# schmidtniko/visual_marker_mapping

Hardware: AMD Instinct MI355X
Metric: lm_iterations_per_sec (higher is better)
Workload: dtype f64; 1 GPU; configs[1]: 500 images x 200 tags, visibility 1.00, 100000 tag observations (400000 corner residual blocks), no loss, perturbed initial guess; eliminated_family=cameras, reduced_system_order=1200, elimination_form=dense Z + MFMA rank-k, kept_family_order=natural

## Files before the change

### visual_marker_mapping_amd/csrc/chol_common.hpp

```cpp
#pragma once
#include "engine.hpp"

namespace vmm {

constexpr int kLd = 65;
constexpr int kLdT = 66;

typedef double double4_t __attribute__((ext_vector_type(4)));

__device__ __forceinline__ double safe_rsqrt(double v, bool& ok)
{
    ok = ok && (v > 0.0) && isfinite(v);
    const double y0 = __builtin_amdgcn_rsq(v);
    const double e = fma(-v * y0, y0, 1.0);
    return fma(y0 * e, fma(e, 0.375, 0.5), y0);
}

__device__ __forceinline__ bool nz_bit(const unsigned long long* nz, const int i, const int k)
{
    return (nz[kDfMaskWords * i + (k >> 6)] >> (k & 63)) & 1ull;
}

constexpr int kPs = 9;
constexpr int kPw = 8;
// ... 19 lines not shown
        const double t = p.l[tri8(j, j)];
        bool okj = true;
        const double inv = safe_rsqrt(t, okj);
        p.ok = p.ok && okj;
        p.inv[j] = inv;
        p.l[tri8(j, j)] = t * inv;
#pragma unroll
        for (int i = j + 1; i < 8; ++i)
            p.l[tri8(i, j)] *= inv;
#pragma unroll
        for (int c = j + 1; c < 8; ++c)
#pragma unroll
            for (int i = c; i < 8; ++i)
                p.l[tri8(i, c)] = fma(-p.l[tri8(i, j)], p.l[tri8(c, j)], p.l[tri8(i, c)]);
    }
}

__device__ __forceinline__ void scale8(double (&x)[8], const Piv8& p)
{
#pragma unroll
    for (int q = 0; q < 8; ++q) {
        x[q] *= p.inv[q];
#pragma unroll
        for (int c = q + 1; c < 8; ++c)
            x[c] = fma(-x[q], p.l[tri8(c, q)], x[c]);
    }
}

constexpr unsigned kSpinLimit = 1u << 22;

__device__ __forceinline__ void raise_sync_timeout(LmCtl* ctl, int bit)
{
    atomicOr(&ctl->sync_timeout, bit);
    atomicExch(&ctl->done, 2);
}

__device__ __forceinline__ void chol_inverse_lds(const double* L, const double* di, double* __restrict__ Linvk)
{
    const int tid = threadIdx.x;
    if (tid >= 64)
        return;
    const int c = tid;
    double x[64];
#pragma unroll
    for (int i = 0; i < 64; ++i) {
        double s0 = 0.0, s1 = 0.0, s2 = 0.0, s3 = 0.0;
#pragma unroll
        for (int m = 0; m + 3 < i; m += 4) {
            s0 += L[i * kLd + m] * x[m];
            s1 += L[i * kLd + m + 1] * x[m + 1];
            s2 += L[i * kLd + m + 2] * x[m + 2];
            s3 += L[i * kLd + m + 3] * x[m + 3];
        }
#pragma unroll
        for (int m = (i / 4) * 4; m < i; ++m)
            s0 += L[i * kLd + m] * x[m];
        const double s = (s0 + s1) + (s2 + s3);
        x[i] = (i == c) ? di[i] : ((i < c) ? 0.0 : -s * di[i]);
        Linvk[i * 64 + c] = x[i];
    }
}

__device__ __forceinline__ void chol_inverse_wg(const double* __restrict__ Ldk, const double* __restrict__ dinvk,
                                                double* __restrict__ Linvk, double* smem)
{
    double* L = smem;
    double* di = smem + 64 * kLd;
// ... 13 lines not shown
```

### visual_marker_mapping_amd/csrc/covariance.hip

```cpp
#include <string.h>

#include <algorithm>
#include <functional>
#include <string>
#include <vector>

#include "host.hpp"

namespace vmm {

struct CovDensePath {
    Engine& e;
    bool v, nz;
    CovDensePath(Engine& e_) : e(e_), v(e_.sparse_schur), nz(e_.chol_nz_on) {}
    int enter()
    {
        if (v) {
            int drc;
            if ((drc = ensure_dense_schur(e))) return drc;
            e.sparse_schur = false;
        }
        e.chol_nz_on = false;
        return VMM_BA_OK;
    }
    ~CovDensePath()
    {
        e.sparse_schur = v;
        e.chol_nz_on = nz;
    }
};

static hipError_t cov_factor_and(Engine& e, int robustify, double huber_a, hipError_t err,
                                 const std::function<hipError_t()>& tail)
{
    vmm_ba_options o;
    vmm_ba_default_options(&o);
    o.robustify = robustify;
    o.huber_a = huber_a;
    for (int attempt = 0; attempt < 2 && err == hipSuccess; ++attempt) {
        init_ctl(e, *e.ctl_host, o, 0);
        err = hipMemcpyAsync(e.ctl, e.ctl_host, sizeof(LmCtl), hipMemcpyHostToDevice, e.stream);
        if (err != hipSuccess)
            break;
        launch_eval_passes(e, robustify, huber_a, false);
        launch_cov_prepare(e);
        launch_elim(e);
        launch_syrk_reduced(e);
        launch_cholesky_solve(e, e.S, e.n_pad, e.ldz, e.yf, e.ctl, attempt > 0);
        launch_chol_inverse(e, e.n_blk - 1);
        err = tail();
        if (err == hipSuccess)
            err = hipMemcpyAsync(e.ctl_host, e.ctl, sizeof(LmCtl), hipMemcpyDeviceToHost, e.stream);
        if (err == hipSuccess)
            err = hipStreamSynchronize(e.stream);
        if (err != hipSuccess || e.ctl_host->done != 2)
            break;
    }
    return err;
}

int tag_pose_handle(const Engine& e, const char* who)
{
    if (e.multi || e.points) {
        set_error(std::string(who) + " needs a single-GPU handle with tag-pose landmarks");
        return VMM_BA_ERR_STATE;
    }
    return VMM_BA_OK;
}

static int select_and_flush(Engine& e)
{
    HIP_TRY(hipSetDevice(e.device));
    return flush_state(e);
}

static int covariance_call(Engine& e, const char* who, int robustify, double huber_a,
                           const std::function<void(Arena&)>& carve, const std::function<hipError_t()>& tail,
                           const char* matrix = "J^T J", const std::function<hipError_t()>& upload = nullptr,
                           const std::string& alloc_step = "")
{
    CovDensePath dense(e);
    int rc;
    if ((rc = dense.enter())) return rc;
    Arena ar;
    if (ar.layout(carve) != hipSuccess)
        return hip_failure(who, alloc_step.c_str(), ar.err);
    const hipError_t err = cov_factor_and(e, robustify, huber_a, upload ? upload() : hipSuccess, tail);
    if (err != hipSuccess)
        return hip_failure(who, "", err);
    if (e.ctl_host->lin_fail) {
        set_error(std::string(who) + ": " + matrix + " is not positive definite (rank-deficient Jacobian)");
        return VMM_BA_ERR_NUMERIC;
    }
    return VMM_BA_OK;
}

}

using namespace vmm;

extern "C" {

int vmm_ba_tag_translation_covariance(vmm_ba_handle h, int robustify, double huber_a, double* cov)
{
    if (!h || !cov) {
        set_error("bad argument");
        return VMM_BA_ERR_ARGUMENT;
    }
    static const char who[] = "tag_translation_covariance";
    Engine& e = *reinterpret_cast<Engine*>(h);
    int rc;
    if ((rc = tag_pose_handle(e, who))) return rc;
    if ((rc = select_and_flush(e))) return rc;
    if (e.n_obs == 0 || e.n_tags == 0) {
        memset(cov, 0, sizeof(double) * 9 * (size_t)e.n_tags);
        return VMM_BA_OK;
    }
    const bool identity_rhs = e.elim_cams;
    const int n_rhs = identity_rhs ? e.n_pad : e.k_dim;
    const int ldb = round_up(n_rhs, 64);
    double *B = nullptr, *cov_dev = nullptr;
    auto carve = [&](Arena& a) {
        B = a.take<double>((size_t)e.n_pad * ldb);
// ... 138 lines not shown
```

### visual_marker_mapping_amd/csrc/diagnostics.hip

```cpp
#include <stdio.h>
#include <string.h>

#include <string>
#include <vector>

#include "host.hpp"

namespace vmm {

template <typename T, hipError_t (*Destroy)(T), int N = 1>
struct Owned {
    T h[N] = {};
    Owned() = default;
    Owned(const Owned&) = delete;
    Owned& operator=(const Owned&) = delete;
    ~Owned() { release(); }
    void release()
    {
        for (T& x : h) {
            if (x)
                (void)Destroy(x);
            x = nullptr;
        }
    }
// ... 61 lines not shown
    if ((rc = restore_raw())) return rc;
    OwnedEvents<2> events;
    hipEvent_t &ev0 = events.h[0], &ev1 = events.h[1];
    HIP_TRY(hipEventCreate(&ev0));
    HIP_TRY(hipEventCreate(&ev1));
    auto timed = [&](auto&& fn, auto&& prep, double* ms_out, int inner = 1) -> int {
        Owned<hipGraph_t, hipGraphDestroy> graph;
        Owned<hipGraphExec_t, hipGraphExecDestroy> exec;
        hipGraph_t& g = graph.h[0];
        hipGraphExec_t& ge = exec.h[0];
        HIP_TRY(hipStreamBeginCapture(e.stream, hipStreamCaptureModeThreadLocal));
        for (int q = 0; q < inner; ++q)
            fn();
        HIP_TRY(hipStreamEndCapture(e.stream, &g));
        HIP_TRY(hipGraphInstantiate(&ge, g, nullptr, nullptr, 0));
        graph.release();
        double total = 0.0;
        for (int r = 0; r < reps + 1; ++r) {
            prep();
            HIP_TRY(hipEventRecord(ev0, e.stream));
            HIP_TRY(hipGraphLaunch(ge, e.stream));
            HIP_TRY(hipEventRecord(ev1, e.stream));
            HIP_TRY(hipEventSynchronize(ev1));
            float ms = 0.f;
            HIP_TRY(hipEventElapsedTime(&ms, ev0, ev1));
            if (r > 0) total += ms;
        }
        exec.release();
        *ms_out = total / reps / inner;
        return VMM_BA_OK;
    };
    auto nop = [] {};
    HIP_TRY(hipMemcpy(e.ctl_host, e.ctl, sizeof(LmCtl), hipMemcpyDeviceToHost));
    e.ctl_host->done = 0;
    e.ctl_host->lin_fail = 0;
    HIP_TRY(hipMemcpy(e.ctl, e.ctl_host, sizeof(LmCtl), hipMemcpyHostToDevice));
    if ((rc = timed([&] { launch_eval_passes(e, o.robustify, o.huber_a, false); }, nop, &out->eval_elim_ms, 8))) return rc;
    out->eval_keep_ms = 0.0;
    if ((rc = timed([&] { launch_cost_kernel(e, e.cam_qt, e.tag_qt, false, o.robustify, o.huber_a); }, nop, &out->cost_ms, 8))) return rc;
    if ((rc = timed([&] { launch_elim(e); }, nop, &out->form_z_ms, 8))) return rc;
    if ((rc = timed([&] { launch_syrk_only(e); }, nop, &out->syrk_ms, 4))) return rc;
    if ((rc = timed([&] { launch_cholesky_solve(e, e.S, e.n_pad, e.ldz, e.yf, e.ctl); },
                    [&] {
                        launch_syrk_reduced(e);
                        launch_pack_lower(e, false);
                        launch_pack_lower(e, true);
                    },
                    &out->cholesky_ms)))
        return rc;
    if ((rc = timed([&] { launch_backsub(e); }, nop, &out->backsub_ms, 8))) return rc;
    if (e.sw.debug) {
        HIP_TRY(hipMemcpy(e.ctl_host, e.ctl, sizeof(LmCtl), hipMemcpyDeviceToHost));
        fprintf(stderr, "[vmm_ba debug] after kernel timing: done=%d lin_fail=%d termination=%d iteration=%d\n",
                e.ctl_host->done, e.ctl_host->lin_fail, e.ctl_host->termination, e.ctl_host->iteration);
    }
    if ((rc = restore_raw())) return rc;
    if ((rc = begin_lm_loop(e, ot, 0))) return rc;
    HIP_TRY(hipEventRecord(ev0, e.stream));
    int passes = 0;
    for (int r = 0; r < reps; ++r) {
        if ((rc = run_iteration(e, ot))) return rc;
        passes += e.last_passes;
    }
    HIP_TRY(hipEventRecord(ev1, e.stream));
    HIP_TRY(hipEventSynchronize(ev1));
    float ms = 0.f;
    HIP_TRY(hipEventElapsedTime(&ms, ev0, ev1));
    out->lm_iteration_ms = ms / passes;
    events.release();
    return restore_raw();
}

int vmm_ba_debug_chol_schedule(int n_blk, int n_df, int n_cu, int32_t* launches, int cap, int* n_launches, int* n_df_used)
{
    if (n_blk < 1 || n_cu < 1 || cap < 0 || (cap > 0 && !launches) || !n_launches || (n_df > 0 && n_df > n_blk - 2)) {
        set_error("bad argument");
        return VMM_BA_ERR_ARGUMENT;
    }
    if (n_df < 0) {
        n_df = dataflow_blocks(n_blk, n_cu, read_switches());
        if (n_df == n_blk)
            n_df = 0;
    }
    const std::vector<CholLaunch> sched = chol_step_schedule(n_blk, n_df);
    for (size_t i = 0; i < sched.size() && (int)i < cap; ++i) {
        const CholLaunch& L = sched[i];
        const int32_t row[8] = { L.k, L.lazy[0], L.lazy[1], L.upd[0], L.upd[1], L.c0, L.t0, L.t1 };
// ... 25 lines not shown
    Engine& e = *reinterpret_cast<Engine*>(h);
    if (e.multi || e.sparse_schur || !e.Z) {
        set_error("debug_overlap needs a single-GPU handle on the dense elimination path");
        return VMM_BA_ERR_STATE;
    }
    HIP_TRY(hipSetDevice(e.device));
    int rc;
    if ((rc = flush_state(e))) return rc;
    vmm_ba_options o;
    vmm_ba_default_options(&o);
    o.max_num_iterations = 1 << 30;
    o.function_tolerance = o.parameter_tolerance = o.gradient_tolerance = 0.0;
    if (e.trace_capacity < 1) {
        if ((rc = dev_alloc(e, &e.trace, 1, false))) return rc;
        e.trace_capacity = 1;
        drop_graphs(e);
    }
    if ((rc = begin_lm_loop(e, o, 0))) return rc;
    if ((rc = enqueue_iteration(e, o))) return rc;
    HIP_TRY(hipStreamSynchronize(e.stream));
    Arena scratch;
    Owned<hipStream_t, hipStreamDestroy> second;
    OwnedEvents<5> events;
    hipStream_t& sb = second.h[0];
    hipEvent_t(&ev)[5] = events.h;
    hipError_t err = scratch.alloc(sizeof(double) * (size_t)e.ldz * e.ldz);
    double* const S2 = reinterpret_cast<double*>(scratch.base);
    if (err == hipSuccess) err = hipStreamCreateWithFlags(&sb, hipStreamNonBlocking);
    for (int i = 0; i < 5 && err == hipSuccess; ++i)
        err = hipEventCreate(&ev[i]);
    auto reset_flags = [&]() -> hipError_t {
        hipError_t r = hipMemcpy(e.ctl_host, e.ctl, sizeof(LmCtl), hipMemcpyDeviceToHost);
        if (r != hipSuccess) return r;
        e.ctl_host->done = 0;
        e.ctl_host->lin_fail = 0;
        e.ctl_host->sync_timeout = 0;
        return hipMemcpy(e.ctl, e.ctl_host, sizeof(LmCtl), hipMemcpyHostToDevice);
    };
    double acc[8] = { 0.0, 0.0, 0.0, 0.0, 0.0, 0.0, 0.0, 0.0 };
    for (int r = 0; r < reps + 1 && err == hipSuccess; ++r) {
        float t[8] = { 0.f, 0.f, 0.f, 0.f, 0.f, 0.f, 0.f, 0.f };
        if ((err = reset_flags()) != hipSuccess) break;
        (void)hipEventRecord(ev[0], e.stream);
        launch_syrk_reduced(e);
        (void)hipEventRecord(ev[1], e.stream);
        launch_cholesky_solve(e, e.S, e.n_pad, e.ldz, e.yf, e.ctl);
        (void)hipEventRecord(ev[2], e.stream);
        if ((err = hipEventSynchronize(ev[2])) != hipSuccess) break;
        (void)hipEventElapsedTime(&t[0], ev[0], ev[1]);
        (void)hipEventElapsedTime(&t[1], ev[1], ev[2]);
        (void)hipEventElapsedTime(&t[2], ev[0], ev[2]);
        if ((err = reset_flags()) != hipSuccess) break;
        launch_syrk_reduced(e);
        if ((err = hipStreamSynchronize(e.stream)) != hipSuccess) break;
        (void)hipEventRecord(ev[0], e.stream);
        (void)hipStreamWaitEvent(sb, ev[0], 0);
        launch_cholesky_solve(e, e.S, e.n_pad, e.ldz, e.yf, e.ctl);
        (void)hipEventRecord(ev[3], e.stream);
        launch_syrk_plan(sb, e.ctl, e.Z, e.ldz, e.syrk);
        launch_reduce_plan(sb, e.ctl, e.syrk, e.ldz, e.n_pad + 1, S2);
        (void)hipEventRecord(ev[1], sb);
        (void)hipStreamWaitEvent(e.stream, ev[1], 0);
        (void)hipEventRecord(ev[2], e.stream);
        if ((err = hipEventSynchronize(ev[2])) != hipSuccess) break;
        (void)hipEventElapsedTime(&t[3], ev[0], ev[2]);
        (void)hipEventElapsedTime(&t[4], ev[0], ev[3]);
        (void)hipEventElapsedTime(&t[5], ev[0], ev[1]);
        if ((err = reset_flags()) != hipSuccess) break;
// ... 34 lines not shown
```

### visual_marker_mapping_amd/csrc/engine.hpp

```cpp
#pragma once
#include <hip/hip_runtime.h>
#include <stdint.h>

#include <string>
#include <vector>

#include "../../include/vmm_ba.h"
#include "geom.hpp"
#include "plan.hpp"

namespace vmm {

constexpr int kLdsRow = 80;

struct ObsOrder {
    int64_t n = 0;
    int64_t n_pad = 0;
    int32_t* own = nullptr;
    int32_t* other = nullptr;
    int32_t* caller = nullptr;
    double* px = nullptr;
    Task* tasks = nullptr;
    int32_t n_tasks = 0;
    int32_t* pose_task = nullptr;
    double* part = nullptr;
    int32_t* start = nullptr;
};

struct LmCtl {
    int32_t max_num_iterations, robustify, jacobi_scaling, max_invalid;
    double huber_a, function_tolerance, gradient_tolerance, parameter_tolerance;
    double max_radius, min_radius, min_relative_decrease, min_lm_diagonal, max_lm_diagonal;
    double radius, decrease_factor;
    int32_t reuse_diagonal, num_invalid;
    double x_cost, cand_cost, model_cost_change, x_norm, initial_cost;
    int32_t iteration;
    int32_t first_eval;
    int32_t done, termination;
    int32_t lin_fail;
    int32_t sync_timeout;
    int32_t num_sync_timeouts;
    int32_t sync_kernels;
    uint32_t spin_limit_df, spin_limit_chain;
    int32_t spin_wg;
    int32_t records;
    int32_t num_successful, num_unsuccessful, num_lm_iterations, num_jac_evals, num_cost_evals;
    int32_t trace_capacity;
    int32_t w_which;
    vmm_ba_iteration cur;
    unsigned long long stamp[6];
    unsigned long long phase_ticks[5];
};

__device__ __forceinline__ int64_t small_sel(const LmCtl* ctl, const int64_t alt_off) { return ctl->w_which ? alt_off : 0; }

__device__ __forceinline__ void phase_stamp(const LmCtl* ctl, int slot)
{
    if (blockIdx.x == 0 && blockIdx.y == 0 && threadIdx.x == 0)
        const_cast<LmCtl*>(ctl)->stamp[slot] = __builtin_amdgcn_s_memrealtime();
}

struct SyrkPlan {
    int n_tiles = 0, n_kt = 0, n_wg = 0, n_segments = 0;
    int32_t *tile_bi = nullptr, *tile_bj = nullptr, *wg_seg0 = nullptr, *tile_seg0 = nullptr;
    int64_t *wg_u0 = nullptr, *wg_u1 = nullptr;
    double* partials = nullptr;
    bool wide = false;
};

struct Engine {
    int device = 0;
    int n_cu = 256;
    hipStream_t stream = nullptr;
    int rank = 0, world = 1;
    Switches sw;
    bool multi = false;
    vmm_ba_allreduce_fn allreduce = nullptr;
    void* allreduce_user = nullptr;
    void* rccl_comm = nullptr;
    bool rccl_graph = true;

    Intrinsics K;
    int n_cams = 0, n_tags = 0, fixed_tag = -1;
    bool points = false;
    int n_tags_user = 0;
    int64_t n_obs_user = 0;
    std::vector<double> user_tag_wh;
    int64_t n_obs = 0;
    bool elim_cams = true;
    int n_e = 0, n_f = 0;

    double* cam_qt = nullptr;
    double* tag_qt = nullptr;
    double* cam_cand = nullptr;
    double* tag_cand = nullptr;
    double* tag_wh = nullptr;

    ObsOrder ordE, ordF;
// ... 149 lines not shown
        return p;
    }
    template <typename Carve>
    hipError_t layout(Carve&& carve)
    {
        carve(*this);
        const size_t total = used;
        used = 0;
        if (alloc(total) == hipSuccess)
            carve(*this);
        return err;
    }
    void copy(void* dst, const void* src, size_t bytes, hipMemcpyKind kind)
    {
        if (err == hipSuccess)
            err = hipMemcpy(dst, src, bytes, kind);
    }
};

int preload_eval_kernels();
int preload_schur_kernels();
int preload_chol_kernels();
int preload_lm_kernels();
int preload_cov_kernels();
int preload_init_kernels();

void launch_eval_passes(Engine& e, int robustify, double huber_a, bool use_ctl);
void launch_cost_kernel(Engine& e, const double* cam, const double* tag, bool guard, int robustify, double huber_a);
void launch_cost(Engine& e, const double* cam, const double* tag, bool guard, int robustify, double huber_a,
                 double* out_scalar);
void launch_stats(Engine& e, double* per_corner_dev);
void launch_project(hipStream_t st, const Intrinsics& K, int64_t n, const double* pc, double* uv);
void launch_sum(Engine& e, bool guard, const double* in, int n, double* out);
void launch_elim(Engine& e);
void launch_schur_rows(Engine& e, bool add_diag);
void launch_syrk_only(Engine& e);
void launch_syrk_reduced(Engine& e);
void launch_pack_lower(Engine& e, bool unpack);
void launch_syrk_plan(hipStream_t st, const LmCtl* ctl, const double* Z, int ldz, const SyrkPlan& p);
void launch_reduce_plan(hipStream_t st, const LmCtl* ctl, const SyrkPlan& p, int ld, int n_rows, double* S);
void launch_cholesky_solve(Engine& e, double* S, int n_pad, int ld, double* y, LmCtl* ctl, bool safe = false);
int dataflow_workgroups(int n_blk);
int dataflow_max_workgroups(int n_cu, const Switches& sw);
int dataflow_blocks(int n_blk, int n_cu, const Switches& sw);
void launch_chol_inverse(Engine& e, int k);
struct CholLaunch {
    int k;
    int lazy[2];
    int upd[2];
    int c0, t0, t1;
};
std::vector<CholLaunch> chol_step_schedule(int n_blk, int n_df);
void chol_schedule_tile(int n_blk, const CholLaunch& L, int t, int* bi, int* bj);
void launch_chol_steps(Engine& e, double* S, int n_pad, int ld, LmCtl* ctl, int n_df);
int preload_chol_step_kernels();
void launch_dataflow(Engine& e, double* S, int n_pad, int ld, LmCtl* ctl, int first_blk, int n_blk);
int preload_chol_dataflow_kernels();
void launch_backsolve_chain(Engine& e, double* S, int n_pad, int ld, double* y, LmCtl* ctl);
void launch_backsolve_steps(Engine& e, double* S, int n_pad, int ld, double* y, LmCtl* ctl);
int preload_backsolve_kernels();
void launch_cov_prepare(Engine& e);
void launch_cov_rhs(Engine& e, double* B, int ldb, bool identity_rhs);
void launch_cov_trsm(Engine& e, double* B, int ldb, int n_chunks, bool identity_rhs);
void launch_cov_gram(Engine& e, const double* X, int ldb, double* cov_dev);
void launch_cov_rhs_slots(Engine& e, const int32_t* slot_src, int n_slots, double* B, int ldb);
void launch_cov_trsm_mfma(Engine& e, double* B, int ldb, const std::vector<int>& chunks_at);
// ... 168 lines not shown
```

### visual_marker_mapping_amd/csrc/kernels_backsolve.hip

```cpp
#include "chol_common.hpp"

namespace vmm {

__global__ __launch_bounds__(256) void k_backsolve_step(const LmCtl* ctl, double* __restrict__ S, int ld,
                                                        int n_pad, int n_blk, int kb, double* __restrict__ y,
                                                        const double* __restrict__ dinv,
                                                        const double* __restrict__ Ld)
{
    if (ctl->done || ctl->lin_fail)
        return;
    __shared__ double red[4][64];
    __shared__ double L[64 * kLd];
    __shared__ double ws[64];
    __shared__ double di[64];
    const int m = blockIdx.x;
    const int tid = threadIdx.x;
    const int c = tid & 63, part = tid >> 6;
    double* w = S + (int64_t)n_pad * ld;
    double wc = 0.0;
    if (kb + 1 < n_blk) {
        const int R0 = (kb + 1) * kNB + part * 16;
        const double* Lb = S + (int64_t)R0 * ld + m * kNB + c;
        double acc = 0.0;
#pragma unroll
        for (int r = 0; r < 16; ++r)
            acc += Lb[(int64_t)r * ld] * y[R0 + r];
        red[part][c] = acc;
    }
    if (m == kb) {
        const int K0 = kb * kNB;
        for (int idx = tid; idx < 64 * 64; idx += 256) {
            const int r = idx >> 6, cc = idx & 63;
            L[r * kLd + cc] = (cc <= r) ? Ld[(int64_t)kb * 4096 + r * 64 + cc] : 0.0;
        }
        if (tid < 64)
            di[tid] = dinv[K0 + tid];
    }
    __syncthreads();
    if (part == 0) {
        wc = w[m * kNB + c];
        if (kb + 1 < n_blk) {
            wc -= (red[0][c] + red[1][c]) + (red[2][c] + red[3][c]);
// ... 27 lines not shown

int backsolve_chain_workgroups(int n_blk) { return n_blk; }

__device__ __forceinline__ void chain_block_done(unsigned* n_done, int n_blk, unsigned* epoch_word, unsigned epoch)
{
    if (atomicAdd(n_done, 1u) == (unsigned)n_blk - 1u) {
        *n_done = 0u;
        *epoch_word = epoch;
    }
}

#ifdef VMM_STAMPS
__device__ unsigned long long g_chain_stamps[128][4];
#define CH_RT(blk, slot)                                                                  \
    do {                                                                                  \
        if (threadIdx.x == 0)                                                             \
            g_chain_stamps[(blk) & 127][slot] = __builtin_amdgcn_s_memrealtime();         \
    } while (0)
extern "C" int vmm_ba_debug_read_chain_stamps(unsigned long long* out)
{
    return (int)hipMemcpyFromSymbol(out, HIP_SYMBOL(g_chain_stamps), sizeof(unsigned long long) * 128 * 4);
}
#else
#define CH_RT(blk, slot)
#endif

template <bool TREE>
__device__ __forceinline__ void backsolve_chain_body(LmCtl* ctl, const double* __restrict__ S, int ld, int n_pad, int n_blk,
                                                     double* y, const double* __restrict__ dinv, unsigned long long* gran,
                                                     unsigned* epoch_word, const double* __restrict__ Ld,
                                                     const double* __restrict__ Linv,
                                                     const unsigned long long* __restrict__ nz, unsigned* n_done)
{
    if (ctl->done || ctl->lin_fail) {
        if constexpr (TREE) {
            if (threadIdx.x == 0)
                chain_block_done(n_done, n_blk, epoch_word, *epoch_word + 1u);
        } else {
            if (blockIdx.x == gridDim.x - 1 && threadIdx.x == 0)
                *epoch_word = *epoch_word + 1u;
        }
        return;
    }
    const unsigned spin_limit = (ctl->spin_limit_chain && (ctl->spin_wg < 0 || ctl->spin_wg == (int)blockIdx.x))
                                    ? ctl->spin_limit_chain : kSpinLimit;
    __shared__ double L[64 * kLd];
    __shared__ double Li[64 * kLd];
    __shared__ double red[4][64];
    __shared__ double ws[64];
    __shared__ double ys[2][64];
    __shared__ double sB[16][256];
    __shared__ int s_timeout;
    const int m = n_blk - 1 - (int)blockIdx.x;
    const int tid = threadIdx.x;
    const int c = tid & 63, part = tid >> 6;
    const unsigned epoch = *epoch_word + 1u;
    const int K0 = m * kNB;
    if (tid == 0)
        s_timeout = 0;
    CH_RT(m, 0);
    auto receive = [&](const int j, double* ysj) {
        if (part == 0) {
            const unsigned long long* g = gran + 2 * (int64_t)(j * kNB + c);
            unsigned long long x0, x1;
            for (unsigned n = 0;;) {
                x0 = __hip_atomic_load(g, __ATOMIC_RELAXED, __HIP_MEMORY_SCOPE_AGENT);
                x1 = __hip_atomic_load(g + 1, __ATOMIC_RELAXED, __HIP_MEMORY_SCOPE_AGENT);
                const bool ok = (unsigned)(x0 >> 32) == epoch && (unsigned)(x1 >> 32) == epoch;
                if (__all(ok) && spin_limit != 1u)
                    break;
                __builtin_amdgcn_s_sleep(1);
                if (++n >= spin_limit) {
                    s_timeout = 1;
                    break;
                }
            }
            ysj[c] = __longlong_as_double((long long)(((x1 & 0xffffffffull) << 32) | (x0 & 0xffffffffull)));
        }
// ... 205 lines not shown
```

### visual_marker_mapping_amd/csrc/kernels_chol_dataflow.hip

```cpp
#include <type_traits>
#include <utility>

#include "chol_common.hpp"

namespace vmm {

constexpr int kDfSlice = 2 * 8 * 64;
constexpr int kPsD = 10;
constexpr unsigned kDfSpinDefault = 1u << 21;
constexpr int kDfXs = 8 * kLdsRow;
constexpr int kDfSmemUsed = 64 * kLdT + 4 * 64 * kPsD + 64 + 2 * 8 * kPsD + 4 * kDfXs;
constexpr int kDfSmem = 84 * 1024 / 8;
static_assert(kDfSmemUsed <= kDfSmem, "dataflow LDS layout");
static_assert(4 * 64 * kPsD + 64 + 4 * kDfXs >= 64 * kLd + 64, "the inverse's staging area must fit into the dead buffers");

struct DfArgs {
    LmCtl* ctl;
    double* S;
    int ld, n_pad, n_blk;
    double* dinv;
    double* Ld;
    double* Linv;
    unsigned long long* G;
    const unsigned* epoch_word;
// ... 819 lines not shown
        const double* XJ = m.Xs + (it & 1) * 2 * kDfXs;
        const double* XR = XJ + kDfXs;
        __syncthreads();
        if (WK == 0 || HAS_T) {
            Ops o[2];
            load_ops_slice<WK, HAS_T>(XJ, XR, fr, fk, o);
            for_tiles([&](auto idx) {
                constexpr int I = decltype(idx)::value;
                if constexpr ((HAS_T || !is_t(WK, I)) && I >= kHelpSplit)
                    mfma_tile<WK, I>(acc, o);
            }, Seq13{});
        }
    }
    double* M = m.RA + WK * (13 - kHelpSplit) * 256;
    for_tiles([&](auto idx) {
        constexpr int I = decltype(idx)::value;
        if constexpr (I >= kHelpSplit) {
#pragma unroll
            for (int r = 0; r < 4; ++r)
                M[((I - kHelpSplit) * 4 + r) * 64 + lane] = acc[I][r];
        }
    }, Seq13{});
    __syncthreads();
}

__device__ __forceinline__ void report_give_up(const DfArgs& a, const unsigned epoch, const int& s_timeout)
{
    if (threadIdx.x == 0
        && (s_timeout || __hip_atomic_load(a.abort_word, __ATOMIC_RELAXED, __HIP_MEMORY_SCOPE_AGENT) == epoch))
        raise_sync_timeout(a.ctl, 1);
}

template <bool HAS_T, bool TREE, int MODE>
__device__ __forceinline__ void role(const DfArgs& a, const int j, const int R, double* smem)
{
    constexpr bool BULK = (MODE & 1) != 0, HELP = (MODE & 2) != 0;
    const int tid = threadIdx.x;
    const int lane = tid & 63;
    const int w = __builtin_amdgcn_readfirstlane(tid >> 6);
    const int K0 = j * kNB;
    const int R0 = R * kNB;
    const int n_blk = a.n_blk, ld = a.ld, n_pad = a.n_pad;
    if (TREE && HAS_T && R < n_blk && !nz_bit(a.nz, R, j))
        return;
    const unsigned epoch = *a.epoch_word + 1u;
    Lds m;
    m.RA = smem;
    m.Pd = m.RA + 64 * kLdT;
    m.Pt = m.Pd + 2 * 64 * kPsD;
    m.invd = m.Pt + 2 * 64 * kPsD;
    m.Pb = m.invd + 64;
    m.Nd = m.Pb + 8 * kPsD;
    m.Xs = m.Nd + 8 * kPsD;
    m.stamp_j = -1;
#ifdef VMM_STAMPS
    if (TREE ? !HAS_T : (HAS_T && R == j + 1))
        m.stamp_j = j;
    {
        const bool stamp_on = m.stamp_j >= 0 && w == 0;
        const int stamp_j = m.stamp_j;
        DF_RT(0);
    }
#endif
    double* Li = m.Pd;
    double* di = Li + 64 * kLd;
    __shared__ int s_timeout;
    if (tid == 0)
        s_timeout = 0;
    SliceMap sm;
    sm.G = a.G;
    sm.n_blk = n_blk;
    sm.slot = TREE ? a.slot : nullptr;
    __syncthreads();
    bool ok = true;
    if (w < 2)
        pivot_path<HAS_T, TREE, MODE>(a, w, lane, j, R, m, sm, epoch, &s_timeout, ok);
    else if (w == 2)
        worker_path<0, HAS_T, TREE, HELP>(a, lane, j, R, m);
// ... 15 lines not shown
        for (int idx = tid; idx < 64 * 64; idx += 256) {
            const int r = idx >> 6, c = idx & 63;
            const double v = (c <= r) ? m.RA[c * kLdT + r] : 0.0;
            if (c <= r)
                a.Ld[(int64_t)j * 4096 + r * 64 + c] = v;
            Li[r * kLd + c] = v;
        }
        if (tid < 64)
            di[tid] = iv;
        __syncthreads();
        if (j < n_blk - 1)
            chol_inverse_lds(Li, di, a.Linv + (int64_t)j * 4096);
        report_give_up(a, epoch, s_timeout);
        return;
    }
    for (int idx = tid; idx < 64 * 32; idx += 256) {
        const int rr = idx >> 5, c = (idx & 31) * 2;
        if (R0 + rr <= n_pad)
            *reinterpret_cast<double2*>(a.S + (int64_t)(R0 + rr) * ld + K0 + c)
                = make_double2(m.RA[rr * kLd + c], m.RA[rr * kLd + c + 1]);
    }
    if (BULK) {
        double* cb = a.Gc + sm.index(j, R) * 4096;
        for (int idx = tid; idx < 64 * 64; idx += 256) {
            const int c = idx >> 6, rr = idx & 63;
            cb[idx] = m.RA[rr * kLd + c];
        }
        __threadfence();
        __syncthreads();
        if (tid == 0)
            __hip_atomic_store(a.done + sm.index(j, R), epoch, __ATOMIC_RELEASE, __HIP_MEMORY_SCOPE_AGENT);
    }
    if (j == n_blk - 1 && tid == 0 && !ok)
        a.ctl->lin_fail = 1;
    report_give_up(a, epoch, s_timeout);
}

}

template <bool TREE, int MODE>
__device__ __forceinline__ void chol_dataflow_body(DfArgs& a)
{
    if (a.ctl->done)
        return;
    a.spin_limit = (a.ctl->spin_limit_df && (a.ctl->spin_wg < 0 || a.ctl->spin_wg == (int)blockIdx.x)) ? a.ctl->spin_limit_df
                                                                                                          : kDfSpinDefault;
    phase_stamp(a.ctl, 3);
    if (a.ctl->lin_fail)
        return;
    __shared__ __attribute__((aligned(16))) double smem[kDfSmem];
    if (TREE) {
        const int j = a.wg[2 * (int)blockIdx.x], R = a.wg[2 * (int)blockIdx.x + 1];
        if (R > j)
            df2::role<true, TREE, MODE>(a, j, R, smem);
        else
            df2::role<false, TREE, MODE>(a, j, j, smem);
        return;
    }
    int b = (int)blockIdx.x, j = 0;
    for (; j < a.n_blk; ++j) {
        const int cnt = a.n_blk - j + 1;
        if (b < cnt)
            break;
        b -= cnt;
    }
    if (j >= a.n_blk)
        return;
    if (b < a.n_blk - j)
        df2::role<true, TREE, MODE>(a, j, j + 1 + b, smem);
    else
        df2::role<false, TREE, MODE>(a, j, j, smem);
}

__global__ __launch_bounds__(256) void k_chol_dataflow(DfArgs a)
{
    chol_dataflow_body<false, 0>(a);
}

__global__ __launch_bounds__(256) void k_chol_dataflow_bulk(DfArgs a)
{
    chol_dataflow_body<false, 1>(a);
}

__global__ __launch_bounds__(256) void k_chol_dataflow_tree(DfArgs a)
{
    chol_dataflow_body<true, 1>(a);
}

__global__ __launch_bounds__(384) void k_chol_dataflow_tree_help(DfArgs a)
{
    chol_dataflow_body<true, 3>(a);
}

void launch_dataflow(Engine& e, double* S, int n_pad, int ld, LmCtl* ctl, int first_blk, int n_blk)
{
    DfArgs a;
    a.ctl = ctl;
    a.S = S + (int64_t)first_blk * kNB * (ld + 1);
    a.ld = ld;
    a.n_pad = n_pad - first_blk * kNB;
    a.n_blk = n_blk - first_blk;
    a.dinv = e.dinv + first_blk * kNB;
    a.Ld = e.Ldiag + (int64_t)first_blk * 4096;
    a.Linv = e.Linv + (int64_t)first_blk * 4096;
// ... 35 lines not shown
```

### visual_marker_mapping_amd/csrc/kernels_chol_step.hip

```cpp
#include "chol_common.hpp"

namespace vmm {

#ifdef VMM_STAMPS
__device__ unsigned long long g_stamps[64];
#define STAMP(slot)                                                                  \
    do {                                                                             \
        if (blockIdx.x == 1 && threadIdx.x == 0 && k == 1) {                         \
            g_stamps[slot] = __builtin_amdgcn_s_memtime();                           \
            g_stamps[16 + slot] = __builtin_amdgcn_s_memrealtime();                  \
        }                                                                            \
    } while (0)
#define USTAMP(slot)                                                                 \
    do {                                                                             \
        if (u == 0 && threadIdx.x == 0 && k == 1 && t == u + n_wg)                   \
            g_stamps[(slot)] = __builtin_amdgcn_s_memtime();                         \
    } while (0)
#else
#define USTAMP(slot)
#define STAMP(slot)
#endif

template <int J0, bool HAS_T>
__device__ __forceinline__ void panel_round(const int w, const int lane,
// ... 146 lines not shown
            if (HAS_T)
                *reinterpret_cast<double2*>(&Ats[mm * kLdsRow + c]) = vt[it];
        }
        __syncthreads();
#pragma unroll 4
        for (int ks = 0; ks < 16; ++ks) {
            const int row = (ks * 4 + fk) * kLdsRow;
            const double ad = -Ads[row + 16 * w + fr];
            const double at = HAS_T ? -Ats[row + 16 * w + fr] : 0.0;
#pragma unroll
            for (int tj = 0; tj < 4; ++tj) {
                const double b = Ads[row + 16 * tj + fr];
                const double adm = (tj <= w) ? ad : 0.0;
                Dacc[tj] = __builtin_amdgcn_mfma_f64_16x16x4f64(adm, b, Dacc[tj], 0, 0, 0);
                if (HAS_T)
                    Tacc[tj] = __builtin_amdgcn_mfma_f64_16x16x4f64(at, b, Tacc[tj], 0, 0, 0);
            }
        }
    }
    STAMP(1);
    bool ok = true;
    panel_round<0, HAS_T>(w, lane, Dacc, Tacc, Pd, Pt, RA, RA, invd, ok);
    panel_round<8, HAS_T>(w, lane, Dacc, Tacc, Pd, Pt, RA, RA, invd, ok);
    panel_round<16, HAS_T>(w, lane, Dacc, Tacc, Pd, Pt, RA, RA, invd, ok);
    panel_round<24, HAS_T>(w, lane, Dacc, Tacc, Pd, Pt, RA, RA, invd, ok);
    panel_round<32, HAS_T>(w, lane, Dacc, Tacc, Pd, Pt, RA, RA, invd, ok);
    panel_round<40, HAS_T>(w, lane, Dacc, Tacc, Pd, Pt, RA, RA, invd, ok);
    panel_round<48, HAS_T>(w, lane, Dacc, Tacc, Pd, Pt, RA, RA, invd, ok);
    panel_round<56, HAS_T>(w, lane, Dacc, Tacc, Pd, Pt, RA, RA, invd, ok);
    __syncthreads();
    STAMP(2);
    if (!HAS_T) {
        if (tid == 0 && !ok)
            ctl->lin_fail = 1;
        if (tid < 64)
            dinv[K0 + tid] = invd[tid];
        for (int idx = tid; idx < 64 * 64; idx += 256) {
            const int r = idx >> 6, c = idx & 63;
            if (c <= r)
                Ld[(int64_t)k * 4096 + r * 64 + c] = RA[c * kLdT + r];
        }
        return;
    }
    STAMP(4);
    const double* R = RA;
    for (int idx = tid; idx < 64 * 32; idx += 256) {
        const int rr = idx >> 5, c = (idx & 31) * 2;
        if (R0 + rr <= n_pad)
            *reinterpret_cast<double2*>(S + (int64_t)(R0 + rr) * ld + K0 + c)
                = make_double2(R[rr * kLd + c], R[rr * kLd + c + 1]);
    }
    {
        const int rr = tid & 63;
        if (R0 + rr <= n_pad)
            for (int c = tid >> 6; c < 64; c += 4)
                P[(int64_t)c * ld + R0 + rr] = R[rr * kLd + c];
    }
    STAMP(5);
}

constexpr int kPanelSmem = 64 * kLdT + 4 * 64 * kPs + 64 + 2 * 64 * kLdsRow;
constexpr int kUpdateSmem = 4 * 64 * kLdsRow;
constexpr int kStepSmem = kPanelSmem > kUpdateSmem ? kPanelSmem : kUpdateSmem;

__device__ __forceinline__ void chol_panel_wg(LmCtl* ctl, double* __restrict__ S, int ld, int n_pad, int k,
                                              double* __restrict__ P, const double* __restrict__ Pprev,
                                              const double* __restrict__ Pprev2, double* __restrict__ dinv,
// ... 394 lines not shown
#pragma unroll
        for (int a = 0; a < 2; ++a)
#pragma unroll
            for (int b = 0; b < 2; ++b)
#pragma unroll
                for (int r = 0; r < 4; ++r)
                    __builtin_nontemporal_store(creg[a][b][r] + acc[a][b][r],
                                                &S[(int64_t)(I0 + wi * 32 + a * 16 + fk + 4 * r) * ld + J0 + wj * 32 + b * 16 + fi]);
#pragma unroll
        for (int it = 0; it < 8; ++it) {
            const int idx = it * 256 + tid;
            const int m = idx >> 5, c = (idx & 31) * 2;
            *reinterpret_cast<double2v*>(&L0[m * kLdsRow + c]) = wa[it];
            *reinterpret_cast<double2v*>(&L0[(64 + m) * kLdsRow + c]) = wb[it];
        }
        __syncthreads();
        bi = nbi;
        bj = nbj;
        t = tn;
        tn = slot[2 + (iter & 1)];
        if (t >= t1)
            break;
    }
}

__global__ __launch_bounds__(256) void k_chol_step(LmCtl* ctl, double* __restrict__ S, int ld, int n_pad, int n_blk,
                                                   int k, int n_panel, double* __restrict__ Pcur,
                                                   const double* __restrict__ Pprev, const double* __restrict__ Pprev2,
                                                   double* __restrict__ dinv, double* __restrict__ Ld,
                                                   double* __restrict__ Linv, const double* __restrict__ PA,
                                                   const double* __restrict__ PB, int c0, int t0, int t1, int n_upd_wg,
                                                   unsigned* tile_ctr)
{
    if (ctl->done)
        return;
    if (k == 0)
        phase_stamp(ctl, 3);
    if (ctl->lin_fail)
        return;
    if (blockIdx.x == 0 && threadIdx.x == 0)
        tile_ctr[(k + 1) & 1] = 0u;
    __shared__ __attribute__((aligned(16))) double smem[kStepSmem];
    if ((int)blockIdx.x < n_panel) {
        chol_panel_wg(ctl, S, ld, n_pad, k, Pcur, Pprev, Pprev2, dinv, Ld, smem);
        if (t1 > t0) {
            __syncthreads();
            if (PB)
                chol_update2_wg(S, ld, n_blk, c0, tile_ctr + (k & 1), t0, t1, PA, PB, smem);
            else
                chol_update_wg(S, ld, n_blk, c0 - 2, tile_ctr + (k & 1), t1, PA, smem);
        }
    } else if ((int)blockIdx.x < n_panel + n_upd_wg) {
        if (PB)
            chol_update2_wg(S, ld, n_blk, c0, tile_ctr + (k & 1), t0, t1, PA, PB, smem);
        else
            chol_update_wg(S, ld, n_blk, c0 - 2, tile_ctr + (k & 1), t1, PA, smem);
    } else
        chol_inverse_wg(Ld + (int64_t)(k - 1) * 4096, dinv + (k - 1) * kNB, Linv + (int64_t)(k - 1) * 4096, smem);
}

__global__ __launch_bounds__(256) void k_chol_inverse(const LmCtl* ctl, const double* __restrict__ Ld,
                                                      const double* __restrict__ dinv, double* __restrict__ Linv, int k)
{
    if (ctl->done || ctl->lin_fail)
        return;
    __shared__ __attribute__((aligned(16))) double smem[64 * kLd + 64];
    chol_inverse_wg(Ld + (int64_t)k * 4096, dinv + k * kNB, Linv + (int64_t)k * 4096, smem);
}

void launch_chol_inverse(Engine& e, int k)
{
    hipLaunchKernelGGL(k_chol_inverse, dim3(1), dim3(256), 0, e.stream, (const LmCtl*)e.ctl, (const double*)e.Ldiag,
                       (const double*)e.dinv, e.Linv, k);
}

constexpr int kPairMinBlocks = 46;

static int update_tiles(int n_blk, int k)
{
    int tiles = 0;
    for (int r = k + 2; r <= n_blk; ++r)
        tiles += ((r < n_blk) ? r : n_blk - 1) - (k + 1);
    return tiles;
}

std::vector<CholLaunch> chol_step_schedule(int n_blk, int n_df)
{
    std::vector<CholLaunch> out;
    const int n_step = n_blk - n_df;
    int k_pair = 0;
    while (n_blk - k_pair > kPairMinBlocks)
        k_pair += 2;
    if (k_pair > n_step)
        k_pair = n_step;
    for (int k = 0; k < n_step; ++k) {
        CholLaunch L = { k, { -1, k > 0 ? k - 1 : -1 }, { -1, -1 }, k + 1, 0, 0 };
        if (k >= 2 && k <= k_pair) {
// ... 73 lines not shown
```

### visual_marker_mapping_amd/csrc/kernels_eval.hip

```cpp
#include "engine.hpp"

namespace vmm {

struct EvalArgs {
    Intrinsics K;
    const Task* tasks;
    int n_tasks;
    const int32_t* other;
    const double* px;
    int64_t n_pad;
    const double* own_pose;
    const double* other_pose;
    const double* tag_wh;
    const uint8_t* cam_const;
    const uint8_t* tag_const;
    int robustify;
    double huber_a;
    double* part;
    void* W;
    void* W_alt;
    const int32_t* caller;
    const uint8_t* mask;
    const LmCtl* ctl;
};

__device__ __forceinline__ int tri(int a, int b) { return a * (a + 1) / 2 + b; }

template <bool OWN_IS_CAM, bool WRITE_W, typename AT, bool POINTS = false>
__device__ __forceinline__ void eval_body(const EvalArgs& a, const int wave)
{
    const int lane = threadIdx.x & 63;
    if (wave >= a.n_tasks)
        return;
    const Task t = a.tasks[wave];
    const int64_t i = (int64_t)t.begin + lane;
    const bool valid = i < t.end;
    const int64_t is = valid ? i : t.begin;
    const int o = a.other[is];
    AT* __restrict__ const Wout = static_cast<AT*>((WRITE_W && a.W_alt && a.ctl && a.ctl->w_which == 0) ? a.W_alt : a.W);

    const int tag_idx = OWN_IS_CAM ? o : t.pose;
    const int cam_idx = OWN_IS_CAM ? t.pose : o;
    const double* camq = (OWN_IS_CAM ? a.own_pose : a.other_pose) + 7 * (int64_t)cam_idx;
    const double* tagq = (OWN_IS_CAM ? a.other_pose : a.own_pose) + 7 * (int64_t)tag_idx;
    Rigid cam, tag;
    double pt[6];
    if (POINTS) {
        load_rigid<false>(camq, cam);
#pragma unroll
        for (int k = 0; k < 6; ++k)
            pt[k] = tagq[k];
    } else {
        load_rigid<true>(camq, cam);
        load_rigid<true>(tagq, tag);
    }
    const double hw = POINTS ? 0.0 : 0.5 * a.tag_wh[2 * tag_idx], hh = POINTS ? 0.0 : 0.5 * a.tag_wh[2 * tag_idx + 1];
    const bool cam_c = a.cam_const[cam_idx] != 0, tag_c = a.tag_const[tag_idx] != 0;
    const bool on = valid && a.mask[a.caller[is]];

    AT H[21];
    double g[6], cost = 0.0;
    AT Wacc[WRITE_W ? 36 : 1];
#pragma unroll
    for (int k = 0; k < 21; ++k)
        H[k] = (AT)0;
#pragma unroll
    for (int k = 0; k < 6; ++k)
        g[k] = 0.0;
    if (WRITE_W) {
#pragma unroll
        for (int k = 0; k < 36; ++k)
            Wacc[k] = (AT)0;
    }

    constexpr bool NEED_JC = OWN_IS_CAM || WRITE_W;
    constexpr bool NEED_JT = !OWN_IS_CAM || WRITE_W;
#pragma unroll 1
    for (int c = 0; c < (POINTS ? 2 : 4); ++c) {
        const double sx = (c == 1 || c == 2) ? hw : -hw;
        const double sy = (c >= 2) ? hh : -hh;
        const double u = a.px[(2 * c) * a.n_pad + is];
        const double v = a.px[(2 * c + 1) * a.n_pad + is];
        CornerEval e;
        if (POINTS) {
            eval_point<NEED_JC, NEED_JT>(a.K, cam, camq, pt[3 * c], pt[3 * c + 1], pt[3 * c + 2], u, v, e, on);
            if (NEED_JT) {
#pragma unroll
                for (int r = 0; r < 2; ++r) {
                    const double j0 = e.jt[r][0], j1 = e.jt[r][1], j2 = e.jt[r][2];
                    e.jt[r][0] = c == 0 ? j0 : 0.0;
                    e.jt[r][1] = c == 0 ? j1 : 0.0;
// ... 40 lines not shown
#pragma unroll
                for (int p = 0; p < 6; ++p)
#pragma unroll
                    for (int q = 0; q < 6; ++q)
                        Wacc[6 * p + q] += ja[p] * jx[q];
            }
        }
    }
    if (WRITE_W && valid) {
#pragma unroll
        for (int k = 0; k < 36; ++k)
            Wout[(int64_t)k * a.n_pad + i] = Wacc[k];
    }
    double red[32];
#pragma unroll
    for (int k = 0; k < 21; ++k)
        red[k] = (double)H[k];
#pragma unroll
    for (int k = 0; k < 6; ++k)
        red[21 + k] = g[k];
    red[27] = cost;
#pragma unroll
    for (int k = 28; k < 32; ++k)
        red[k] = 0.0;
    const double mine = wave_sum32(red, lane);
    const int slot = wave_sum32_index(lane);
    if (!(lane & 1) && slot < 28)
        a.part[(int64_t)wave * kPart + slot] = mine;
}

template <bool E_IS_CAM, typename AT = double, bool POINTS = false>
__global__ __launch_bounds__(256) __attribute__((amdgpu_waves_per_eu(2, 2))) void k_eval_both(const EvalArgs aE, const EvalArgs aF, const int nb_e)
{
    if (aE.ctl) {
        if (aE.ctl->done)
            return;
        phase_stamp(aE.ctl, 0);
    }
    if ((int)blockIdx.x < nb_e)
        eval_body<E_IS_CAM, true, AT, POINTS>(aE, (int)((blockIdx.x * blockDim.x + threadIdx.x) >> 6));
    else
        eval_body<!E_IS_CAM, false, AT, POINTS>(aF, (int)(((blockIdx.x - nb_e) * blockDim.x + threadIdx.x) >> 6));
}


struct FusedArgs {
    const int32_t* pair_obs;
    const int32_t* e_list;
    const int32_t* e_part0;
    int n_e_act, n_f, n_f_pad, n_chunks, group, n_groups;
    double* partF;
};

template <bool E_IS_CAM, typename AT, bool POINTS>
__global__ __launch_bounds__(256) __attribute__((amdgpu_waves_per_eu(1, 1)))
void k_eval_fused(const EvalArgs a, const FusedArgs fa)
{
    if (a.ctl) {
        if (a.ctl->done)
            return;
        phase_stamp(a.ctl, 0);
    }
    const int lane = threadIdx.x & 63;
    const int wave = (int)((blockIdx.x * blockDim.x + threadIdx.x) >> 6);
    if (wave >= fa.n_groups * fa.n_chunks)
        return;
    const int grp = wave / fa.n_chunks, c = wave - grp * fa.n_chunks;
    const int f = 64 * c + lane;
    const bool fvalid = f < fa.n_f;
    const int fs = fvalid ? f : fa.n_f - 1;
    AT* __restrict__ const Wout = static_cast<AT*>((a.W_alt && a.ctl && a.ctl->w_which == 0) ? a.W_alt : a.W);
    const double* keptq = a.other_pose + 7 * (int64_t)fs;
    Rigid kept;
    double pt[6];
    if (POINTS && E_IS_CAM) {
#pragma unroll
        for (int k = 0; k < 6; ++k)
            pt[k] = keptq[k];
    } else if (POINTS) {
        load_rigid<false>(keptq, kept);
    } else {
        load_rigid<true>(keptq, kept);
    }
    AT HF[21];
    double gF[6];
#pragma unroll
    for (int k = 0; k < 21; ++k)
        HF[k] = (AT)0;
#pragma unroll
    for (int k = 0; k < 6; ++k)
        gF[k] = 0.0;
    const int e0 = grp * fa.group, e1 = min(e0 + fa.group, fa.n_e_act);
    constexpr int NPX = POINTS ? 4 : 8;
    int e_n = __builtin_amdgcn_readfirstlane(fa.e_list[e0]);
    int idx_n = fvalid ? fa.pair_obs[(int64_t)e_n * fa.n_f_pad + f] : -1;
    int e_nn = e_n, idx_nn = -1;
    if (e0 + 1 < e1) {
        e_nn = __builtin_amdgcn_readfirstlane(fa.e_list[e0 + 1]);
        idx_nn = fvalid ? fa.pair_obs[(int64_t)e_nn * fa.n_f_pad + f] : -1;
    }
    double px_n[NPX];
    int on_n;
    {
        const int64_t isn = idx_n >= 0 ? idx_n : 0;
// ... 133 lines not shown
            red[k] = 0.0;
        const double mine = wave_sum32(red, lane);
        const int slot = wave_sum32_index(lane);
        if (!(lane & 1) && slot < 28)
            a.part[(int64_t)(fa.e_part0[e] + c) * kPart + slot] = mine;
    }
    if (fvalid) {
        double* pf = fa.partF + (int64_t)grp * 28 * fa.n_f_pad + f;
#pragma unroll
        for (int k = 0; k < 21; ++k)
            pf[(int64_t)k * fa.n_f_pad] = (double)HF[k];
#pragma unroll
        for (int k = 0; k < 6; ++k)
            pf[(int64_t)(21 + k) * fa.n_f_pad] = gF[k];
    }
}

struct ReduceArgs {
    int n_pose;
    const int32_t* pose_task;
    int n_fixed;
    int64_t st, sk, sp;
    const double* part;
    double* Hout;
    double* gout;
    double* pose_cost;
    const double* pose7;
    int euclid;
    double* gm_out;
};

__global__ void k_reduce_pose(const LmCtl* ctl, const ReduceArgs rE, const ReduceArgs rF, const int64_t alt_off)
{
    int64_t off = 0;
    if (ctl) {
        if (ctl->done)
            return;
        off = ctl->w_which ? 0 : alt_off;
    }
    int tid = blockIdx.x * blockDim.x + threadIdx.x;
    const bool first = tid < 32 * rE.n_pose;
    if (!first)
        tid -= 32 * rE.n_pose;
    const ReduceArgs& r = first ? rE : rF;
    const int n_pose = r.n_pose;
    const int32_t* __restrict__ pose_task = r.pose_task;
    const double* __restrict__ part = r.part;
    double* __restrict__ Hout = r.Hout + off;
    double* __restrict__ gout = r.gout + off;
    double* __restrict__ pose_cost = r.pose_cost;
    const int p = tid >> 5, k = tid & 31;
    if (p >= n_pose || k >= 28)
        return;
    const int t0 = pose_task ? pose_task[p] : 0, t1 = pose_task ? pose_task[p + 1] : r.n_fixed;
    const double* __restrict__ pp = part + (int64_t)k * r.sk + (int64_t)p * r.sp;
    double s0 = 0.0, s1 = 0.0, s2 = 0.0, s3 = 0.0;
    int t = t0;
    for (; t + 3 < t1; t += 4) {
        s0 += pp[(int64_t)t * r.st];
        s1 += pp[(int64_t)(t + 1) * r.st];
        s2 += pp[(int64_t)(t + 2) * r.st];
        s3 += pp[(int64_t)(t + 3) * r.st];
    }
    if (t < t1) s0 += pp[(int64_t)t * r.st];
    if (t + 1 < t1) s1 += pp[(int64_t)(t + 1) * r.st];
    if (t + 2 < t1) s2 += pp[(int64_t)(t + 2) * r.st];
    const double s = (s0 + s1) + (s2 + s3);
    if (k < 21) {
        int a = 0;
        while ((a + 1) * (a + 2) / 2 <= k)
            ++a;
        const int b = k - a * (a + 1) / 2;
        Hout[36 * (int64_t)p + 6 * a + b] = s;
        Hout[36 * (int64_t)p + 6 * b + a] = s;
    } else if (k < 27) {
        gout[6 * (int64_t)p + (k - 21)] = s;
    } else if (pose_cost) {
        pose_cost[p] = s;
    }
    if (r.gm_out) {
        double ng[6];
#pragma unroll
        for (int j = 0; j < 6; ++j)
            ng[j] = -__shfl(s, 21 + j, 32);
        if (k == 21) {
            const double* x = r.pose7 + 7 * (int64_t)p;
            double xp[7], gm = 0.0;
            if (r.euclid) {
#pragma unroll
                for (int j = 0; j < 6; ++j)
                    xp[j] = x[j] + ng[j];
                xp[6] = x[6];
            } else {
                pose_plus(x, ng, xp);
            }
#pragma unroll
            for (int j = 0; j < 7; ++j)
                gm = fmax(gm, fabs(x[j] - xp[j]));
            r.gm_out[p] = gm;
        }
    }
}

__global__ __launch_bounds__(256) void k_sum(const LmCtl* ctl, const double* __restrict__ in, int n, int stride,
                                             double* __restrict__ out)
{
    if (ctl && ctl->done)
        return;
    __shared__ double sh[256];
    double s = 0.0;
    for (int i = threadIdx.x; i < n; i += 256)
        s += in[(int64_t)i * stride];
    sh[threadIdx.x] = s;
    __syncthreads();
    for (int m = 128; m >= 1; m >>= 1) {
        if ((int)threadIdx.x < m)
            sh[threadIdx.x] += sh[threadIdx.x + m];
        __syncthreads();
    }
    if (threadIdx.x == 0)
        out[0] = sh[0];
}

struct CostArgs {
    Intrinsics K;
    const Task* tasks;
    int n_tasks;
    const int32_t* other;
    const double* px;
    int64_t n_pad;
    const double* own_pose;
    const double* other_pose;
    const double* tag_wh;
    int robustify;
    double huber_a;
    double* part;
    const int32_t* caller;
    const uint8_t* mask;
    const LmCtl* ctl;
};

template <bool OWN_IS_CAM, bool POINTS = false>
__global__ __launch_bounds__(256) void k_cost(const CostArgs a)
{
    if (a.ctl && a.ctl->done)
        return;
    const int wave = (int)((blockIdx.x * blockDim.x + threadIdx.x) >> 6);
    const int lane = threadIdx.x & 63;
    if (wave >= a.n_tasks)
        return;
    const Task t = a.tasks[wave];
    const int64_t i = (int64_t)t.begin + lane;
    const bool valid = i < t.end;
    const int64_t is = valid ? i : t.begin;
    const int o = a.other[is];
    const int tag_idx = OWN_IS_CAM ? o : t.pose;
    const int cam_idx = OWN_IS_CAM ? t.pose : o;
    const double* camq = (OWN_IS_CAM ? a.own_pose : a.other_pose) + 7 * (int64_t)cam_idx;
    const double* tagq = (OWN_IS_CAM ? a.other_pose : a.own_pose) + 7 * (int64_t)tag_idx;
    Rigid cam, tag;
    double pt[6];
    if (POINTS) {
        load_rigid<false>(camq, cam);
#pragma unroll
        for (int k = 0; k < 6; ++k)
            pt[k] = tagq[k];
    } else {
        load_rigid<true>(camq, cam);
        load_rigid<true>(tagq, tag);
    }
    const double hw = POINTS ? 0.0 : 0.5 * a.tag_wh[2 * tag_idx], hh = POINTS ? 0.0 : 0.5 * a.tag_wh[2 * tag_idx + 1];
    double cost = 0.0;
#pragma unroll
    for (int c = 0; c < (POINTS ? 2 : 4); ++c) {
        const double sx = (c == 1 || c == 2) ? hw : -hw;
        const double sy = (c >= 2) ? hh : -hh;
        CornerEval e;
        if (POINTS)
// ... 105 lines not shown
    const double rad = 1.0 + r2 * (K.k1 + r2 * (K.k2 + r2 * K.k3));
    double xd, yd;
    distort(K, true, x, y, r2, rad, xd, yd);
    uv[2 * i] = K.fx * xd + K.cx;
    uv[2 * i + 1] = K.fy * yd + K.cy;
}


static inline int blocks_for_tasks(int n_tasks) { return (n_tasks + 3) / 4; }

static EvalArgs make_eval_args(Engine& e, const ObsOrder& ord, bool own_is_cam, void* W, bool lm = false)
{
    EvalArgs a;
    a.K = e.K;
    a.tasks = ord.tasks;
    a.n_tasks = ord.n_tasks;
    a.other = ord.other;
    a.px = ord.px;
    a.n_pad = ord.n_pad;
    const double* cam = lm ? e.cam_cand : e.cam_qt;
    const double* tag = lm ? e.tag_cand : e.tag_qt;
    a.own_pose = own_is_cam ? cam : tag;
    a.other_pose = own_is_cam ? tag : cam;
    a.tag_wh = e.tag_wh;
    a.cam_const = e.pose_const;
    a.tag_const = e.pose_const + e.n_cams;
    a.robustify = 0;
    a.huber_a = 1.0;
    a.part = ord.part;
    a.W = W;
    a.W_alt = (lm && W) ? (e.f32_accum ? (void*)e.Wf2 : (void*)e.W2) : nullptr;
    a.caller = ord.caller;
    a.mask = e.obs_mask;
    a.ctl = e.ctl;
    return a;
}

void launch_eval_passes(Engine& e, int robustify, double huber_a, bool use_ctl)
{
    const bool e_is_cam = e.elim_cams;
    const bool lm = use_ctl;
    EvalArgs aE = make_eval_args(e, e.ordE, e_is_cam, e.f32_accum ? (void*)e.Wf : (void*)e.W, lm);
    EvalArgs aF = make_eval_args(e, e.ordF, !e_is_cam, nullptr, lm);
    aE.robustify = aF.robustify = robustify;
    aE.huber_a = aF.huber_a = huber_a;
    if (!use_ctl)
        aE.ctl = aF.ctl = nullptr;
    const int nb_e = blocks_for_tasks(aE.n_tasks), nb_f = blocks_for_tasks(aF.n_tasks);
    if (e.fused_eval) {
        FusedArgs fa;
        fa.pair_obs = e.pair_obs;
        fa.e_list = e.fused_e_list;
        fa.e_part0 = e.fused_e_part0;
        fa.n_e_act = e.fused_n_e_act;
        fa.n_f = e.n_f;
        fa.n_f_pad = e.fused_f_pad;
        fa.n_chunks = e.fused_chunks;
        fa.group = e.fused_group;
        fa.n_groups = e.fused_groups;
        fa.partF = e.fused_partF;
        aE.part = e.fused_partE;
        const int n_waves = fa.n_groups * fa.n_chunks;
        const dim3 grid((n_waves + 3) / 4);
        if (n_waves > 0) {
            if (e.points) {
                if (e_is_cam)
// ... 43 lines not shown
    rE.pose7 = want_gm ? (e_is_cam ? e.cam_cand : e.tag_cand) : nullptr;
    rE.euclid = (e.points && !e_is_cam) ? 1 : 0;
    rE.gm_out = want_gm ? e.pose_gm + (e_is_cam ? 0 : e.n_cams) : nullptr;
    rF.pose7 = want_gm ? (e_is_cam ? e.tag_cand : e.cam_cand) : nullptr;
    rF.euclid = (e.points && e_is_cam) ? 1 : 0;
    rF.gm_out = want_gm ? e.pose_gm + (e_is_cam ? e.n_cams : 0) : nullptr;
    rF.n_pose = e.n_f;
    rF.pose_task = e.ordF.pose_task;
    rF.part = e.ordF.part;
    rE.n_fixed = rF.n_fixed = 0;
    rE.st = rF.st = kPart;
    rE.sk = rF.sk = 1;
    rE.sp = rF.sp = 0;
    if (e.fused_eval) {
        rE.pose_task = e.fused_pose_task;
        rE.part = e.fused_partE;
        rF.pose_task = nullptr;
        rF.n_fixed = e.fused_groups;
        rF.part = e.fused_partF;
        rF.st = 28 * (int64_t)e.fused_f_pad;
        rF.sk = e.fused_f_pad;
        rF.sp = 1;
    }
    rF.Hout = e_is_cam ? oH_tag : oH_cam;
    rF.gout = e_is_cam ? og_tag : og_cam;
    rF.pose_cost = nullptr;
    hipLaunchKernelGGL(k_reduce_pose, dim3(((e.n_e + e.n_f) * 32 + 255) / 256), dim3(256), 0, e.stream, ctl, rE, rF,
                       (lm && !e.multi) ? e.small_alt_off : (int64_t)0);
    if (!lm)
        hipLaunchKernelGGL(k_sum, dim3(1), dim3(256), 0, e.stream, ctl, e.part_cost, e.n_e, 1,
                           e.cost_slot);
}

void launch_sum(Engine& e, bool guard, const double* in, int n, double* out)
{
    hipLaunchKernelGGL(k_sum, dim3(1), dim3(256), 0, e.stream, guard ? e.ctl : (const LmCtl*)nullptr, in, n, 1, out);
}

void launch_cost_kernel(Engine& e, const double* cam, const double* tag, bool guard, int robustify, double huber_a)
{
    CostArgs a;
    a.K = e.K;
    a.tasks = e.ordE.tasks;
    a.n_tasks = e.ordE.n_tasks;
    a.other = e.ordE.other;
    a.px = e.ordE.px;
    a.n_pad = e.ordE.n_pad;
    a.own_pose = e.elim_cams ? cam : tag;
    a.other_pose = e.elim_cams ? tag : cam;
    a.tag_wh = e.tag_wh;
    a.robustify = robustify;
    a.huber_a = huber_a;
    a.part = e.part_k1;
    a.caller = e.ordE.caller;
    a.mask = e.obs_mask;
    a.ctl = guard ? e.ctl : nullptr;
    if (a.n_tasks <= 0)
        return;
    const dim3 grid(blocks_for_tasks(a.n_tasks));
    if (e.points) {
        if (e.elim_cams)
            hipLaunchKernelGGL((k_cost<true, true>), grid, dim3(256), 0, e.stream, a);
        else
            hipLaunchKernelGGL((k_cost<false, true>), grid, dim3(256), 0, e.stream, a);
    } else if (e.elim_cams)
        hipLaunchKernelGGL((k_cost<true>), grid, dim3(256), 0, e.stream, a);
// ... 15 lines not shown
    double* part_cam = e.stats_part;
    double* part_tag = e.stats_part + oc.n_tasks;
    int32_t* n_cam = e.stats_cnt;
    int32_t* n_tag = e.stats_cnt + oc.n_tasks;
    StatsArgs a;
    a.K = e.K;
    a.tag_wh = e.tag_wh;
    a.mask = e.obs_mask;
    a.tasks = oc.tasks; a.n_tasks = oc.n_tasks; a.other = oc.other; a.caller = oc.caller; a.px = oc.px;
    a.n_pad = oc.n_pad; a.own_pose = e.cam_qt; a.other_pose = e.tag_qt; a.part = part_cam; a.part_n = n_cam;
    a.per_corner = per_corner_dev;
    if (a.n_tasks > 0)
        hipLaunchKernelGGL((k_stats<true>), dim3(blocks_for_tasks(a.n_tasks)), dim3(256), 0, e.stream, a);
    a.tasks = ot.tasks; a.n_tasks = ot.n_tasks; a.other = ot.other; a.caller = ot.caller; a.px = ot.px;
    a.n_pad = ot.n_pad; a.own_pose = e.tag_qt; a.other_pose = e.cam_qt; a.part = part_tag; a.part_n = n_tag;
    a.per_corner = nullptr;
    if (a.n_tasks > 0)
        hipLaunchKernelGGL((k_stats<false>), dim3(blocks_for_tasks(a.n_tasks)), dim3(256), 0, e.stream, a);
    hipLaunchKernelGGL(k_stats_pose, dim3((e.n_cams + e.n_tags + 255) / 256), dim3(256), 0, e.stream, e.n_cams,
                       (const int32_t*)oc.pose_task, (const double*)part_cam, (const int32_t*)n_cam, e.n_tags,
                       (const int32_t*)ot.pose_task, (const double*)part_tag, (const int32_t*)n_tag, e.stats_pose);
}

void launch_project(hipStream_t st, const Intrinsics& K, int64_t n, const double* pc, double* uv)
{
    if (n > 0)
        hipLaunchKernelGGL(k_project, dim3((unsigned)((n + 255) / 256)), dim3(256), 0, st, K, n, pc, uv);
}

int preload_eval_kernels()
{
    hipFuncAttributes at;
    int bad = 0;
    bad += hipFuncGetAttributes(&at, reinterpret_cast<const void*>(&k_eval_both<true, double>)) != hipSuccess;
    bad += hipFuncGetAttributes(&at, reinterpret_cast<const void*>(&k_eval_both<false, double>)) != hipSuccess;
    bad += hipFuncGetAttributes(&at, reinterpret_cast<const void*>(&k_eval_both<true, float>)) != hipSuccess;
    bad += hipFuncGetAttributes(&at, reinterpret_cast<const void*>(&k_eval_both<false, float>)) != hipSuccess;
    bad += hipFuncGetAttributes(&at, reinterpret_cast<const void*>(&k_eval_both<true, double, true>)) != hipSuccess;
    bad += hipFuncGetAttributes(&at, reinterpret_cast<const void*>(&k_eval_both<false, double, true>)) != hipSuccess;
    bad += hipFuncGetAttributes(&at, reinterpret_cast<const void*>(&k_eval_fused<true, double, false>)) != hipSuccess;
    bad += hipFuncGetAttributes(&at, reinterpret_cast<const void*>(&k_eval_fused<false, double, false>)) != hipSuccess;
    bad += hipFuncGetAttributes(&at, reinterpret_cast<const void*>(&k_eval_fused<true, float, false>)) != hipSuccess;
    bad += hipFuncGetAttributes(&at, reinterpret_cast<const void*>(&k_eval_fused<false, float, false>)) != hipSuccess;
    bad += hipFuncGetAttributes(&at, reinterpret_cast<const void*>(&k_eval_fused<true, double, true>)) != hipSuccess;
    bad += hipFuncGetAttributes(&at, reinterpret_cast<const void*>(&k_eval_fused<false, double, true>)) != hipSuccess;
    bad += hipFuncGetAttributes(&at, reinterpret_cast<const void*>(&k_cost<true, true>)) != hipSuccess;
    bad += hipFuncGetAttributes(&at, reinterpret_cast<const void*>(&k_cost<false, true>)) != hipSuccess;
    bad += hipFuncGetAttributes(&at, reinterpret_cast<const void*>(&k_reduce_pose)) != hipSuccess;
    bad += hipFuncGetAttributes(&at, reinterpret_cast<const void*>(&k_sum)) != hipSuccess;
    bad += hipFuncGetAttributes(&at, reinterpret_cast<const void*>(&k_cost<true>)) != hipSuccess;
    bad += hipFuncGetAttributes(&at, reinterpret_cast<const void*>(&k_cost<false>)) != hipSuccess;
    bad += hipFuncGetAttributes(&at, reinterpret_cast<const void*>(&k_stats<true>)) != hipSuccess;
    bad += hipFuncGetAttributes(&at, reinterpret_cast<const void*>(&k_stats<false>)) != hipSuccess;
    bad += hipFuncGetAttributes(&at, reinterpret_cast<const void*>(&k_stats_pose)) != hipSuccess;
    bad += hipFuncGetAttributes(&at, reinterpret_cast<const void*>(&k_project)) != hipSuccess;
    return bad;
}

}
```

### visual_marker_mapping_amd/csrc/kernels_lm.hip

```cpp
#include <float.h>

#include "engine.hpp"

namespace vmm {

__device__ __forceinline__ void control_reduce(double (&v)[8], double (&m)[2], double* sh)
{
    const int lane = threadIdx.x & 63, wave = threadIdx.x >> 6;
    const int nw = blockDim.x >> 6;
#pragma unroll
    for (int level = 0; level < 3; ++level) {
        const int off = 32 >> level;
        const bool hi = (lane & off) != 0;
#pragma unroll
        for (int j = 0; j < (4 >> level); ++j) {
            const double keep = hi ? v[2 * j + 1] : v[2 * j];
            const double send = hi ? v[2 * j] : v[2 * j + 1];
            v[j] = keep + __shfl_xor(send, off, 64);
        }
    }
#pragma unroll
    for (int off = 4; off >= 1; off >>= 1)
        v[0] += __shfl_xor(v[0], off, 64);
    {
// ... 59 lines not shown

#ifdef VMM_STAMPS
__device__ unsigned long long g_ctl_stamps[16];
#define CTL_RT(slot)                                                    \
    do {                                                                \
        if (threadIdx.x == 0)                                           \
            g_ctl_stamps[slot] = __builtin_amdgcn_s_memrealtime();      \
    } while (0)
extern "C" int vmm_ba_debug_read_ctl_stamps(unsigned long long* out)
{
    return (int)hipMemcpyFromSymbol(out, HIP_SYMBOL(g_ctl_stamps), sizeof(unsigned long long) * 16);
}
#else
#define CTL_RT(slot)
#endif

struct DecideArgs {
    const double* pose_part;
    const double* cross_parts;
    int n_cross;
    const double* cost_parts;
    int n_cost;
    const double* pose_gm;
};

__global__ __launch_bounds__(1024) void k_control(LmCtl* ctl, PoseViews pv, const DecideArgs dz,
                                                 const double* __restrict__ src, double* __restrict__ dst,
                                                 size_t small_count, const double* __restrict__ H0,
                                                 const double* __restrict__ g0, const int64_t alt_off,
                                                 double* __restrict__ scale, int32_t* __restrict__ active,
                                                 double* __restrict__ diag, double* __restrict__ D2,
                                                 vmm_ba_iteration* __restrict__ trace)
{
    if (ctl->done)
        return;
    const unsigned long long t_begin = __builtin_amdgcn_s_memrealtime();
    CTL_RT(0);
    __shared__ double sh[256];
    __shared__ int s_stop, s_reuse, s_accept, s_moved;
    __shared__ double s_radius, s_lo, s_hi;
    const int tid = threadIdx.x;
    const int n_pose = pv.n_cams + pv.n_tags;
    const int n_tan = 6 * n_pose;
    const bool first = ctl->first_eval != 0;
    const bool jacobi = ctl->jacobi_scaling != 0;
    const int which = ctl->w_which;
    const bool staged = src != dst;
    const double* __restrict__ nb = staged ? src : dst + (which ? 0 : alt_off);
    const double* __restrict__ Hn = nb + (H0 - dst);
    const double* __restrict__ gn = nb + (g0 - dst);
    __shared__ LmCtl s_c;
    if (tid == 0)
        s_c = *ctl;
    double gd = 0.0, quad = 0.0, sn = 0.0, xn = 0.0, bad = 0.0, cross = 0.0, ccost = 0.0, xn0 = 0.0, gm = 0.0;
    for (int p = tid; p < n_pose; p += (int)blockDim.x) {
        if (!first) {
            const double* o = dz.pose_part + 5 * (int64_t)p;
            gd += o[0];
            quad += o[1];
            sn += o[2];
            xn += o[3];
            bad = fmax(bad, o[4]);
        }
        const double* Hp = Hn + 36 * (int64_t)p;
        int act;
        if (first) {
            act = (Hp[0] + Hp[7] + Hp[14]) > 0.0 ? 1 : 0;
            active[p] = act;
            for (int k = 0; k < 6; ++k)
                scale[6 * (int64_t)p + k] = jacobi ? 1.0 / (1.0 + sqrt(Hp[7 * k])) : 1.0;
        } else {
            act = active[p];
        }
        if (act) {
            const double* x = pose_ptr(pv, p, true);
            if (first)
                for (int k = 0; k < 7; ++k)
                    xn0 += x[k] * x[k];
            if (dz.pose_gm) {
                gm = fmax(gm, dz.pose_gm[p]);
            } else {
                double ng[6], xp[7];
                for (int k = 0; k < 6; ++k)
                    ng[k] = -gn[6 * (int64_t)p + k];
                block_plus(pv, p, x, ng, xp);
                for (int k = 0; k < 7; ++k)
                    gm = fmax(gm, fabs(x[k] - xp[k]));
            }
        }
    }
    if (!first)
        for (int i = tid; i < dz.n_cross; i += (int)blockDim.x)
            cross += dz.cross_parts[i];
    for (int i = tid; i < dz.n_cost; i += (int)blockDim.x)
        ccost += dz.cost_parts[i];
    CTL_RT(1);
    double red[8] = { gd, quad, sn, xn, cross, ccost, xn0, 0.0 };
    double redm[2] = { bad, gm };
    control_reduce(red, redm, sh);
    CTL_RT(2);
    if (tid == 0) {
        LmCtl& c = s_c;
        gd = red[0];
        quad = red[1];
        sn = red[2];
        xn = red[3];
        cross = red[4];
        ccost = red[5];
        xn0 = red[6];
        bad = redm[0];
        gm = redm[1];
        auto span = [](unsigned long long a, unsigned long long b) { return b > a ? b - a : 0ull; };
        int accept = 0;
        if (first) {
            c.w_which = which ^ 1;
            c.phase_ticks[0] += span(c.stamp[0], t_begin);
        } else {
            const bool lin_fail = c.lin_fail != 0 || bad != 0.0;
            const double mcc = lin_fail ? 0.0 : -gd - 0.5 * (quad + 2.0 * cross);
            c.model_cost_change = mcc;
            c.cur.model_cost_change = mcc;
            const bool valid = !lin_fail && (mcc > 0.0);
            c.cur.step_is_valid = valid ? 1 : 0;
            if (!valid) {
                c.num_invalid++;
                if (c.num_invalid >= c.max_invalid) {
                    c.done = 1;
                    c.termination = VMM_BA_FAILURE;
                } else {
                    c.radius = c.radius / c.decrease_factor;
                    c.decrease_factor *= 2.0;
                    c.reuse_diagonal = 1;
                    c.cur.cost = c.x_cost;
                    c.cur.step_is_successful = 0;
                }
            } else {
                c.num_invalid = 0;
                double cand = ccost;
                c.num_cost_evals++;
                if (!isfinite(cand))
                    cand = DBL_MAX;
                c.cand_cost = cand;
                const double step_norm = sqrt(sn);
                c.cur.step_norm = step_norm;
                const double x_cost = c.x_cost;
                const double cost_change = x_cost - cand;
                if (step_norm <= c.parameter_tolerance * (c.x_norm + c.parameter_tolerance)) {
                    c.done = 1;
                    c.termination = VMM_BA_CONVERGENCE;
                } else if (fabs(cost_change) <= c.function_tolerance * x_cost) {
                    c.cur.cost_change = cost_change;
                    c.done = 1;
                    c.termination = VMM_BA_CONVERGENCE;
                } else {
                    c.cur.cost_change = cost_change;
                    const double rd = (cand >= DBL_MAX) ? -DBL_MAX : cost_change / mcc;
                    c.cur.relative_decrease = rd;
                    if (rd > c.min_relative_decrease) {
                        accept = 1;
                        const double q = 2.0 * rd - 1.0;
                        double den = 1.0 - q * q * q;
                        den = den < 1.0 / 3.0 ? 1.0 / 3.0 : den;
                        double r = c.radius / den;
                        c.radius = r > c.max_radius ? c.max_radius : r;
                        c.decrease_factor = 2.0;
                        c.reuse_diagonal = 0;
                        c.w_which = which ^ 1;
                        c.x_norm = sqrt(xn);
                        c.cur.step_is_successful = 1;
                    } else {
                        c.cur.step_is_successful = 0;
                        c.cur.cost = cand;
                        c.radius = c.radius / c.decrease_factor;
                        c.decrease_factor *= 2.0;
                        c.reuse_diagonal = 1;
                    }
                }
            }
            c.phase_ticks[0] += span(c.stamp[0], t_begin);
            c.phase_ticks[1] += span(c.stamp[5], c.stamp[2]);
            c.phase_ticks[2] += span(c.stamp[2], c.stamp[3]);
            c.phase_ticks[3] += span(c.stamp[3], c.stamp[4]);
            c.phase_ticks[4] += span(c.stamp[4], c.stamp[0]);
        }
        c.stamp[5] = t_begin;
        const int moved = (first || accept) ? 1 : 0;
        if (!c.done && moved) {
            const double cst = ccost;
            c.x_cost = cst;
            c.num_jac_evals++;
            if (first) {
                c.first_eval = 0;
                c.initial_cost = cst;
                c.x_norm = sqrt(xn0);
                c.cur.iteration = 0;
                c.cur.step_is_valid = 1;
                c.cur.step_is_successful = 1;
            }
            c.cur.cost = cst;
            c.cur.gradient_max_norm = gm;
            if (!isfinite(cst)) {
                c.done = 1;
                c.termination = VMM_BA_FAILURE;
            }
        }
        int stop = c.done;
        if (!stop) {
            vmm_ba_iteration cur = c.cur;
            cur.trust_region_radius = c.radius;
            if (cur.step_is_successful)
                c.num_successful++;
            else
                c.num_unsuccessful++;
            if (c.records < c.trace_capacity)
                trace[c.records] = cur;
            c.records++;
            if (cur.iteration >= c.max_num_iterations) {
                stop = 1;
                c.termination = VMM_BA_NO_CONVERGENCE;
            } else if (cur.step_is_successful && cur.gradient_max_norm <= c.gradient_tolerance) {
                stop = 1;
                c.termination = VMM_BA_CONVERGENCE;
            } else if (c.radius <= c.min_radius) {
                stop = 1;
                c.termination = VMM_BA_CONVERGENCE;
            }
            if (stop) {
                c.done = 1;
            } else {
                vmm_ba_iteration z;
                z.iteration = cur.iteration + 1;
                z.step_is_valid = 0;
                z.step_is_successful = 0;
                z.reserved = 0;
                z.cost = c.x_cost;
                z.cost_change = 0.0;
                z.gradient_max_norm = cur.gradient_max_norm;
                z.step_norm = 0.0;
                z.relative_decrease = 0.0;
                z.trust_region_radius = 0.0;
                z.model_cost_change = 0.0;
                c.cur = z;
                c.iteration = z.iteration;
                c.lin_fail = 0;
                c.num_lm_iterations++;
            }
        }
        s_stop = stop;
        s_accept = accept;
        s_moved = moved;
        s_reuse = c.reuse_diagonal;
        s_radius = c.radius;
        s_lo = c.min_lm_diagonal;
        s_hi = c.max_lm_diagonal;
        if (!stop)
            c.reuse_diagonal = 1;
        else
            c.phase_ticks[1] += span(t_begin, __builtin_amdgcn_s_memrealtime());
        CTL_RT(3);
        *ctl = c;
        CTL_RT(4);
    }
    __syncthreads();
    CTL_RT(5);
    if (s_accept) {
        for (int i = tid; i < 7 * pv.n_cams; i += (int)blockDim.x)
            pv.cam_qt[i] = pv.cam_cand[i];
        for (int i = tid; i < 7 * pv.n_tags; i += (int)blockDim.x)
            pv.tag_qt[i] = pv.tag_cand[i];
    }
    if (staged && s_moved)
        for (size_t i = tid; i < small_count; i += blockDim.x)
            dst[i] = src[i];
    if (s_stop)
        return;
    const double* __restrict__ Hx = s_moved ? Hn : H0 + (which ? alt_off : 0);
    const double lo = s_lo, hi = s_hi;
    for (int q = tid; q < n_tan; q += (int)blockDim.x) {
        double d;
        if (!s_reuse) {
            const int p = q / 6, k = q % 6;
            const double sc = scale[q];
            d = sc * sc * Hx[36 * (int64_t)p + 7 * k];
            d = fmin(fmax(d, lo), hi);
            diag[q] = d;
        } else {
            d = diag[q];
        }
        const double lm = sqrt(d / s_radius);
        D2[q] = lm * lm;
    }
    CTL_RT(6);
}

__device__ __forceinline__ void candidate_for_pose(const PoseViews& pv, const int p, const double (&d)[6],
                                                   double* __restrict__ delta, const double* __restrict__ H,
                                                   const double* __restrict__ g, const int32_t* __restrict__ active,
                                                   double* __restrict__ pose_part)
{
    double bad = 0.0;
#pragma unroll
    for (int k = 0; k < 6; ++k) {
        delta[6 * (int64_t)p + k] = d[k];
        if (!isfinite(d[k]))
            bad = 1.0;
    }
    const double* x = pose_ptr(pv, p, false);
    double out[7];
    block_plus(pv, p, x, d, out);
    double* c = pose_ptr(pv, p, true);
    double sn = 0.0, xn = 0.0;
    for (int k = 0; k < 7; ++k) {
        c[k] = out[k];
        const double df = x[k] - out[k];
        sn += df * df;
        xn += out[k] * out[k];
    }
    const double* Hp = H + 36 * (int64_t)p;
    double gd = 0.0, quad = 0.0;
    for (int a = 0; a < 6; ++a) {
        gd += d[a] * g[6 * (int64_t)p + a];
        double r = 0.0;
        for (int b = 0; b < 6; ++b)
            r += Hp[6 * a + b] * d[b];
        quad += d[a] * r;
    }
    const bool act = active[p] != 0;
    double* o = pose_part + 5 * (int64_t)p;
    o[0] = gd;
    o[1] = quad;
    o[2] = act ? sn : 0.0;
    o[3] = act ? xn : 0.0;
    o[4] = bad;
}

template <bool FUSE, bool SPARSE>
__global__ __launch_bounds__(256) void k_backsub(const LmCtl* ctl, int n_e, int e_off_pose,
                                                 const int32_t* __restrict__ pose_task,
                                                 const double* __restrict__ Z, int ldz, int n_red,
                                                 const double* __restrict__ yf, const double* __restrict__ Le,
                                                 const double* __restrict__ ze, const double* __restrict__ scale,
                                                 double* __restrict__ step_comm, double* __restrict__ part_cross,
                                                 PoseViews pv, int f_off_pose, int n_f, int nb_e,
                                                 double* __restrict__ delta, const double* __restrict__ H0,
                                                 const double* __restrict__ g0, const int64_t alt_off,
                                                 const int32_t* __restrict__ active,
                                                 double* __restrict__ pose_part,
                                                 const int32_t* __restrict__ e_start,
                                                 const int32_t* __restrict__ e_other,
                                                 const int32_t* __restrict__ row_of)
{
    if (!FUSE && blockIdx.x == 0 && threadIdx.x == 0)
        step_comm[7 * (int64_t)n_e] = (ctl->done == 2) ? 1.0 : 0.0;
    if (ctl->done)
        return;
    phase_stamp(ctl, 4);
    const bool lin_fail = ctl->lin_fail != 0;
    const double* __restrict__ H = H0 + small_sel(ctl, alt_off);
    const double* __restrict__ g = g0 + small_sel(ctl, alt_off);
    if (FUSE && (int)blockIdx.x >= nb_e) {
        const int f = ((int)blockIdx.x - nb_e) * blockDim.x + threadIdx.x;
        if (f >= n_f)
            return;
        const int p = f_off_pose + f;
        double d[6];
#pragma unroll
        for (int k = 0; k < 6; ++k)
            d[k] = lin_fail ? 0.0 : -yf[(row_of ? row_of[f] : 6 * f) + k] * scale[6 * (int64_t)p + k];
        candidate_for_pose(pv, p, d, delta, H, g, active, pose_part);
        return;
    }
    const int e = (int)blockIdx.x;
    const int lane = threadIdx.x & 63, wave = threadIdx.x >> 6;
    if (e >= n_e)
        return;
    const bool owned = pose_task[e + 1] > pose_task[e];
    if (!owned || lin_fail) {
        if (wave != 0)
            return;
        if (lane < 6)
            step_comm[6 * (int64_t)e + lane] = 0.0;
        if (lane == 0) {
            part_cross[e] = 0.0;
            if (FUSE) {
                const double d[6] = { 0.0, 0.0, 0.0, 0.0, 0.0, 0.0 };
                candidate_for_pose(pv, e_off_pose + e, d, delta, H, g, active, pose_part);
            }
        }
        return;
    }
    __shared__ double s_acc[4][6];
    double acc[6] = { 0, 0, 0, 0, 0, 0 };
    if (SPARSE) {
        const int es = e_start[e], rs = 6 * (e_start[e + 1] - es);
        const double* zp = Z + 36 * (int64_t)es;
        for (int t = (int)threadIdx.x; t < rs; t += 256) {
            const int k = t / 6, c = t - 6 * k;
            const int fo = e_other[es + k];
            const double yv = yf[(row_of ? row_of[fo] : 6 * fo) + c];
#pragma unroll
            for (int i = 0; i < 6; ++i)
                acc[i] += zp[36 * k + 6 * c + i] * yv;
        }
    } else {
        const double* zr = Z + (int64_t)(6 * e) * ldz;
        for (int c = 2 * (int)threadIdx.x; c < n_red; c += 512) {
            const double2 yv = *reinterpret_cast<const double2*>(yf + c);
#pragma unroll
            for (int i = 0; i < 6; ++i) {
                const double2 zv = *reinterpret_cast<const double2*>(zr + (int64_t)i * ldz + c);
                acc[i] += zv.x * yv.x + zv.y * yv.y;
            }
        }
    }
#pragma unroll
    for (int i = 0; i < 6; ++i) {
        const double a = wave_sum(acc[i]);
        if (lane == 0)
            s_acc[wave][i] = a;
    }
    __syncthreads();
    if (wave != 0)
        return;
    double v[6];
    double cr = 0.0;
#pragma unroll
    for (int i = 0; i < 6; ++i) {
        const double a = (s_acc[0][i] + s_acc[1][i]) + (s_acc[2][i] + s_acc[3][i]);
        v[i] = ze[6 * (int64_t)e + i] - a;
        cr += v[i] * a;
    }
    const double* L = Le + 36 * (int64_t)e;
#pragma unroll
    for (int i = 5; i >= 0; --i) {
        double s = v[i];
#pragma unroll
        for (int k = i + 1; k < 6; ++k)
            s -= L[6 * k + i] * v[k];
        v[i] = s / L[6 * i + i];
    }
    double d[6];
#pragma unroll
    for (int i = 0; i < 6; ++i)
        d[i] = -v[i] * scale[6 * (int64_t)(e_off_pose + e) + i];
    if (lane < 6) {
        double out = 0.0;
#pragma unroll
        for (int i = 0; i < 6; ++i)
            out = (lane == i) ? d[i] : out;
        step_comm[6 * (int64_t)e + lane] = out;
    }
    if (lane == 0) {
        part_cross[e] = cr;
        if (FUSE)
            candidate_for_pose(pv, e_off_pose + e, d, delta, H, g, active, pose_part);
    }
}

__global__ void k_candidate(LmCtl* ctl, PoseViews pv, int n_e, int e_off_pose, int f_off_pose,
                            const double* __restrict__ step_comm, const double* __restrict__ yf,
                            const double* __restrict__ scale, double* __restrict__ delta,
                            const double* __restrict__ H, const double* __restrict__ g,
                            const int32_t* __restrict__ active, double* __restrict__ pose_part,
                            const int32_t* __restrict__ row_of)
{
    const bool remote = step_comm[7 * (int64_t)n_e] > 0.0;
    if (remote && blockIdx.x == 0 && threadIdx.x == 0 && ctl->done != 1) {
        if (ctl->done == 0)
            atomicOr(&ctl->sync_timeout, 4);
        atomicExch(&ctl->done, 2);
    }
    if (ctl->done || remote)
        return;
    const int p = blockIdx.x * blockDim.x + threadIdx.x;
    const int n_pose = pv.n_cams + pv.n_tags;
    if (p >= n_pose)
        return;
    const bool is_e = (p >= e_off_pose) && (p < e_off_pose + n_e);
    double d[6];
    for (int k = 0; k < 6; ++k) {
        if (ctl->lin_fail)
            d[k] = 0.0;
        else if (is_e)
            d[k] = step_comm[6 * (int64_t)(p - e_off_pose) + k];
        else
            d[k] = -yf[(row_of ? row_of[p - f_off_pose] : 6 * (p - f_off_pose)) + k] * scale[6 * (int64_t)p + k];
    }
    candidate_for_pose(pv, p, d, delta, H, g, active, pose_part);
}

__global__ __launch_bounds__(256) void k_begin_loop(LmCtl* ctl, const LmCtl init, const int n_cam7, const int n_tag7,
                                                    const double* __restrict__ stage_cam,
                                                    const double* __restrict__ stage_tag, double* __restrict__ cam_qt,
                                                    double* __restrict__ tag_qt, double* __restrict__ cam_cand,
                                                    double* __restrict__ tag_cand)
{
    const int i = blockIdx.x * blockDim.x + threadIdx.x;
    if (i == 0)
        *ctl = init;
    if (i < n_cam7) {
        double v;
        if (stage_cam) {
            v = stage_cam[i];
            cam_qt[i] = v;
        } else {
            v = cam_qt[i];
        }
        cam_cand[i] = v;
    } else if (i < n_cam7 + n_tag7) {
        const int k = i - n_cam7;
        double v;
        if (stage_tag) {
            v = stage_tag[k];
            tag_qt[k] = v;
// ... 122 lines not shown
```

### visual_marker_mapping_amd/csrc/kernels_schur.hip

```cpp
#include "engine.hpp"
#include "small_solve.hpp"

namespace vmm {


__device__ __forceinline__ bool chol6(double (&A)[36])
{
    return cholesky<6>(A, A, RowMajor<6>{}, PivotOrOne{});
}

template <typename WT, bool SPARSE>
__global__ __launch_bounds__(256) void k_form_z(LmCtl* ctl, int64_t n_obs, int64_t n_pad,
                                                 const int32_t* __restrict__ own,
                                                 const int32_t* __restrict__ other,
                                                 const WT* __restrict__ W0, const WT* __restrict__ W1,
                                                 const double* __restrict__ H_E0, const double* __restrict__ g_E0,
                                                 const int64_t alt_off,
                                                 const double* __restrict__ D2,
                                                 double* __restrict__ Le, double* __restrict__ ze,
                                                 const double* __restrict__ scale, int e_off_pose,
                                                 int f_off_pose, double* __restrict__ Z, int ldz, int zcol,
                                                 const int32_t* __restrict__ e_start)
{
    if (ctl->done)
        return;
    phase_stamp(ctl, 2);
    const int64_t i = (int64_t)blockIdx.x * blockDim.x + threadIdx.x;
    if (i >= n_obs)
        return;
    const WT* __restrict__ W = ctl->w_which ? W1 : W0;
    const double* __restrict__ H_E = H_E0 + small_sel(ctl, alt_off);
    const double* __restrict__ g_E = g_E0 + small_sel(ctl, alt_off);
    const int e = own[i], f = other[i];
    const double* se = scale + 6 * (int64_t)(e_off_pose + e);
    const double* sf = scale + 6 * (int64_t)(f_off_pose + f);
    double L[36];
    {
        const double* d2 = D2 + 6 * (int64_t)(e_off_pose + e);
#pragma unroll
        for (int a = 0; a < 6; ++a) {
#pragma unroll
            for (int b = 0; b < 6; ++b)
                L[6 * a + b] = se[a] * H_E[36 * (int64_t)e + 6 * a + b] * se[b];
            L[6 * a + a] += d2[a];
        }
    }
    const bool ok = chol6(L);
    const bool first = i == 0 || own[i - 1] != e;
    if (first) {
        if (!ok)
            ctl->lin_fail = 1;
        double v[6];
#pragma unroll
        for (int a = 0; a < 6; ++a)
            v[a] = se[a] * g_E[6 * (int64_t)e + a];
        forward_substitute<6>(L, RowMajor<6>{}, [&](const int r) { return v[r]; }, [&](const int r, const double t) { v[r] = t; });
#pragma unroll
        for (int k = 0; k < 36; ++k)
            Le[36 * (int64_t)e + k] = L[k];
#pragma unroll
        for (int k = 0; k < 6; ++k) {
            ze[6 * (int64_t)e + k] = v[k];
            if (!SPARSE)
                Z[(int64_t)(6 * e + k) * ldz + zcol] = v[k];
        }
    }
    double X[36];
#pragma unroll
    for (int a = 0; a < 6; ++a)
#pragma unroll
        for (int b = 0; b < 6; ++b)
            X[6 * a + b] = se[a] * (double)W[(int64_t)(6 * a + b) * n_pad + i] * sf[b];
    forward_block<6, 6>(L, RowMajor<6>{}, X);
    int64_t rs = ldz;
    double* zrow = Z + (int64_t)(6 * e) * ldz + 6 * f;
    if (SPARSE) {
        double* zb = Z + 36 * i;
#pragma unroll
        for (int c = 0; c < 6; ++c)
#pragma unroll
            for (int r = 0; r < 6; ++r)
                zb[6 * c + r] = X[6 * r + c];
        return;
    }
#pragma unroll
    for (int r = 0; r < 6; ++r)
#pragma unroll
        for (int c = 0; c < 6; ++c)
            zrow[(int64_t)r * rs + c] = X[6 * r + c];
}


typedef double double4_t __attribute__((ext_vector_type(4)));

constexpr int kSyrkKT = kKT;
constexpr int kSyrkT = kST;
constexpr int kSyrkRow = 144;
constexpr int kSyrkTile = kSyrkT * kSyrkT;

struct SyrkPlanDev {
    int n_tiles, n_kt, n_wg;
    const int32_t* tile_bi;
    const int32_t* tile_bj;
    const int64_t* wg_u0;
    const int64_t* wg_u1;
    const int32_t* wg_seg0;
    const int32_t* tile_seg0;
    double* partials;
};

__global__ __launch_bounds__(256, 2) void k_syrk_streamk(const LmCtl* ctl, const double* __restrict__ Z, int ldz,
                                                         SyrkPlanDev pl)
{
    if (ctl && ctl->done)
        return;
    __shared__ __attribute__((aligned(16))) double As[2][kSyrkKT * kSyrkRow];
    __shared__ __attribute__((aligned(16))) double Bs[2][kSyrkKT * kSyrkRow];
    const int g = blockIdx.x;
    int64_t u = pl.wg_u0[g];
    const int64_t u_end = pl.wg_u1[g];
    int seg = pl.wg_seg0[g];
    const int tid = threadIdx.x;
    const int lane = tid & 63, wave = tid >> 6;
    const int wi = wave >> 1, wj = wave & 1;
    const int lr = tid >> 5;
    const int lc = (tid & 31) * 4;
    const int fk = lane >> 4, fi = lane & 15;
    while (u < u_end) {
        const int t = (int)(u / pl.n_kt);
        const int kt0 = (int)(u % pl.n_kt);
        const int64_t left = u_end - u;
        const int kt1 = (kt0 + left < pl.n_kt) ? (int)(kt0 + left) : pl.n_kt;
        const int I0 = pl.tile_bi[t] * kSyrkT, J0 = pl.tile_bj[t] * kSyrkT;
        const bool diag = I0 == J0;
        double4_t acc[4][4];
#pragma unroll
        for (int a = 0; a < 4; ++a)
#pragma unroll
            for (int b = 0; b < 4; ++b)
                acc[a][b] = (double4_t){ 0.0, 0.0, 0.0, 0.0 };
        double4_t va[2], vb[2];
        auto gload = [&](int kt) {
#pragma unroll
            for (int h = 0; h < 2; ++h) {
                const double* zr = Z + (int64_t)(kt * kSyrkKT + lr + 8 * h) * ldz;
                va[h] = *reinterpret_cast<const double4_t*>(zr + I0 + lc);
                vb[h] = *reinterpret_cast<const double4_t*>(zr + J0 + lc);
            }
        };
        auto lstore = [&](int buf) {
#pragma unroll
            for (int h = 0; h < 2; ++h) {
                *reinterpret_cast<double4_t*>(&As[buf][(lr + 8 * h) * kSyrkRow + lc]) = va[h];
                *reinterpret_cast<double4_t*>(&Bs[buf][(lr + 8 * h) * kSyrkRow + lc]) = vb[h];
            }
        };
        gload(kt0);
        __syncthreads();
        lstore(0);
        __syncthreads();
        const bool live = !(diag && wi == 0 && wj == 1);
        for (int kt = kt0; kt < kt1; ++kt) {
            const int buf = (kt - kt0) & 1;
            if (kt + 1 < kt1)
                gload(kt + 1);
            const double* Ap = As[buf];
            const double* Bp = Bs[buf];
            if (live) {
#pragma unroll
                for (int ks = 0; ks < kSyrkKT / 4; ++ks) {
                    const int row = (ks * 4 + fk) * kSyrkRow;
                    double a[4], b[4];
#pragma unroll
                    for (int i = 0; i < 4; ++i) {
                        a[i] = Ap[row + wi * 64 + 16 * i + fi];
                        b[i] = Bp[row + wj * 64 + 16 * i + fi];
                    }
#pragma unroll
                    for (int i = 0; i < 4; ++i)
#pragma unroll
                        for (int j = 0; j < 4; ++j)
                            acc[i][j] = __builtin_amdgcn_mfma_f64_16x16x4f64(a[i], b[j], acc[i][j], 0, 0, 0);
                }
            }
            if (kt + 1 < kt1)
                lstore(buf ^ 1);
            __syncthreads();
        }
        double* Cb = pl.partials + (size_t)seg * kSyrkTile;
        if (live) {
#pragma unroll
            for (int a = 0; a < 4; ++a)
#pragma unroll
                for (int b = 0; b < 4; ++b)
#pragma unroll
                    for (int r = 0; r < 4; ++r)
                        Cb[(wi * 64 + a * 16 + fk + 4 * r) * kSyrkT + wj * 64 + b * 16 + fi] = acc[a][b][r];
        }
        u += kt1 - kt0;
        ++seg;
    }
}

constexpr int kWideRows = 2 * kSyrkKT;
constexpr int kWideStage = kWideRows * kSyrkRow;

template <bool DIAG, int W>
struct WideTiles {
    static constexpr int NT = DIAG ? 9 : 16, NA = DIAG ? 2 : 4, NB = DIAG ? 8 - W : 4;
    static __device__ __host__ constexpr int arow(int i) { return DIAG ? (i == 0 ? W : 7 - W) : 4 * (W >> 1) + i; }
    static __device__ __host__ constexpr int bcol(int j) { return DIAG ? j : 4 * (W & 1) + j; }
    static __device__ __host__ constexpr int ai(int n) { return DIAG ? (n <= W ? 0 : 1) : (n >> 2); }
    static __device__ __host__ constexpr int bi(int n) { return DIAG ? (n <= W ? n : n - (W + 1)) : (n & 3); }
};

template <bool DIAG, int W>
__device__ __forceinline__ void syrk_wide_item(const double* __restrict__ Z, const int ldz, const int I0, const int J0,
                                               const int kt0, const int kt1, double* smem, double* __restrict__ Cb)
{
    using T = WideTiles<DIAG, W>;
    const int tid = threadIdx.x;
    const int lane = tid & 63;
    const int g = tid >> 8;
    const int t = tid & 255;
    const int lr = t >> 5;
    const int lc = (t & 31) * 4;
    const int fk = lane >> 4, fi = lane & 15;
    constexpr int kGStage = kSyrkKT * kSyrkRow;
    double* const Ag = smem + g * 4 * kGStage;
    double4_t acc[T::NT];
#pragma unroll
    for (int n = 0; n < T::NT; ++n)
        acc[n] = (double4_t){ 0.0, 0.0, 0.0, 0.0 };
// ... 69 lines not shown
    if (g == 0)
        __syncthreads();
    __syncthreads();
    constexpr int H = T::NT / 2;
    double* const X = smem + (size_t)W * 16 * 256;
#pragma unroll
    for (int n = 0; n < T::NT; ++n)
        if ((n < H) == (g == 1)) {
#pragma unroll
            for (int r = 0; r < 4; ++r)
                X[(n * 4 + r) * 64 + lane] = acc[n][r];
        }
    __syncthreads();
#pragma unroll
    for (int n = 0; n < T::NT; ++n)
        if ((n < H) == (g == 0)) {
            const int tr = T::arow(T::ai(n)), tc = T::bcol(T::bi(n));
            double v[4];
#pragma unroll
            for (int r = 0; r < 4; ++r) {
                v[r] = acc[n][r] + X[(n * 4 + r) * 64 + lane];
                Cb[(16 * tr + fk + 4 * r) * kSyrkT + 16 * tc + fi] = v[r];
            }
            if (DIAG && tr > tc && (tr >> 2) == (tc >> 2)) {
#pragma unroll
                for (int r = 0; r < 4; ++r)
                    Cb[(16 * tc + fi) * kSyrkT + 16 * tr + fk + 4 * r] = v[r];
            }
        }
}

__global__ __launch_bounds__(512, 1) void k_syrk_wide(const LmCtl* ctl, const double* __restrict__ Z, int ldz, SyrkPlanDev pl)
{
    if (ctl && ctl->done)
        return;
    __shared__ __attribute__((aligned(16))) double smem[4 * kWideStage];
    static_assert(4 * kWideStage >= 4 * 16 * 256, "the accumulator exchange must fit into the stage buffers");
    const int gidx = blockIdx.x;
    const int64_t u = pl.wg_u0[gidx], u_end = pl.wg_u1[gidx];
    if (u >= u_end)
        return;
    const int t = (int)(u / pl.n_kt);
    const int kt0 = (int)(u % pl.n_kt), kt1 = kt0 + (int)(u_end - u);
    const int I0 = pl.tile_bi[t] * kSyrkT, J0 = pl.tile_bj[t] * kSyrkT;
    double* Cb = pl.partials + (size_t)pl.wg_seg0[gidx] * kSyrkTile;
    const int w = __builtin_amdgcn_readfirstlane((int)(threadIdx.x >> 6) & 3);
    if (I0 == J0) {
        switch (w) {
        case 0: syrk_wide_item<true, 0>(Z, ldz, I0, J0, kt0, kt1, smem, Cb); break;
        case 1: syrk_wide_item<true, 1>(Z, ldz, I0, J0, kt0, kt1, smem, Cb); break;
        case 2: syrk_wide_item<true, 2>(Z, ldz, I0, J0, kt0, kt1, smem, Cb); break;
        default: syrk_wide_item<true, 3>(Z, ldz, I0, J0, kt0, kt1, smem, Cb); break;
        }
    } else {
        switch (w) {
        case 0: syrk_wide_item<false, 0>(Z, ldz, I0, J0, kt0, kt1, smem, Cb); break;
        case 1: syrk_wide_item<false, 1>(Z, ldz, I0, J0, kt0, kt1, smem, Cb); break;
        case 2: syrk_wide_item<false, 2>(Z, ldz, I0, J0, kt0, kt1, smem, Cb); break;
        default: syrk_wide_item<false, 3>(Z, ldz, I0, J0, kt0, kt1, smem, Cb); break;
        }
    }
}

struct DiagArgs {
    const double* H_F;
    const double* g_F;
    const double* scale_F;
    const double* D2_F;
    int n_red, n_pad;
    int64_t alt_off;
};

template <bool ADD_DIAG>
__global__ __launch_bounds__(256) void k_reduce_partials(const LmCtl* ctl, SyrkPlanDev pl, int ld, int n_rows,
                                                         double* __restrict__ S, DiagArgs da,
                                                         double* __restrict__ packed = nullptr)
{
    if (ctl && ctl->done)
        return;
    const int t = blockIdx.x >> 4;
    const int sub = blockIdx.x & 15;
    const int qi = sub >> 3, qj = (sub >> 2) & 1, rs = sub & 3;
    const int I0 = pl.tile_bi[t] * kSyrkT + 64 * qi, J0 = pl.tile_bj[t] * kSyrkT + 64 * qj;
    if (J0 > I0 || I0 + 16 * rs >= n_rows)
        return;
    const int s0 = pl.tile_seg0[t], s1 = pl.tile_seg0[t + 1];
    const int tr = 16 * rs + (threadIdx.x >> 5), tc = (threadIdx.x & 31) * 2;
    if (ADD_DIAG && ctl) {
        da.H_F += small_sel(ctl, da.alt_off);
        da.g_F += small_sel(ctl, da.alt_off);
    }
    double2 acc[2] = { make_double2(0.0, 0.0), make_double2(0.0, 0.0) };
    const double* p0 = pl.partials + (size_t)(64 * qi + tr) * kSyrkT + 64 * qj + tc;
#pragma unroll 4
    for (int q = s0; q < s1; ++q) {
        const double* pq = p0 + (size_t)q * kSyrkTile;
#pragma unroll
        for (int i = 0; i < 2; ++i) {
            const double2 v = *reinterpret_cast<const double2*>(pq + 8 * i * kSyrkT);
            acc[i].x += v.x;
            acc[i].y += v.y;
        }
    }
#pragma unroll
    for (int i = 0; i < 2; ++i) {
        const int row = I0 + tr + 8 * i;
        if (row >= n_rows)
            continue;
        double out[2] = { -acc[i].x, -acc[i].y };
#pragma unroll
        for (int h = 0; h < 2; ++h) {
            const int col = J0 + tc + h;
            double v = out[h];
            if (ADD_DIAG) {
                if (row == da.n_pad) {
                    if (col < da.n_red)
                        v += da.scale_F[col] * da.g_F[col];
                } else if (row < da.n_red && col <= row && (row / 6) == (col / 6)) {
                    const int f = row / 6, a = row % 6, b = col % 6;
                    v += da.scale_F[row] * da.H_F[36 * (int64_t)f + 6 * a + b] * da.scale_F[col];
                    if (a == b)
                        v += da.D2_F[row];
                } else if (row >= da.n_red && row < da.n_pad && col == row) {
                    v = 1.0;
                }
            }
            out[h] = v;
        }
        if (!ADD_DIAG && packed) {
            const int64_t base = (int64_t)row * (row + 1) / 2;
#pragma unroll
            for (int h = 0; h < 2; ++h)
                if (J0 + tc + h <= row)
                    packed[base + J0 + tc + h] = out[h];
        } else {
            *reinterpret_cast<double2*>(S + (int64_t)row * ld + J0 + tc) = make_double2(out[0], out[1]);
        }
    }
}

struct PairArgs {
    const LmCtl* ctl;
    const int32_t* item_row;
    const int32_t* item_p0;
    const int32_t* pair_start;
    const int32_t* tstart;
    const int2* terms;
    const int32_t* f_start;
    const int32_t* f2e;
    const double* Zc;
    const double* ze;
    double* S;
    int ld, n_items, n_f;
    DiagArgs da;
    int add_diag;
    const int32_t* pair_col;
    const int32_t* row_of;
};

constexpr int kPairChunk = 128;
constexpr int kPairBlk = 38;

__global__ __launch_bounds__(kPairThreads) void k_schur_pairs(PairArgs a)
{
    if (a.ctl && a.ctl->done)
        return;
    const int tid = threadIdx.x;
    const int n_red = a.da.n_red, n_pad = a.da.n_pad, ld = a.ld;
    if ((int)blockIdx.x >= a.n_items) {
        const int nb = gridDim.x - a.n_items, b = (int)blockIdx.x - a.n_items;
        for (int row = b; row <= n_pad; row += nb) {
            if (row == n_pad) {
                for (int j = n_red + tid; j < n_pad; j += kPairThreads)
                    a.S[(int64_t)n_pad * ld + j] = 0.0;
            } else if (row >= n_red) {
                for (int j = tid; j < n_pad; j += kPairThreads)
                    a.S[(int64_t)row * ld + j] = (a.add_diag && j == row) ? 1.0 : 0.0;
            } else {
                const int c0 = 6 * (row / 6) + 6, c1 = min((row / 64) * 64 + 64, n_pad);
                for (int j = c0 + tid; j < c1; j += kPairThreads)
                    a.S[(int64_t)row * ld + j] = 0.0;
            }
        }
        return;
    }
    __shared__ __attribute__((aligned(16))) double As[kPairChunk * kPairBlk];
    const int f = a.item_row[blockIdx.x];
    const int row_p0 = a.pair_start[f];
    const int sl = tid % kPairSplit;
    const int p = a.item_p0[blockIdx.x] + tid / (6 * kPairSplit), c = (tid / kPairSplit) % 6;
    const int j = p - row_p0;
    const bool expl = a.pair_col != nullptr;
    const bool valid = tid < 6 * kPairSplit * kPairsPerItem && (expl ? p < a.pair_start[f + 1] : j <= f + 1);
    const int rbase = expl ? a.row_of[f] : 6 * f;
    const int cbase = expl ? (valid ? a.pair_col[p] : 0) : 6 * j;
    const bool rhs = expl ? cbase < 0 : j == f + 1;
    int t = valid ? a.tstart[p] + sl : 0;
    const int t1 = valid ? a.tstart[p + 1] : 0;
// ... 62 lines not shown
            int2 tn[TB];
#pragma unroll
            for (int u = 0; u < TB; ++u)
                tn[u] = terms[min(t + (TB + u) * kPairSplit, t1 - 1)];
            int n_ok = 0;
#pragma unroll
            for (int u = 0; u < TB; ++u) {
                if (ok[u]) {
                    const double* __restrict__ Ap = As + kPairBlk * (tt[u].x - lo);
#pragma unroll
                    for (int r = 0; r < 6; ++r)
#pragma unroll
                        for (int q = 0; q < 6; ++q)
                            acc[q] = fma(Ap[6 * q + r], b[u][r], acc[q]);
                    ++n_ok;
                }
            }
            t += n_ok * kPairSplit;
            if (n_ok < TB)
                break;
#pragma unroll
            for (int u = 0; u < TB; ++u)
                tt[u] = tn[u];
        }
    }
#pragma unroll
    for (int m = 1; m < kPairSplit; m <<= 1)
#pragma unroll
        for (int q = 0; q < 6; ++q)
            acc[q] += __shfl_xor(acc[q], m, 64);
    if (!active || sl != 0)
        return;
    if (a.add_diag && a.ctl) {
        a.da.H_F += small_sel(a.ctl, a.da.alt_off);
        a.da.g_F += small_sel(a.ctl, a.da.alt_off);
    }
    if (rhs) {
#pragma unroll
        for (int q = 0; q < 6; ++q) {
            const int par = 6 * f + q;
            a.S[(int64_t)n_pad * ld + rbase + q] = (a.add_diag ? a.da.scale_F[par] * a.da.g_F[par] : 0.0) - acc[q];
        }
        return;
    }
    const bool diag_pair = cbase == rbase;
#pragma unroll
    for (int q = 0; q < 6; ++q) {
        const int par = 6 * f + q;
        double v = -acc[q];
        if (a.add_diag && diag_pair) {
            v += a.da.scale_F[par] * a.da.H_F[36 * (int64_t)f + 6 * q + c] * a.da.scale_F[6 * f + c];
            if (q == c)
                v += a.da.D2_F[par];
        }
        a.S[(int64_t)(rbase + q) * ld + cbase + c] = v;
    }
}

__global__ __launch_bounds__(256) void k_fill_lower(const LmCtl* ctl, double* __restrict__ S, int ld, int n_pad, int unit_diag)
{
    if (ctl && ctl->done)
        return;
    const int row = blockIdx.x;
    const int c1 = row == n_pad ? n_pad : (row / 64) * 64 + 64;
    double2* __restrict__ dst = reinterpret_cast<double2*>(S + (int64_t)row * ld);
    for (int j = threadIdx.x; 2 * j < c1; j += 256) {
        double2 v = make_double2(0.0, 0.0);
        if (unit_diag && row < n_pad) {
            if (2 * j == row)
                v.x = 1.0;
            if (2 * j + 1 == row)
                v.y = 1.0;
        }
        dst[j] = v;
    }
}


static SyrkPlanDev plan_dev(const SyrkPlan& p)
{
    SyrkPlanDev d;
    d.n_tiles = p.n_tiles;
    d.n_kt = p.n_kt;
    d.n_wg = p.n_wg;
    d.tile_bi = p.tile_bi;
    d.tile_bj = p.tile_bj;
    d.wg_u0 = p.wg_u0;
    d.wg_u1 = p.wg_u1;
    d.wg_seg0 = p.wg_seg0;
    d.tile_seg0 = p.tile_seg0;
    d.partials = p.partials;
    return d;
}

void launch_elim(Engine& e)
{
    const int e_off = e.elim_cams ? 0 : e.n_cams;
    const int f_off = e.elim_cams ? e.n_cams : 0;
    const double* H_E = e.elim_cams ? e.H_cam : e.H_tag;
    const double* g_E = e.elim_cams ? e.g_cam : e.g_tag;
    if (e.ordE.n > 0) {
        const dim3 grid((unsigned)((e.ordE.n + 255) / 256));
        double* const Zout = e.sparse_schur ? e.Zc : e.Z;
#define VMM_FORM_Z(WT, SP, W0, W1)                                                                                      \
    hipLaunchKernelGGL((k_form_z<WT, SP>), grid, dim3(256), 0, e.stream, e.ctl, e.ordE.n, e.ordE.n_pad, e.ordE.own,      \
                       e.ordE.other, (const WT*)(W0), (const WT*)(W1), H_E, g_E, e.small_alt_off, (const double*)e.D2,   \
                       e.Le, e.ze, e.scale, e_off, f_off, Zout, e.ldz, e.n_pad, (const int32_t*)e.ordE.start)
        if (e.f32_accum) {
            if (e.sparse_schur)
                VMM_FORM_Z(float, true, e.Wf, e.Wf2);
            else
                VMM_FORM_Z(float, false, e.Wf, e.Wf2);
        } else {
            if (e.sparse_schur)
                VMM_FORM_Z(double, true, e.W, e.W2);
            else
                VMM_FORM_Z(double, false, e.W, e.W2);
        }
#undef VMM_FORM_Z
    }
}

void launch_syrk_plan(hipStream_t st, const LmCtl* ctl, const double* Z, int ldz, const SyrkPlan& p)
// ... 55 lines not shown
        launch_schur_rows(e, !e.multi);
    else
        launch_syrk_plan(e.stream, e.ctl, e.Z, e.ldz, e.syrk);
}

void launch_syrk_reduced(Engine& e)
{
    launch_syrk_only(e);
    if (e.sparse_schur)
        return;
    if (e.multi) {
        DiagArgs none = {};
        if (e.syrk.n_tiles > 0)
            hipLaunchKernelGGL((k_reduce_partials<false>), dim3(16 * e.syrk.n_tiles), dim3(256), 0, e.stream, e.ctl,
                               plan_dev(e.syrk), e.ldz, e.n_pad + 1, e.S, none, e.S_packed);
        return;
    }
    const int f_off = e.elim_cams ? e.n_cams : 0;
    DiagArgs da;
    da.H_F = e.elim_cams ? e.H_tag : e.H_cam;
    da.g_F = e.elim_cams ? e.g_tag : e.g_cam;
    da.scale_F = e.scale + 6 * (size_t)f_off;
    da.D2_F = e.D2 + 6 * (size_t)f_off;
    da.n_red = e.n_red;
    da.n_pad = e.n_pad;
    da.alt_off = e.small_alt_off;
    hipLaunchKernelGGL((k_reduce_partials<true>), dim3(16 * e.syrk.n_tiles), dim3(256), 0, e.stream, e.ctl,
                       plan_dev(e.syrk), e.ldz, e.n_pad + 1, e.S, da);
}

__global__ __launch_bounds__(256) void k_pack_lower(const LmCtl* ctl, const double* __restrict__ S, int ld, int n_rows,
                                                    double* __restrict__ packed, bool unpack, double* __restrict__ Sout)
{
    if (ctl && ctl->done)
        return;
    const int r = blockIdx.x;
    if (r >= n_rows)
        return;
    const int64_t base = (int64_t)r * (r + 1) / 2;
    for (int c = threadIdx.x; c <= r; c += 256) {
        if (unpack)
            Sout[(int64_t)r * ld + c] = packed[base + c];
        else
            packed[base + c] = S[(int64_t)r * ld + c];
    }
}

__global__ __launch_bounds__(256) void k_unpack_diag(const LmCtl* ctl, const double* __restrict__ packed, int ld,
                                                     int f_off_pose, const double* __restrict__ H_F,
                                                     const double* __restrict__ g_F, const double* __restrict__ scale,
                                                     const double* __restrict__ D2, double* __restrict__ S, int n_red,
                                                     int n_pad, const int32_t* __restrict__ pose_of_row,
                                                     const int32_t* __restrict__ row_of)
{
    if (ctl && ctl->done)
        return;
    const int r = blockIdx.x;
    const int64_t base = (int64_t)r * (r + 1) / 2;
    const double* sF = scale + 6 * (int64_t)f_off_pose;
    const double* dF = D2 + 6 * (int64_t)f_off_pose;
    if (pose_of_row) {
        const int fr = r < n_pad ? pose_of_row[r] : -1;
        for (int c = threadIdx.x; c <= r; c += 256) {
            double v = packed[base + c];
            const int fc = c < n_pad ? pose_of_row[c] : -1;
            if (r == n_pad) {
                if (fc >= 0) {
                    const int k = 6 * fc + (c - row_of[fc]);
                    v += sF[k] * g_F[k];
                }
            } else if (fr >= 0) {
                if (fc == fr) {
                    const int a = r - row_of[fr], b = c - row_of[fr];
                    double add = sF[6 * fr + a] * H_F[36 * (int64_t)fr + 6 * a + b] * sF[6 * fr + b];
                    if (c == r)
                        add += dF[6 * fr + a];
                    v += add;
                }
            } else if (c == r) {
                v = 1.0;
            }
            S[(int64_t)r * ld + c] = v;
        }
        return;
    }
    for (int c = threadIdx.x; c <= r; c += 256) {
        double v = packed[base + c];
        if (r == n_pad) {
// ... 56 lines not shown
```

### visual_marker_mapping_amd/csrc/standalone.hip

```cpp
#include <string.h>

#include <algorithm>
#include <mutex>
#include <string>
#include <vector>

#include "host.hpp"

using namespace vmm;

extern "C" {

constexpr int kMaxProjectDevices = 64;

int vmm_ba_project_points(const double intr[4], const double dist[5], int64_t n, const double* points_cam,
                          double* uv, int device)
{
    if (!intr || !dist || n < 0 || (n > 0 && (!points_cam || !uv))) {
        set_error("bad argument");
        return VMM_BA_ERR_ARGUMENT;
    }
    if (n == 0)
        return VMM_BA_OK;
    HIP_TRY(hipSetDevice(device));
// ... 127 lines not shown
    e.allocs.clear();
    e.stream = nullptr;
}

int vmm_ba_dense_spd_solve(int device, int n, const double* A, const double* b, double* x, int* info)
{
    if (n <= 0 || !A || !b || !x) {
        set_error("bad argument");
        return VMM_BA_ERR_ARGUMENT;
    }
    const int n_pad = round_up(n, kNB), ld = n_pad + kNB;
    Engine e;
    int rc = make_scratch(e, device, ld);
    double *S = nullptr, *y = nullptr;
    if (!rc) rc = dev_alloc(e, &S, (size_t)ld * ld);
    if (!rc) rc = dev_alloc(e, &y, (size_t)ld);
    if (rc) {
        free_scratch(e);
        return rc;
    }
    std::vector<double> hs((size_t)ld * ld, 0.0);
    for (int i = 0; i < n; ++i)
        for (int j = 0; j <= i; ++j)
            hs[(size_t)i * ld + j] = A[(size_t)i * n + j];
    for (int i = n; i < n_pad; ++i)
        hs[(size_t)i * ld + i] = 1.0;
    for (int j = 0; j < n; ++j)
        hs[(size_t)n_pad * ld + j] = b[j];
    LmCtl c;
    hipError_t err = hipSuccess;
    for (int attempt = 0; attempt < 2 && err == hipSuccess; ++attempt) {
        memset(&c, 0, sizeof(c));
        if (attempt == 0) {
            c.spin_limit_df = e.sw.spin_df;
            c.spin_limit_chain = e.sw.spin_chain;
            c.spin_wg = e.sw.spin_wg;
        }
        err = hipMemcpyAsync(e.ctl, &c, sizeof(LmCtl), hipMemcpyHostToDevice, e.stream);
        if (err == hipSuccess)
            err = hipMemcpyAsync(S, hs.data(), sizeof(double) * hs.size(), hipMemcpyHostToDevice, e.stream);
        if (err == hipSuccess) {
            launch_cholesky_solve(e, S, n_pad, ld, y, e.ctl, attempt > 0);
            err = hipGetLastError();
        }
        if (err == hipSuccess) err = hipMemcpyAsync(x, y, sizeof(double) * n, hipMemcpyDeviceToHost, e.stream);
        if (err == hipSuccess) err = hipMemcpyAsync(&c, e.ctl, sizeof(LmCtl), hipMemcpyDeviceToHost, e.stream);
        if (err == hipSuccess) err = hipStreamSynchronize(e.stream);
        if (c.done != 2)
            break;
    }
    free_scratch(e);
    if (err != hipSuccess) {
        set_error(std::string("dense_spd_solve: ") + hipGetErrorString(err));
        return VMM_BA_ERR_HIP;
    }
    if (info)
        *info = c.lin_fail;
    return VMM_BA_OK;
}

int vmm_ba_dense_syrk(int device, int k, int n, const double* Zh, double* C)
{
    if (k <= 0 || n <= 0 || !Zh || !C) {
        set_error("bad argument");
        return VMM_BA_ERR_ARGUMENT;
    }
    const int n_pad = round_up(n, kST), ld = n_pad;
    const int n_blk = n_pad / kST;
    const int k_pad = round_up(k, kKT);
    Engine e;
    int rc = make_scratch(e, device, ld);
    double *Z = nullptr, *S = nullptr;
    SyrkPlan plan;
    if (!rc) rc = dev_alloc(e, &Z, (size_t)k_pad * ld);
    if (!rc) rc = dev_alloc(e, &S, (size_t)ld * ld);
    if (!rc) rc = make_syrk_plan(e, plan, n_blk, n_blk, k_pad);
    if (rc) {
        free_scratch(e);
        return rc;
    }
    std::vector<double> hz((size_t)k_pad * ld, 0.0);
    for (int r = 0; r < k; ++r)
        for (int c = 0; c < n; ++c)
            hz[(size_t)r * ld + c] = Zh[(size_t)r * n + c];
    hipError_t err = hipMemcpyAsync(Z, hz.data(), sizeof(double) * hz.size(), hipMemcpyHostToDevice, e.stream);
    std::vector<double> hs((size_t)ld * ld, 0.0);
    if (err == hipSuccess) {
        launch_syrk_plan(e.stream, nullptr, Z, ld, plan);
        launch_reduce_plan(e.stream, nullptr, plan, ld, n_pad, S);
        err = hipGetLastError();
// ... 16 lines not shown
```

### visual_marker_mapping_amd/csrc/vmm_ba.hip

```cpp
#include <dlfcn.h>
#include <math.h>
#include <rccl/rccl.h>
#include <stdio.h>
#include <stdlib.h>
#include <string.h>

#include <algorithm>
#include <chrono>
#include <cmath>
#include <string>
#include <functional>
#include <vector>

#include "host.hpp"

namespace vmm {

static thread_local std::string g_err;
void set_error(const std::string& s) { g_err = s; }

template <typename T>
static int upload(Engine& e, T* dst, const std::vector<T>& src)
{
    if (!src.empty())
// ... 79 lines not shown
    if ((rc = upload(e, o.start, p.start))) return rc;
    if ((rc = upload(e, o.own, p.own))) return rc;
    if ((rc = upload(e, o.other, p.other))) return rc;
    if ((rc = upload(e, o.caller, p.caller))) return rc;
    if ((rc = upload(e, o.px, p.px))) return rc;
    if ((rc = upload(e, o.tasks, p.tasks))) return rc;
    if ((rc = upload(e, o.pose_task, p.pose_task))) return rc;
    return VMM_BA_OK;
}

int make_syrk_plan(Engine& e, SyrkPlan& p, int n_row_blk, int n_col_blk, int k_pad)
{
    const SyrkSchedule s = plan_syrk(n_row_blk, n_col_blk, k_pad, e.n_cu, e.sw);
    p = SyrkPlan();
    p.n_tiles = s.n_tiles;
    p.n_kt = s.n_kt;
    p.n_wg = s.n_wg;
    p.n_segments = s.n_segments;
    p.wide = s.wide;
    int rc;
    if ((rc = dev_alloc(e, &p.tile_bi, s.tile_bi.size()))) return rc;
    if ((rc = dev_alloc(e, &p.tile_bj, s.tile_bj.size()))) return rc;
    if ((rc = dev_alloc(e, &p.wg_u0, s.wg_u0.size()))) return rc;
    if ((rc = dev_alloc(e, &p.wg_u1, s.wg_u1.size()))) return rc;
    if ((rc = dev_alloc(e, &p.wg_seg0, s.wg_seg0.size()))) return rc;
    if ((rc = dev_alloc(e, &p.tile_seg0, s.tile_seg0.size()))) return rc;
    if ((rc = dev_alloc(e, &p.partials, (size_t)std::max(s.n_segments, 1) * kST * kST, false))) return rc;
    if ((rc = upload(e, p.tile_bi, s.tile_bi))) return rc;
    if ((rc = upload(e, p.tile_bj, s.tile_bj))) return rc;
    if ((rc = upload(e, p.wg_u0, s.wg_u0))) return rc;
    if ((rc = upload(e, p.wg_u1, s.wg_u1))) return rc;
    if ((rc = upload(e, p.wg_seg0, s.wg_seg0))) return rc;
    if ((rc = upload(e, p.tile_seg0, s.tile_seg0))) return rc;
    HIP_TRY(hipStreamSynchronize(e.stream));
    return VMM_BA_OK;
}
int setup_lookahead(Engine& e, int n_blk_max, int ld)
{
    (void)n_blk_max;
    for (int i = 0; i < 4; ++i)
        e.P4[i] = e.P + (size_t)i * kNB * ld;
    return VMM_BA_OK;
}

static void points_to_tag(const double* pts, double* qt)
{
    double ex[3], ey[3], ez[3];
    for (int a = 0; a < 3; ++a) {
        ex[a] = pts[3 + a] - pts[a];
        ey[a] = pts[9 + a] - pts[a];
    }
    auto normalise = [](double* v) {
        const double n = sqrt(v[0] * v[0] + v[1] * v[1] + v[2] * v[2]);
        if (n > 0.0)
            for (int a = 0; a < 3; ++a)
                v[a] /= n;
    };
    normalise(ex);
    normalise(ey);
    ez[0] = ex[1] * ey[2] - ex[2] * ey[1];
    ez[1] = ex[2] * ey[0] - ex[0] * ey[2];
    ez[2] = ex[0] * ey[1] - ex[1] * ey[0];
    normalise(ez);
    ey[0] = ez[1] * ex[2] - ez[2] * ex[1];
    ey[1] = ez[2] * ex[0] - ez[0] * ex[2];
    ey[2] = ez[0] * ex[1] - ez[1] * ex[0];
// ... 271 lines not shown
                         enqueue_segment(e, o, seg);
                         if (capture_alive(e))
                             *where = kSegName[seg];
                         return VMM_BA_OK;
                     }))) {
                    drop_graphs(e);
                    return rc;
                }
        }
        e.graph_robustify = o.robustify;
        e.graph_huber_a = o.huber_a;
    }
    Range r("vmm_ba lm_iteration");
    if (one_graph) {
        HIP_TRY(hipGraphLaunch(e.iter_graph, e.stream));
        e.last_passes = e.sw.graph_passes;
        return VMM_BA_OK;
    }
    int rc;
    for (int seg = 0; seg < kNumSeg; ++seg) {
        HIP_TRY(hipGraphLaunch(e.iter_graph_seg[seg], e.stream));
        if ((rc = allreduce_after(e, seg)))
            return rc;
    }
    return VMM_BA_OK;
}

static int recover_sync_timeout(Engine& e, const vmm_ba_options& o)
{
    LmCtl& c = *e.ctl_host;
    c.num_sync_timeouts++;
    c.sync_kernels |= c.sync_timeout;
    c.sync_timeout = 0;
    c.lin_fail = 0;
    c.done = 0;
    if (e.sw.spin_once)
        c.spin_limit_df = c.spin_limit_chain = 0;
    HIP_TRY(hipMemcpyAsync(e.ctl, e.ctl_host, sizeof(LmCtl), hipMemcpyHostToDevice, e.stream));
    Range r("vmm_ba sync time-out recovery");
    int rc;
    for (int seg = 1; seg < kNumSeg; ++seg) {
        if (seg == kNumSeg - 1 && !e.multi)
            break;
        enqueue_segment(e, o, seg, true);
        if (e.multi && (rc = allreduce_after(e, seg)))
            return rc;
    }
    HIP_TRY(hipGetLastError());
    return VMM_BA_OK;
}

int begin_lm_loop(Engine& e, const vmm_ba_options& o, int trace_capacity)
{
    init_ctl(e, *e.ctl_host, o, trace_capacity);
    launch_begin_loop(e, *e.ctl_host);
    HIP_TRY(hipGetLastError());
    if (e.dirty_cam || e.dirty_tag) {
        HIP_TRY(hipEventRecord(e.pose_ev, e.stream));
        e.pose_ev_pending = true;
        e.dirty_cam = e.dirty_tag = false;
    }
    return VMM_BA_OK;
}

int flush_state(Engine& e)
{
    if (!e.dirty_cam && !e.dirty_tag)
        return VMM_BA_OK;
    if (e.dirty_cam)
        HIP_TRY(hipMemcpyAsync(e.cam_qt, e.pose_stage, sizeof(double) * 7 * e.n_cams, hipMemcpyHostToDevice, e.stream));
    if (e.dirty_tag)
        HIP_TRY(hipMemcpyAsync(e.tag_qt, e.pose_stage + (size_t)7 * e.n_cams, sizeof(double) * 7 * e.n_tags,
                               hipMemcpyHostToDevice, e.stream));
    HIP_TRY(hipEventRecord(e.pose_ev, e.stream));
    e.pose_ev_pending = true;
    e.dirty_cam = e.dirty_tag = false;
    return VMM_BA_OK;
}

void init_ctl(Engine& e, LmCtl& c, const vmm_ba_options& o, int trace_capacity)
{
    memset(&c, 0, sizeof(c));
    c.spin_limit_df = e.sw.spin_df;
    c.spin_limit_chain = e.sw.spin_chain;
    c.spin_wg = e.sw.spin_wg;
    c.max_num_iterations = o.max_num_iterations;
    c.robustify = o.robustify;
    c.jacobi_scaling = o.jacobi_scaling;
    c.max_invalid = o.max_num_consecutive_invalid_steps;
    c.huber_a = o.huber_a;
    c.function_tolerance = o.function_tolerance;
    c.gradient_tolerance = o.gradient_tolerance;
    c.parameter_tolerance = o.parameter_tolerance;
    c.max_radius = o.max_trust_region_radius;
    c.min_radius = o.min_trust_region_radius;
    c.min_relative_decrease = o.min_relative_decrease;
    c.min_lm_diagonal = o.min_lm_diagonal;
    c.max_lm_diagonal = o.max_lm_diagonal;
    c.radius = o.initial_trust_region_radius;
    c.decrease_factor = 2.0;
    c.first_eval = 1;
    c.termination = VMM_BA_NO_CONVERGENCE;
    c.trace_capacity = trace_capacity;
}


static int validate_problem(const vmm_ba_problem* p, const vmm_ba_create_options& co)
{
    if (p->n_cams <= 0 || p->n_tags <= 0 || p->n_obs < 0 || !p->cam_qt || !p->tag_qt || !p->tag_wh
        || (p->n_obs > 0 && (!p->obs_cam || !p->obs_tag || !p->obs_px))) {
        set_error("problem needs >= 1 camera, >= 1 tag and non-null arrays");
        return VMM_BA_ERR_ARGUMENT;
    }
    if (p->n_obs >= (int64_t)1 << 31) {
        set_error("n_obs must fit in 31 bits");
        return VMM_BA_ERR_ARGUMENT;
    }
    for (int64_t i = 0; i < p->n_obs; ++i)
        if (p->obs_cam[i] < 0 || p->obs_cam[i] >= p->n_cams || p->obs_tag[i] < 0 || p->obs_tag[i] >= p->n_tags) {
            set_error("observation " + std::to_string(i) + " references a camera or tag index out of range");
            return VMM_BA_ERR_ARGUMENT;
        }
    if (p->fixed_tag >= p->n_tags) {
        set_error("fixed_tag out of range");
        return VMM_BA_ERR_ARGUMENT;
    }
    if (co.landmarks != VMM_BA_LANDMARK_TAG_POSES && co.landmarks != VMM_BA_LANDMARK_POINTS) {
        set_error("create_options.landmarks must be VMM_BA_LANDMARK_TAG_POSES or VMM_BA_LANDMARK_POINTS");
        return VMM_BA_ERR_ARGUMENT;
    }
    if (co.landmarks == VMM_BA_LANDMARK_POINTS && co.precision != VMM_BA_PRECISION_F64) {
        set_error("point landmarks run in f64 only");
        return VMM_BA_ERR_ARGUMENT;
    }
// ... 103 lines not shown
    if (e.fused_eval) {
        if ((rc = dev_alloc(e, &e.pair_obs, P.pair_obs.size()))) return rc;
        if ((rc = dev_alloc(e, &e.fused_e_list, P.fused_e_list.size()))) return rc;
        if ((rc = dev_alloc(e, &e.fused_e_part0, P.fused_e_part0.size()))) return rc;
        if ((rc = dev_alloc(e, &e.fused_pose_task, P.fused_pose_task.size()))) return rc;
        if ((rc = dev_alloc(e, &e.fused_partE, (size_t)std::max(P.fused_slots, 1) * kPart))) return rc;
        if ((rc = dev_alloc(e, &e.fused_partF, (size_t)e.fused_groups * 28 * e.fused_f_pad))) return rc;
        if ((rc = upload(e, e.pair_obs, P.pair_obs))) return rc;
        if ((rc = upload(e, e.fused_e_list, P.fused_e_list))) return rc;
        if ((rc = upload(e, e.fused_e_part0, P.fused_e_part0))) return rc;
        if ((rc = upload(e, e.fused_pose_task, P.fused_pose_task))) return rc;
    }

    e.small_count = (size_t)42 * n_pose + 2;
    if ((rc = dev_alloc(e, &e.small, e.small_count))) return rc;
    e.H_cam = e.small;
    e.H_tag = e.H_cam + (size_t)36 * e.n_cams;
    e.g_cam = e.H_tag + (size_t)36 * e.n_tags;
    e.g_tag = e.g_cam + (size_t)6 * e.n_cams;
    e.cost_slot = e.g_tag + (size_t)6 * e.n_tags;
    if ((rc = dev_alloc(e, &e.small_stage, e.small_count + (size_t)e.n_e))) return rc;
    e.ev_pose_cost = e.small_stage + e.small_count;
    e.small_alt_off = e.multi ? 0 : (int64_t)(e.small_stage - e.small);
    e.ev_H_cam = e.small_stage;
    e.ev_H_tag = e.ev_H_cam + (size_t)36 * e.n_cams;
    e.ev_g_cam = e.ev_H_tag + (size_t)36 * e.n_tags;
    e.ev_g_tag = e.ev_g_cam + (size_t)6 * e.n_cams;
    e.ev_cost = e.ev_g_tag + (size_t)6 * e.n_tags;
    if ((rc = dev_alloc(e, &e.obs_mask, (size_t)std::max<int64_t>(e.n_obs, 1), false))) return rc;
    if (hipMemsetAsync(e.obs_mask, 1, (size_t)std::max<int64_t>(e.n_obs, 1), e.stream) != hipSuccess) {
        set_error("hipMemsetAsync(obs_mask) failed");
        return VMM_BA_ERR_HIP;
    }
    if ((rc = dev_alloc(e, &e.pose_const, (size_t)n_pose))) return rc;
    if ((rc = upload_pose_const(e, nullptr, nullptr))) return rc;
    const size_t n_stat = (size_t)e.ordE.n_tasks + (size_t)e.ordF.n_tasks + 1;
    if ((rc = dev_alloc(e, &e.stats_part, n_stat))) return rc;
    if ((rc = dev_alloc(e, &e.stats_cnt, n_stat))) return rc;
    if ((rc = dev_alloc(e, &e.stats_pose, (size_t)2 * n_pose))) return rc;
    if (e.f32_accum) {
        if ((rc = dev_alloc(e, &e.Wf, (size_t)36 * e.ordE.n_pad))) return rc;
        if ((rc = dev_alloc(e, &e.Wf2, (size_t)36 * e.ordE.n_pad))) return rc;
    } else {
        if ((rc = dev_alloc(e, &e.W, (size_t)36 * e.ordE.n_pad))) return rc;
        if ((rc = dev_alloc(e, &e.W2, (size_t)36 * e.ordE.n_pad))) return rc;
    }
    if ((rc = dev_alloc(e, &e.scale, (size_t)6 * n_pose))) return rc;
    if ((rc = dev_alloc(e, &e.diag, (size_t)6 * n_pose))) return rc;
    if ((rc = dev_alloc(e, &e.D2, (size_t)6 * n_pose))) return rc;
    if ((rc = dev_alloc(e, &e.delta, (size_t)6 * n_pose))) return rc;
    if ((rc = dev_alloc(e, &e.active, (size_t)n_pose))) return rc;

    if ((rc = dev_alloc(e, &e.Le, (size_t)36 * e.n_e))) return rc;
    if ((rc = dev_alloc(e, &e.ze, (size_t)6 * e.n_e))) return rc;
    if (e.sparse_schur) {
        if ((rc = dev_alloc(e, &e.Zc, (size_t)36 * std::max<int64_t>(e.n_obs, 1)))) return rc;
        if ((rc = dev_alloc(e, &e.f2e, P.f2e.size()))) return rc;
        if ((rc = dev_alloc(e, &e.pair_start, P.pair_start.size()))) return rc;
        if ((rc = dev_alloc(e, &e.pair_tstart, P.pair_tstart.size()))) return rc;
        if ((rc = dev_alloc(e, &e.pair_terms, P.pair_terms.size()))) return rc;
        if ((rc = dev_alloc(e, &e.row_items, P.row_items.size()))) return rc;
        if ((rc = upload(e, e.f2e, P.f2e))) return rc;
        if ((rc = upload(e, e.pair_start, P.pair_start))) return rc;
        if ((rc = upload(e, e.pair_tstart, P.pair_tstart))) return rc;
        if ((rc = upload(e, e.pair_terms, P.pair_terms))) return rc;
        if ((rc = upload(e, e.row_items, P.row_items))) return rc;
// ... 352 lines not shown
    const auto t0 = std::chrono::steady_clock::now();
    vmm_ba_iteration* user_trace = s->trace;
    const int user_cap = s->trace ? s->trace_capacity : 0;
    memset(s, 0, sizeof(*s));
    s->trace = user_trace;
    s->trace_capacity = user_cap;

    const int need_cap = std::max(user_cap, 1);
    int rc;
    if (need_cap > e.trace_capacity) {
        drop_graphs(e);
        if (e.trace) {
            HIP_TRY(hipStreamSynchronize(e.stream));
            e.allocs.erase(std::remove(e.allocs.begin(), e.allocs.end(), (void*)e.trace), e.allocs.end());
            (void)hipFree(e.trace);
            e.trace = nullptr;
            e.trace_capacity = 0;
        }
        if ((rc = dev_alloc(e, &e.trace, (size_t)need_cap, false))) return rc;
        e.trace_capacity = need_cap;
    }
    if ((rc = begin_lm_loop(e, o, user_cap))) return rc;

    const int poll = std::max(1, o.poll_interval);
    const int64_t max_steps = (int64_t)o.max_num_iterations + 2;
    int64_t enq = 0;
    for (;;) {
        for (int k = 0; k < poll && enq < max_steps; ++k) {
            if ((rc = run_iteration(e, o))) return rc;
            enq += e.last_passes;
        }
        HIP_TRY(hipMemcpyAsync(e.ctl_host, e.ctl, sizeof(LmCtl), hipMemcpyDeviceToHost, e.stream));
        HIP_TRY(hipStreamSynchronize(e.stream));
        if (e.ctl_host->done == 2) {
            if (e.ctl_host->num_sync_timeouts >= 1000) {
                set_error("the one-launch factorisation gave up waiting in 1000 passes of one solve (kernels: "
                          + std::to_string(e.ctl_host->sync_kernels | e.ctl_host->sync_timeout) + ")");
                return VMM_BA_ERR_HIP;
            }
            if ((rc = recover_sync_timeout(e, o))) return rc;
            enq = e.ctl_host->num_lm_iterations;
            continue;
        }
        if (e.ctl_host->done)
            break;
        if (enq >= max_steps) {
            set_error("LM loop did not terminate within max_num_iterations + 2 passes");
            return VMM_BA_ERR_STATE;
        }
    }
    const LmCtl& c = *e.ctl_host;
    s->termination_type = c.termination;
    s->iterations = c.records;
    s->num_successful_steps = c.num_successful;
    s->num_unsuccessful_steps = c.num_unsuccessful;
    s->num_lm_iterations = c.num_lm_iterations;
    s->num_jacobian_evals = c.num_jac_evals;
    s->num_cost_evals = c.num_cost_evals;
    s->elimination = e.elim_cams ? VMM_BA_ELIM_CAMERAS : VMM_BA_ELIM_TAGS;
    s->initial_cost = c.initial_cost;
    s->final_cost = c.x_cost;
    s->time_eval_s = 1e-8 * (double)c.phase_ticks[0];
    s->time_control_s = 1e-8 * (double)c.phase_ticks[1];
    s->time_eliminate_s = 1e-8 * (double)c.phase_ticks[2];
    s->time_factor_solve_s = 1e-8 * (double)c.phase_ticks[3];
    s->time_step_s = 1e-8 * (double)c.phase_ticks[4];
    s->num_sync_timeouts = c.num_sync_timeouts;
    s->sync_timeout_kernels = c.sync_kernels;
    s->block_sparse = e.sparse_schur ? 1 : 0;
    s->tree_ordering = (e.sparse_schur && !e.h_row_of.empty()) ? (int32_t)e.nd_node_first_blk.size() : 0;
    if (user_trace && user_cap > 0) {
        const int n = std::min(c.records, user_cap);
        if (n > 0) {
            HIP_TRY(hipMemcpyAsync(user_trace, e.trace, sizeof(vmm_ba_iteration) * n, hipMemcpyDeviceToHost, e.stream));
            HIP_TRY(hipStreamSynchronize(e.stream));
        }
    }
// ... 8 lines not shown
        return VMM_BA_ERR_ARGUMENT;
    }
    Engine& e = *reinterpret_cast<Engine*>(h);
    HIP_TRY(hipSetDevice(e.device));
    int rc;
    if ((rc = flush_state(e))) return rc;
    launch_cost(e, e.cam_qt, e.tag_qt, false, robustify, huber_a, e.cost_comm);
    if ((rc = do_allreduce(e, e.cost_comm, 1))) return rc;
    HIP_TRY(hipMemcpyAsync(cost, e.cost_comm, sizeof(double), hipMemcpyDeviceToHost, e.stream));
    HIP_TRY(hipStreamSynchronize(e.stream));
    return VMM_BA_OK;
}

int vmm_ba_set_observation_mask(vmm_ba_handle h, const uint8_t* mask)
{
    if (!h) {
        set_error("null handle");
        return VMM_BA_ERR_ARGUMENT;
    }
    Engine& e = *reinterpret_cast<Engine*>(h);
    HIP_TRY(hipSetDevice(e.device));
    if (e.n_obs == 0)
        return VMM_BA_OK;
    if (mask) {
        std::vector<uint8_t> m((size_t)e.n_obs);
        const int rep = e.points ? 2 : 1;
        for (int64_t i = 0; i < e.n_obs; ++i)
            m[(size_t)i] = mask[i / rep] ? 1 : 0;
        HIP_TRY(hipMemcpyAsync(e.obs_mask, m.data(), m.size(), hipMemcpyHostToDevice, e.stream));
        HIP_TRY(hipStreamSynchronize(e.stream));
    } else {
        HIP_TRY(hipMemsetAsync(e.obs_mask, 1, (size_t)e.n_obs, e.stream));
    }
    return VMM_BA_OK;
}

int vmm_ba_set_constant_poses(vmm_ba_handle h, const uint8_t* cam_const, const uint8_t* tag_const)
{
    if (!h) {
        set_error("null handle");
        return VMM_BA_ERR_ARGUMENT;
    }
    Engine& e = *reinterpret_cast<Engine*>(h);
    HIP_TRY(hipSetDevice(e.device));
    return upload_pose_const(e, cam_const, tag_const);
}

int vmm_ba_reprojection_stats(vmm_ba_handle h, double* per_cam_mean, double* per_tag_mean, double* avg,
                              double* per_corner)
{
    if (!h) {
        set_error("null handle");
        return VMM_BA_ERR_ARGUMENT;
    }
    Engine& e = *reinterpret_cast<Engine*>(h);
    if (e.points) {
        set_error("reprojection_stats works on tag poses: read them with vmm_ba_get_state and use a tag-pose handle");
        return VMM_BA_ERR_STATE;
    }
    HIP_TRY(hipSetDevice(e.device));
    int rc;
    if ((rc = flush_state(e))) return rc;
    const int n_pose = e.n_cams + e.n_tags;
    if (per_corner && e.n_obs > 0 && !e.stats_corner && (rc = dev_alloc(e, &e.stats_corner, (size_t)8 * e.n_obs, false)))
        return rc;
    launch_stats(e, (per_corner && e.n_obs > 0) ? e.stats_corner : nullptr);
// ... 75 lines not shown
```

Baseline: 2483 LM iterations/s.

## Pack LM control header into one vector load and presort observation mask

Moves the frequently read control flags (done, lin_fail, w_which, spin limits) into a 32-byte aligned header that every kernel fetches with a single vector load, issued early alongside other loads so their latency overlaps. The observation mask is permuted into task order once, whenever it changes, which removes the per-residual indirect caller lookup in the eval kernels. Per-workgroup and per-tile SYRK metadata are precomputed on the host into packed records to replace several scattered index loads. This adds small device buffers and a mask-sort kernel that has to be rerun every time the mask is updated.

```diff
diff --git a/visual_marker_mapping_amd/csrc/chol_common.hpp b/visual_marker_mapping_amd/csrc/chol_common.hpp
--- a/visual_marker_mapping_amd/csrc/chol_common.hpp
+++ b/visual_marker_mapping_amd/csrc/chol_common.hpp
@@ -75,7 +75,7 @@
 __device__ __forceinline__ void raise_sync_timeout(LmCtl* ctl, int bit)
 {
     atomicOr(&ctl->sync_timeout, bit);
-    atomicExch(&ctl->done, 2);
+    atomicExch(&ctl->head.done, 2);
 }
 
 __device__ __forceinline__ void chol_inverse_lds(const double* L, const double* di, double* __restrict__ Linvk)
diff --git a/visual_marker_mapping_amd/csrc/covariance.hip b/visual_marker_mapping_amd/csrc/covariance.hip
--- a/visual_marker_mapping_amd/csrc/covariance.hip
+++ b/visual_marker_mapping_amd/csrc/covariance.hip
@@ -53,7 +53,7 @@
             err = hipMemcpyAsync(e.ctl_host, e.ctl, sizeof(LmCtl), hipMemcpyDeviceToHost, e.stream);
         if (err == hipSuccess)
             err = hipStreamSynchronize(e.stream);
-        if (err != hipSuccess || e.ctl_host->done != 2)
+        if (err != hipSuccess || e.ctl_host->head.done != 2)
             break;
     }
     return err;
@@ -88,7 +88,7 @@
     const hipError_t err = cov_factor_and(e, robustify, huber_a, upload ? upload() : hipSuccess, tail);
     if (err != hipSuccess)
         return hip_failure(who, "", err);
-    if (e.ctl_host->lin_fail) {
+    if (e.ctl_host->head.lin_fail) {
         set_error(std::string(who) + ": " + matrix + " is not positive definite (rank-deficient Jacobian)");
         return VMM_BA_ERR_NUMERIC;
     }
diff --git a/visual_marker_mapping_amd/csrc/diagnostics.hip b/visual_marker_mapping_amd/csrc/diagnostics.hip
--- a/visual_marker_mapping_amd/csrc/diagnostics.hip
+++ b/visual_marker_mapping_amd/csrc/diagnostics.hip
@@ -117,8 +117,8 @@
     };
     auto nop = [] {};
     HIP_TRY(hipMemcpy(e.ctl_host, e.ctl, sizeof(LmCtl), hipMemcpyDeviceToHost));
-    e.ctl_host->done = 0;
-    e.ctl_host->lin_fail = 0;
+    e.ctl_host->head.done = 0;
+    e.ctl_host->head.lin_fail = 0;
     HIP_TRY(hipMemcpy(e.ctl, e.ctl_host, sizeof(LmCtl), hipMemcpyHostToDevice));
     if ((rc = timed([&] { launch_eval_passes(e, o.robustify, o.huber_a, false); }, nop, &out->eval_elim_ms, 8))) return rc;
     out->eval_keep_ms = 0.0;
@@ -137,7 +137,7 @@
     if (e.sw.debug) {
         HIP_TRY(hipMemcpy(e.ctl_host, e.ctl, sizeof(LmCtl), hipMemcpyDeviceToHost));
         fprintf(stderr, "[vmm_ba debug] after kernel timing: done=%d lin_fail=%d termination=%d iteration=%d\n",
-                e.ctl_host->done, e.ctl_host->lin_fail, e.ctl_host->termination, e.ctl_host->iteration);
+                e.ctl_host->head.done, e.ctl_host->head.lin_fail, e.ctl_host->termination, e.ctl_host->iteration);
     }
     if ((rc = restore_raw())) return rc;
     if ((rc = begin_lm_loop(e, ot, 0))) return rc;
@@ -229,8 +229,8 @@
     auto reset_flags = [&]() -> hipError_t {
         hipError_t r = hipMemcpy(e.ctl_host, e.ctl, sizeof(LmCtl), hipMemcpyDeviceToHost);
         if (r != hipSuccess) return r;
-        e.ctl_host->done = 0;
-        e.ctl_host->lin_fail = 0;
+        e.ctl_host->head.done = 0;
+        e.ctl_host->head.lin_fail = 0;
         e.ctl_host->sync_timeout = 0;
         return hipMemcpy(e.ctl, e.ctl_host, sizeof(LmCtl), hipMemcpyHostToDevice);
     };
diff --git a/visual_marker_mapping_amd/csrc/engine.hpp b/visual_marker_mapping_amd/csrc/engine.hpp
--- a/visual_marker_mapping_amd/csrc/engine.hpp
+++ b/visual_marker_mapping_amd/csrc/engine.hpp
@@ -1,5 +1,6 @@
 #pragma once
 #include <hip/hip_runtime.h>
+#include <stddef.h>
 #include <stdint.h>
 
 #include <string>
@@ -19,6 +20,7 @@
     int32_t* own = nullptr;
     int32_t* other = nullptr;
     int32_t* caller = nullptr;
+    uint8_t* mask = nullptr;
     double* px = nullptr;
     Task* tasks = nullptr;
     int32_t n_tasks = 0;
@@ -27,7 +29,19 @@
     int32_t* start = nullptr;
 };
 
+struct alignas(32) LmHead {
+    int32_t done;
+    int32_t w_which;
+    int32_t lin_fail;
+    int32_t first_eval;
+    uint32_t spin_limit_df, spin_limit_chain;
+    int32_t spin_wg;
+    int32_t reserved;
+};
+static_assert(sizeof(LmHead) == 32, "LmHead is one 32-byte scalar load");
+
 struct LmCtl {
+    LmHead head;
     int32_t max_num_iterations, robustify, jacobi_scaling, max_invalid;
     double huber_a, function_tolerance, gradient_tolerance, parameter_tolerance;
     double max_radius, min_radius, min_relative_decrease, min_lm_diagonal, max_lm_diagonal;
@@ -35,24 +49,46 @@
     int32_t reuse_diagonal, num_invalid;
     double x_cost, cand_cost, model_cost_change, x_norm, initial_cost;
     int32_t iteration;
-    int32_t first_eval;
-    int32_t done, termination;
-    int32_t lin_fail;
+    int32_t termination;
     int32_t sync_timeout;
     int32_t num_sync_timeouts;
     int32_t sync_kernels;
-    uint32_t spin_limit_df, spin_limit_chain;
-    int32_t spin_wg;
     int32_t records;
     int32_t num_successful, num_unsuccessful, num_lm_iterations, num_jac_evals, num_cost_evals;
     int32_t trace_capacity;
-    int32_t w_which;
     vmm_ba_iteration cur;
     unsigned long long stamp[6];
     unsigned long long phase_ticks[5];
 };
 
-__device__ __forceinline__ int64_t small_sel(const LmCtl* ctl, const int64_t alt_off) { return ctl->w_which ? alt_off : 0; }
+static_assert(offsetof(LmCtl, head) == 0, "the header is the front of the control block");
+
+__device__ __forceinline__ LmHead lm_head(const LmCtl* ctl)
+{
+    typedef int32_t head_words __attribute__((ext_vector_type(8)));
+    head_words v = { 0, 0, 0, 0, 0, 0, 0, 0 };
+    if (ctl)
+        v = *reinterpret_cast<const head_words*>(&ctl->head);
+    LmHead h;
+    h.done = v[0];
+    h.w_which = v[1];
+    h.lin_fail = v[2];
+    h.first_eval = v[3];
+    h.spin_limit_df = (uint32_t)v[4];
+    h.spin_limit_chain = (uint32_t)v[5];
+    h.spin_wg = v[6];
+    h.reserved = v[7];
+    return h;
+}
+
+__device__ __forceinline__ void loads_requested() { asm volatile("" ::: "memory"); }
+
+__device__ __forceinline__ int64_t small_sel(const LmHead& h, const int64_t alt_off) { return h.w_which ? alt_off : 0; }
+
+__device__ __forceinline__ unsigned spin_limit_of(const LmHead& h, const unsigned limit, const unsigned dflt)
+{
+    return (limit && (h.spin_wg < 0 || h.spin_wg == (int)blockIdx.x)) ? limit : dflt;
+}
 
 __device__ __forceinline__ void phase_stamp(const LmCtl* ctl, int slot)
 {
@@ -60,10 +96,23 @@
         const_cast<LmCtl*>(ctl)->stamp[slot] = __builtin_amdgcn_s_memrealtime();
 }
 
+struct alignas(32) SyrkWgRec {
+    int32_t I0, J0;
+    int32_t kt0, kt1;
+    int32_t seg;
+    int32_t diag;
+    int32_t tile, units;
+};
+struct alignas(16) SyrkTileRec {
+    int32_t I0, J0, s0, s1;
+};
+
 struct SyrkPlan {
     int n_tiles = 0, n_kt = 0, n_wg = 0, n_segments = 0;
     int32_t *tile_bi = nullptr, *tile_bj = nullptr, *wg_seg0 = nullptr, *tile_seg0 = nullptr;
     int64_t *wg_u0 = nullptr, *wg_u1 = nullptr;
+    SyrkWgRec* wg_rec = nullptr;
+    SyrkTileRec* tile_rec = nullptr;
     double* partials = nullptr;
     bool wide = false;
 };
@@ -279,6 +328,7 @@
 void launch_stats(Engine& e, double* per_corner_dev);
 void launch_project(hipStream_t st, const Intrinsics& K, int64_t n, const double* pc, double* uv);
 void launch_sum(Engine& e, bool guard, const double* in, int n, double* out);
+void launch_sort_mask(Engine& e);
 void launch_elim(Engine& e);
 void launch_schur_rows(Engine& e, bool add_diag);
 void launch_syrk_only(Engine& e);
diff --git a/visual_marker_mapping_amd/csrc/kernels_backsolve.hip b/visual_marker_mapping_amd/csrc/kernels_backsolve.hip
--- a/visual_marker_mapping_amd/csrc/kernels_backsolve.hip
+++ b/visual_marker_mapping_amd/csrc/kernels_backsolve.hip
@@ -7,7 +7,8 @@
                                                         const double* __restrict__ dinv,
                                                         const double* __restrict__ Ld)
 {
-    if (ctl->done || ctl->lin_fail)
+    const LmHead head = lm_head(ctl);
+    if (head.done || head.lin_fail)
         return;
     __shared__ double red[4][64];
     __shared__ double L[64 * kLd];
@@ -101,7 +102,8 @@
                                                      const double* __restrict__ Linv,
                                                      const unsigned long long* __restrict__ nz, unsigned* n_done)
 {
-    if (ctl->done || ctl->lin_fail) {
+    const LmHead head = lm_head(ctl);
+    if (head.done || head.lin_fail) {
         if constexpr (TREE) {
             if (threadIdx.x == 0)
                 chain_block_done(n_done, n_blk, epoch_word, *epoch_word + 1u);
@@ -111,8 +113,7 @@
         }
         return;
     }
-    const unsigned spin_limit = (ctl->spin_limit_chain && (ctl->spin_wg < 0 || ctl->spin_wg == (int)blockIdx.x))
-                                    ? ctl->spin_limit_chain : kSpinLimit;
+    const unsigned spin_limit = spin_limit_of(head, head.spin_limit_chain, kSpinLimit);
     __shared__ double L[64 * kLd];
     __shared__ double Li[64 * kLd];
     __shared__ double red[4][64];
diff --git a/visual_marker_mapping_amd/csrc/kernels_chol_dataflow.hip b/visual_marker_mapping_amd/csrc/kernels_chol_dataflow.hip
--- a/visual_marker_mapping_amd/csrc/kernels_chol_dataflow.hip
+++ b/visual_marker_mapping_amd/csrc/kernels_chol_dataflow.hip
@@ -875,7 +875,7 @@
 }
 
 template <bool HAS_T, bool TREE, int MODE>
-__device__ __forceinline__ void role(const DfArgs& a, const int j, const int R, double* smem)
+__device__ __forceinline__ void role(const DfArgs& a, const int j, const int R, double* smem, const unsigned epoch0)
 {
     constexpr bool BULK = (MODE & 1) != 0, HELP = (MODE & 2) != 0;
     const int tid = threadIdx.x;
@@ -886,7 +886,7 @@
     const int n_blk = a.n_blk, ld = a.ld, n_pad = a.n_pad;
     if (TREE && HAS_T && R < n_blk && !nz_bit(a.nz, R, j))
         return;
-    const unsigned epoch = *a.epoch_word + 1u;
+    const unsigned epoch = epoch0 + 1u;
     Lds m;
     m.RA = smem;
     m.Pd = m.RA + 64 * kLdT;
@@ -968,7 +968,7 @@
             __hip_atomic_store(a.done + sm.index(j, R), epoch, __ATOMIC_RELEASE, __HIP_MEMORY_SCOPE_AGENT);
     }
     if (j == n_blk - 1 && tid == 0 && !ok)
-        a.ctl->lin_fail = 1;
+        a.ctl->head.lin_fail = 1;
     report_give_up(a, epoch, s_timeout);
 }
 
@@ -977,20 +977,22 @@
 template <bool TREE, int MODE>
 __device__ __forceinline__ void chol_dataflow_body(DfArgs& a)
 {
-    if (a.ctl->done)
+    const LmHead head = lm_head(a.ctl);
+    const unsigned epoch0 = *a.epoch_word;
+    loads_requested();
+    if (head.done)
         return;
-    a.spin_limit = (a.ctl->spin_limit_df && (a.ctl->spin_wg < 0 || a.ctl->spin_wg == (int)blockIdx.x)) ? a.ctl->spin_limit_df
-                                                                                                          : kDfSpinDefault;
+    a.spin_limit = spin_limit_of(head, head.spin_limit_df, kDfSpinDefault);
     phase_stamp(a.ctl, 3);
-    if (a.ctl->lin_fail)
+    if (head.lin_fail)
         return;
     __shared__ __attribute__((aligned(16))) double smem[kDfSmem];
     if (TREE) {
         const int j = a.wg[2 * (int)blockIdx.x], R = a.wg[2 * (int)blockIdx.x + 1];
         if (R > j)
-            df2::role<true, TREE, MODE>(a, j, R, smem);
+            df2::role<true, TREE, MODE>(a, j, R, smem, epoch0);
         else
-            df2::role<false, TREE, MODE>(a, j, j, smem);
+            df2::role<false, TREE, MODE>(a, j, j, smem, epoch0);
         return;
     }
     int b = (int)blockIdx.x, j = 0;
@@ -1003,9 +1005,9 @@
     if (j >= a.n_blk)
         return;
     if (b < a.n_blk - j)
-        df2::role<true, TREE, MODE>(a, j, j + 1 + b, smem);
+        df2::role<true, TREE, MODE>(a, j, j + 1 + b, smem, epoch0);
     else
-        df2::role<false, TREE, MODE>(a, j, j, smem);
+        df2::role<false, TREE, MODE>(a, j, j, smem, epoch0);
 }
 
 __global__ __launch_bounds__(256) void k_chol_dataflow(DfArgs a)
diff --git a/visual_marker_mapping_amd/csrc/kernels_chol_step.hip b/visual_marker_mapping_amd/csrc/kernels_chol_step.hip
--- a/visual_marker_mapping_amd/csrc/kernels_chol_step.hip
+++ b/visual_marker_mapping_amd/csrc/kernels_chol_step.hip
@@ -202,7 +202,7 @@
     STAMP(2);
     if (!HAS_T) {
         if (tid == 0 && !ok)
-            ctl->lin_fail = 1;
+            ctl->head.lin_fail = 1;
         if (tid < 64)
             dinv[K0 + tid] = invd[tid];
         for (int idx = tid; idx < 64 * 64; idx += 256) {
@@ -663,11 +663,12 @@
                                                    const double* __restrict__ PB, int c0, int t0, int t1, int n_upd_wg,
                                                    unsigned* tile_ctr)
 {
-    if (ctl->done)
+    const LmHead head = lm_head(ctl);
+    if (head.done)
         return;
     if (k == 0)
         phase_stamp(ctl, 3);
-    if (ctl->lin_fail)
+    if (head.lin_fail)
         return;
     if (blockIdx.x == 0 && threadIdx.x == 0)
         tile_ctr[(k + 1) & 1] = 0u;
@@ -693,7 +694,8 @@
 __global__ __launch_bounds__(256) void k_chol_inverse(const LmCtl* ctl, const double* __restrict__ Ld,
                                                       const double* __restrict__ dinv, double* __restrict__ Linv, int k)
 {
-    if (ctl->done || ctl->lin_fail)
+    const LmHead head = lm_head(ctl);
+    if (head.done || head.lin_fail)
         return;
     __shared__ __attribute__((aligned(16))) double smem[64 * kLd + 64];
     chol_inverse_wg(Ld + (int64_t)k * 4096, dinv + k * kNB, Linv + (int64_t)k * 4096, smem);
diff --git a/visual_marker_mapping_amd/csrc/kernels_eval.hip b/visual_marker_mapping_amd/csrc/kernels_eval.hip
--- a/visual_marker_mapping_amd/csrc/kernels_eval.hip
+++ b/visual_marker_mapping_amd/csrc/kernels_eval.hip
@@ -21,6 +21,7 @@
     void* W_alt;
     const int32_t* caller;
     const uint8_t* mask;
+    const uint8_t* mask_sorted;
     const LmCtl* ctl;
 };
 
@@ -30,14 +31,24 @@
 __device__ __forceinline__ void eval_body(const EvalArgs& a, const int wave)
 {
     const int lane = threadIdx.x & 63;
-    if (wave >= a.n_tasks)
-        return;
-    const Task t = a.tasks[wave];
+    const LmHead head = lm_head(a.ctl);
+    const bool have = wave < a.n_tasks;
+    Task t = {};
+    if (have)
+        t = a.tasks[wave];
+    loads_requested();
+    if (head.done)
+        return;
+    if (a.ctl)
+        phase_stamp(a.ctl, 0);
+    if (!have)
+        return;
     const int64_t i = (int64_t)t.begin + lane;
     const bool valid = i < t.end;
     const int64_t is = valid ? i : t.begin;
     const int o = a.other[is];
-    AT* __restrict__ const Wout = static_cast<AT*>((WRITE_W && a.W_alt && a.ctl && a.ctl->w_which == 0) ? a.W_alt : a.W);
+    const uint8_t mask_is = a.mask_sorted[is];
+    AT* __restrict__ const Wout = static_cast<AT*>((WRITE_W && a.W_alt && a.ctl && head.w_which == 0) ? a.W_alt : a.W);
 
     const int tag_idx = OWN_IS_CAM ? o : t.pose;
     const int cam_idx = OWN_IS_CAM ? t.pose : o;
@@ -56,7 +67,7 @@
     }
     const double hw = POINTS ? 0.0 : 0.5 * a.tag_wh[2 * tag_idx], hh = POINTS ? 0.0 : 0.5 * a.tag_wh[2 * tag_idx + 1];
     const bool cam_c = a.cam_const[cam_idx] != 0, tag_c = a.tag_const[tag_idx] != 0;
-    const bool on = valid && a.mask[a.caller[is]];
+    const bool on = valid && mask_is;
 
     AT H[21];
     double g[6], cost = 0.0;
@@ -163,11 +174,6 @@
 template <bool E_IS_CAM, typename AT = double, bool POINTS = false>
 __global__ __launch_bounds__(256) __attribute__((amdgpu_waves_per_eu(2, 2))) void k_eval_both(const EvalArgs aE, const EvalArgs aF, const int nb_e)
 {
-    if (aE.ctl) {
-        if (aE.ctl->done)
-            return;
-        phase_stamp(aE.ctl, 0);
-    }
     if ((int)blockIdx.x < nb_e)
         eval_body<E_IS_CAM, true, AT, POINTS>(aE, (int)((blockIdx.x * blockDim.x + threadIdx.x) >> 6));
     else
@@ -187,11 +193,11 @@
 __global__ __launch_bounds__(256) __attribute__((amdgpu_waves_per_eu(1, 1)))
 void k_eval_fused(const EvalArgs a, const FusedArgs fa)
 {
-    if (a.ctl) {
-        if (a.ctl->done)
-            return;
+    const LmHead head = lm_head(a.ctl);
+    if (head.done)
+        return;
+    if (a.ctl)
         phase_stamp(a.ctl, 0);
-    }
     const int lane = threadIdx.x & 63;
     const int wave = (int)((blockIdx.x * blockDim.x + threadIdx.x) >> 6);
     if (wave >= fa.n_groups * fa.n_chunks)
@@ -200,7 +206,7 @@
     const int f = 64 * c + lane;
     const bool fvalid = f < fa.n_f;
     const int fs = fvalid ? f : fa.n_f - 1;
-    AT* __restrict__ const Wout = static_cast<AT*>((a.W_alt && a.ctl && a.ctl->w_which == 0) ? a.W_alt : a.W);
+    AT* __restrict__ const Wout = static_cast<AT*>((a.W_alt && a.ctl && head.w_which == 0) ? a.W_alt : a.W);
     const double* keptq = a.other_pose + 7 * (int64_t)fs;
     Rigid kept;
     double pt[6];
@@ -400,12 +406,7 @@
 
 __global__ void k_reduce_pose(const LmCtl* ctl, const ReduceArgs rE, const ReduceArgs rF, const int64_t alt_off)
 {
-    int64_t off = 0;
-    if (ctl) {
-        if (ctl->done)
-            return;
-        off = ctl->w_which ? 0 : alt_off;
-    }
+    const LmHead head = lm_head(ctl);
     int tid = blockIdx.x * blockDim.x + threadIdx.x;
     const bool first = tid < 32 * rE.n_pose;
     if (!first)
@@ -414,14 +415,30 @@
     const int n_pose = r.n_pose;
     const int32_t* __restrict__ pose_task = r.pose_task;
     const double* __restrict__ part = r.part;
+    const int p = tid >> 5, k = tid & 31;
+    const bool mine = p < n_pose && k < 28;
+    int t0 = 0, t1 = r.n_fixed;
+    if (mine && pose_task) {
+        t0 = pose_task[p];
+        t1 = pose_task[p + 1];
+    }
+    loads_requested();
+    if (head.done)
+        return;
+    const int64_t off = (ctl && !head.w_which) ? alt_off : 0;
     double* __restrict__ Hout = r.Hout + off;
     double* __restrict__ gout = r.gout + off;
     double* __restrict__ pose_cost = r.pose_cost;
-    const int p = tid >> 5, k = tid & 31;
-    if (p >= n_pose || k >= 28)
-        return;
-    const int t0 = pose_task ? pose_task[p] : 0, t1 = pose_task ? pose_task[p + 1] : r.n_fixed;
+    if (!mine)
+        return;
     const double* __restrict__ pp = part + (int64_t)k * r.sk + (int64_t)p * r.sp;
+    double x[7] = { 0.0, 0.0, 0.0, 0.0, 0.0, 0.0, 0.0 };
+    if (r.gm_out && k == 21) {
+#pragma unroll
+        for (int j = 0; j < 7; ++j)
+            x[j] = r.pose7[7 * (int64_t)p + j];
+    }
+    loads_requested();
     double s0 = 0.0, s1 = 0.0, s2 = 0.0, s3 = 0.0;
     int t = t0;
     for (; t + 3 < t1; t += 4) {
@@ -452,7 +469,6 @@
         for (int j = 0; j < 6; ++j)
             ng[j] = -__shfl(s, 21 + j, 32);
         if (k == 21) {
-            const double* x = r.pose7 + 7 * (int64_t)p;
             double xp[7], gm = 0.0;
             if (r.euclid) {
 #pragma unroll
@@ -473,7 +489,7 @@
 __global__ __launch_bounds__(256) void k_sum(const LmCtl* ctl, const double* __restrict__ in, int n, int stride,
                                              double* __restrict__ out)
 {
-    if (ctl && ctl->done)
+    if (lm_head(ctl).done)
         return;
     __shared__ double sh[256];
     double s = 0.0;
@@ -511,7 +527,7 @@
 template <bool OWN_IS_CAM, bool POINTS = false>
 __global__ __launch_bounds__(256) void k_cost(const CostArgs a)
 {
-    if (a.ctl && a.ctl->done)
+    if (lm_head(a.ctl).done)
         return;
     const int wave = (int)((blockIdx.x * blockDim.x + threadIdx.x) >> 6);
     const int lane = threadIdx.x & 63;
@@ -683,6 +699,7 @@
     a.W_alt = (lm && W) ? (e.f32_accum ? (void*)e.Wf2 : (void*)e.W2) : nullptr;
     a.caller = ord.caller;
     a.mask = e.obs_mask;
+    a.mask_sorted = ord.mask;
     a.ctl = e.ctl;
     return a;
 }
@@ -792,6 +809,22 @@
                            e.cost_slot);
 }
 
+__global__ __launch_bounds__(256) void k_sort_mask(int64_t n, const int32_t* __restrict__ caller,
+                                                   const uint8_t* __restrict__ mask, uint8_t* __restrict__ out)
+{
+    const int64_t i = (int64_t)blockIdx.x * blockDim.x + threadIdx.x;
+    if (i < n)
+        out[i] = mask[caller[i]];
+}
+
+void launch_sort_mask(Engine& e)
+{
+    for (const ObsOrder* o : { &e.ordE, &e.ordF })
+        if (o->n > 0)
+            hipLaunchKernelGGL(k_sort_mask, dim3((unsigned)((o->n + 255) / 256)), dim3(256), 0, e.stream, o->n,
+                               (const int32_t*)o->caller, (const uint8_t*)e.obs_mask, o->mask);
+}
+
 void launch_sum(Engine& e, bool guard, const double* in, int n, double* out)
 {
     hipLaunchKernelGGL(k_sum, dim3(1), dim3(256), 0, e.stream, guard ? e.ctl : (const LmCtl*)nullptr, in, n, 1, out);
@@ -873,6 +906,7 @@
 {
     hipFuncAttributes at;
     int bad = 0;
+    bad += hipFuncGetAttributes(&at, reinterpret_cast<const void*>(&k_sort_mask)) != hipSuccess;
     bad += hipFuncGetAttributes(&at, reinterpret_cast<const void*>(&k_eval_both<true, double>)) != hipSuccess;
     bad += hipFuncGetAttributes(&at, reinterpret_cast<const void*>(&k_eval_both<false, double>)) != hipSuccess;
     bad += hipFuncGetAttributes(&at, reinterpret_cast<const void*>(&k_eval_both<true, float>)) != hipSuccess;
diff --git a/visual_marker_mapping_amd/csrc/kernels_lm.hip b/visual_marker_mapping_amd/csrc/kernels_lm.hip
--- a/visual_marker_mapping_amd/csrc/kernels_lm.hip
+++ b/visual_marker_mapping_amd/csrc/kernels_lm.hip
@@ -115,35 +115,58 @@
                                                  double* __restrict__ diag, double* __restrict__ D2,
                                                  vmm_ba_iteration* __restrict__ trace)
 {
-    if (ctl->done)
+    const LmHead head = lm_head(ctl);
+    const bool jacobi = ctl->jacobi_scaling != 0;
+    const int tid = threadIdx.x;
+    const int n_pose = pv.n_cams + pv.n_tags;
+    const int n_tan = 6 * n_pose;
+    const int n_cam7 = 7 * pv.n_cams, n_qt = 7 * n_pose;
+    const bool first = head.first_eval != 0;
+    const int which = head.w_which;
+    const bool staged = src != dst;
+    const double* __restrict__ nb = staged ? src : dst + (which ? 0 : alt_off);
+    const double* __restrict__ Hn = nb + (H0 - dst);
+    const double* __restrict__ gn = nb + (g0 - dst);
+    struct PoseIn {
+        double o[5], gm;
+        int act;
+    };
+    auto request = [&](const int p, PoseIn& in) {
+        const double* o = dz.pose_part + 5 * (int64_t)p;
+#pragma unroll
+        for (int k = 0; k < 5; ++k)
+            in.o[k] = o[k];
+        in.gm = dz.pose_gm ? dz.pose_gm[p] : 0.0;
+        in.act = active[p];
+    };
+    PoseIn in = {};
+    if (tid < n_pose)
+        request(tid, in);
+    const double pre_cross = tid < dz.n_cross ? dz.cross_parts[tid] : 0.0;
+    const double pre_cost = tid < dz.n_cost ? dz.cost_parts[tid] : 0.0;
+    constexpr int kCtlWords = (int)(sizeof(LmCtl) / sizeof(uint32_t));
+    static_assert(kCtlWords <= 1024 && sizeof(LmCtl) % sizeof(uint32_t) == 0, "one word per thread");
+    const uint32_t ctl_word = tid < kCtlWords ? reinterpret_cast<const uint32_t*>(ctl)[tid] : 0u;
+    loads_requested();
+    if (head.done)
         return;
     const unsigned long long t_begin = __builtin_amdgcn_s_memrealtime();
     CTL_RT(0);
     __shared__ double sh[256];
     __shared__ int s_stop, s_reuse, s_accept, s_moved;
     __shared__ double s_radius, s_lo, s_hi;
-    const int tid = threadIdx.x;
-    const int n_pose = pv.n_cams + pv.n_tags;
-    const int n_tan = 6 * n_pose;
-    const bool first = ctl->first_eval != 0;
-    const bool jacobi = ctl->jacobi_scaling != 0;
-    const int which = ctl->w_which;
-    const bool staged = src != dst;
-    const double* __restrict__ nb = staged ? src : dst + (which ? 0 : alt_off);
-    const double* __restrict__ Hn = nb + (H0 - dst);
-    const double* __restrict__ gn = nb + (g0 - dst);
     __shared__ LmCtl s_c;
-    if (tid == 0)
-        s_c = *ctl;
     double gd = 0.0, quad = 0.0, sn = 0.0, xn = 0.0, bad = 0.0, cross = 0.0, ccost = 0.0, xn0 = 0.0, gm = 0.0;
     for (int p = tid; p < n_pose; p += (int)blockDim.x) {
+        if (p != tid)
+            request(p, in);
+        loads_requested();
         if (!first) {
-            const double* o = dz.pose_part + 5 * (int64_t)p;
-            gd += o[0];
-            quad += o[1];
-            sn += o[2];
-            xn += o[3];
-            bad = fmax(bad, o[4]);
+            gd += in.o[0];
+            quad += in.o[1];
+            sn += in.o[2];
+            xn += in.o[3];
+            bad = fmax(bad, in.o[4]);
         }
         const double* Hp = Hn + 36 * (int64_t)p;
         int act;
@@ -153,7 +176,7 @@
             for (int k = 0; k < 6; ++k)
                 scale[6 * (int64_t)p + k] = jacobi ? 1.0 / (1.0 + sqrt(Hp[7 * k])) : 1.0;
         } else {
-            act = active[p];
+            act = in.act;
         }
         if (act) {
             const double* x = pose_ptr(pv, p, true);
@@ -161,7 +184,7 @@
                 for (int k = 0; k < 7; ++k)
                     xn0 += x[k] * x[k];
             if (dz.pose_gm) {
-                gm = fmax(gm, dz.pose_gm[p]);
+                gm = fmax(gm, in.gm);
             } else {
                 double ng[6], xp[7];
                 for (int k = 0; k < 6; ++k)
@@ -172,11 +195,18 @@
             }
         }
     }
-    if (!first)
-        for (int i = tid; i < dz.n_cross; i += (int)blockDim.x)
+    if (!first) {
+        if (tid < dz.n_cross)
+            cross += pre_cross;
+        for (int i = tid + (int)blockDim.x; i < dz.n_cross; i += (int)blockDim.x)
             cross += dz.cross_parts[i];
-    for (int i = tid; i < dz.n_cost; i += (int)blockDim.x)
+    }
+    if (tid < dz.n_cost)
+        ccost += pre_cost;
+    for (int i = tid + (int)blockDim.x; i < dz.n_cost; i += (int)blockDim.x)
         ccost += dz.cost_parts[i];
+    if (tid < kCtlWords)
+        reinterpret_cast<uint32_t*>(&s_c)[tid] = ctl_word;
     CTL_RT(1);
     double red[8] = { gd, quad, sn, xn, cross, ccost, xn0, 0.0 };
     double redm[2] = { bad, gm };
@@ -196,10 +226,10 @@
         auto span = [](unsigned long long a, unsigned long long b) { return b > a ? b - a : 0ull; };
         int accept = 0;
         if (first) {
-            c.w_which = which ^ 1;
+            c.head.w_which = which ^ 1;
             c.phase_ticks[0] += span(c.stamp[0], t_begin);
         } else {
-            const bool lin_fail = c.lin_fail != 0 || bad != 0.0;
+            const bool lin_fail = c.head.lin_fail != 0 || bad != 0.0;
             const double mcc = lin_fail ? 0.0 : -gd - 0.5 * (quad + 2.0 * cross);
             c.model_cost_change = mcc;
             c.cur.model_cost_change = mcc;
@@ -208,7 +238,7 @@
             if (!valid) {
                 c.num_invalid++;
                 if (c.num_invalid >= c.max_invalid) {
-                    c.done = 1;
+                    c.head.done = 1;
                     c.termination = VMM_BA_FAILURE;
                 } else {
                     c.radius = c.radius / c.decrease_factor;
@@ -229,11 +259,11 @@
                 const double x_cost = c.x_cost;
                 const double cost_change = x_cost - cand;
                 if (step_norm <= c.parameter_tolerance * (c.x_norm + c.parameter_tolerance)) {
-                    c.done = 1;
+                    c.head.done = 1;
                     c.termination = VMM_BA_CONVERGENCE;
                 } else if (fabs(cost_change) <= c.function_tolerance * x_cost) {
                     c.cur.cost_change = cost_change;
-                    c.done = 1;
+                    c.head.done = 1;
                     c.termination = VMM_BA_CONVERGENCE;
                 } else {
                     c.cur.cost_change = cost_change;
@@ -248,7 +278,7 @@
                         c.radius = r > c.max_radius ? c.max_radius : r;
                         c.decrease_factor = 2.0;
                         c.reuse_diagonal = 0;
-                        c.w_which = which ^ 1;
+                        c.head.w_which = which ^ 1;
                         c.x_norm = sqrt(xn);
                         c.cur.step_is_successful = 1;
                     } else {
@@ -268,12 +298,12 @@
         }
         c.stamp[5] = t_begin;
         const int moved = (first || accept) ? 1 : 0;
-        if (!c.done && moved) {
+        if (!c.head.done && moved) {
             const double cst = ccost;
             c.x_cost = cst;
             c.num_jac_evals++;
             if (first) {
-                c.first_eval = 0;
+                c.head.first_eval = 0;
                 c.initial_cost = cst;
                 c.x_norm = sqrt(xn0);
                 c.cur.iteration = 0;
@@ -283,11 +313,11 @@
             c.cur.cost = cst;
             c.cur.gradient_max_norm = gm;
             if (!isfinite(cst)) {
-                c.done = 1;
+                c.head.done = 1;
                 c.termination = VMM_BA_FAILURE;
             }
         }
-        int stop = c.done;
+        int stop = c.head.done;
         if (!stop) {
             vmm_ba_iteration cur = c.cur;
             cur.trust_region_radius = c.radius;
@@ -309,7 +339,7 @@
                 c.termination = VMM_BA_CONVERGENCE;
             }
             if (stop) {
-                c.done = 1;
+                c.head.done = 1;
             } else {
                 vmm_ba_iteration z;
                 z.iteration = cur.iteration + 1;
@@ -325,7 +355,7 @@
                 z.model_cost_change = 0.0;
                 c.cur = z;
                 c.iteration = z.iteration;
-                c.lin_fail = 0;
+                c.head.lin_fail = 0;
                 c.num_lm_iterations++;
             }
         }
@@ -341,27 +371,68 @@
         else
             c.phase_ticks[1] += span(t_begin, __builtin_amdgcn_s_memrealtime());
         CTL_RT(3);
-        *ctl = c;
-        CTL_RT(4);
     }
     __syncthreads();
+    if (tid < kCtlWords)
+        reinterpret_cast<uint32_t*>(ctl)[tid] = reinterpret_cast<const uint32_t*>(&s_c)[tid];
+    CTL_RT(4);
     CTL_RT(5);
-    if (s_accept) {
-        for (int i = tid; i < 7 * pv.n_cams; i += (int)blockDim.x)
-            pv.cam_qt[i] = pv.cam_cand[i];
-        for (int i = tid; i < 7 * pv.n_tags; i += (int)blockDim.x)
-            pv.tag_qt[i] = pv.tag_cand[i];
+    constexpr int kCtlRounds = 5;
+    const bool stop = s_stop != 0, accept = s_accept != 0, reuse = s_reuse != 0;
+    const double* __restrict__ Hx = s_moved ? Hn : H0 + (which ? alt_off : 0);
+    double pre_qt[kCtlRounds], pre_a[kCtlRounds], pre_b[kCtlRounds];
+#pragma unroll
+    for (int r = 0; r < kCtlRounds; ++r) {
+        const int i = tid + r * (int)blockDim.x;
+        pre_qt[r] = pre_a[r] = pre_b[r] = 0.0;
+        if (accept && i < n_qt)
+            pre_qt[r] = i < n_cam7 ? pv.cam_cand[i] : pv.tag_cand[i - n_cam7];
+        if (!stop && i < n_tan) {
+            if (reuse) {
+                pre_a[r] = diag[i];
+            } else {
+                pre_a[r] = scale[i];
+                pre_b[r] = Hx[36 * (int64_t)(i / 6) + 7 * (i % 6)];
+            }
+        }
+    }
+    loads_requested();
+    if (accept) {
+#pragma unroll
+        for (int r = 0; r < kCtlRounds; ++r) {
+            const int i = tid + r * (int)blockDim.x;
+            if (i < n_qt)
+                (i < n_cam7 ? pv.cam_qt[i] : pv.tag_qt[i - n_cam7]) = pre_qt[r];
+        }
+        for (int i = tid + kCtlRounds * (int)blockDim.x; i < n_qt; i += (int)blockDim.x)
+            (i < n_cam7 ? pv.cam_qt[i] : pv.tag_qt[i - n_cam7]) = i < n_cam7 ? pv.cam_cand[i] : pv.tag_cand[i - n_cam7];
     }
     if (staged && s_moved)
         for (size_t i = tid; i < small_count; i += blockDim.x)
             dst[i] = src[i];
-    if (s_stop)
-        return;
-    const double* __restrict__ Hx = s_moved ? Hn : H0 + (which ? alt_off : 0);
+    if (stop)
+        return;
     const double lo = s_lo, hi = s_hi;
-    for (int q = tid; q < n_tan; q += (int)blockDim.x) {
+#pragma unroll
+    for (int r = 0; r < kCtlRounds; ++r) {
+        const int q = tid + r * (int)blockDim.x;
+        if (q >= n_tan)
+            continue;
         double d;
-        if (!s_reuse) {
+        if (!reuse) {
+            const double sc = pre_a[r];
+            d = sc * sc * pre_b[r];
+            d = fmin(fmax(d, lo), hi);
+            diag[q] = d;
+        } else {
+            d = pre_a[r];
+        }
+        const double lm = sqrt(d / s_radius);
+        D2[q] = lm * lm;
+    }
+    for (int q = tid + kCtlRounds * (int)blockDim.x; q < n_tan; q += (int)blockDim.x) {
+        double d;
+        if (!reuse) {
             const int p = q / 6, k = q % 6;
             const double sc = scale[q];
             d = sc * sc * Hx[36 * (int64_t)p + 7 * k];
@@ -377,9 +448,8 @@
 }
 
 __device__ __forceinline__ void candidate_for_pose(const PoseViews& pv, const int p, const double (&d)[6],
-                                                   double* __restrict__ delta, const double* __restrict__ H,
-                                                   const double* __restrict__ g, const int32_t* __restrict__ active,
-                                                   double* __restrict__ pose_part)
+                                                   double* __restrict__ delta, const double* x, const double* Hp,
+                                                   const double* gp, const int32_t* actp, double* __restrict__ pose_part)
 {
     double bad = 0.0;
 #pragma unroll
@@ -388,7 +458,6 @@
         if (!isfinite(d[k]))
             bad = 1.0;
     }
-    const double* x = pose_ptr(pv, p, false);
     double out[7];
     block_plus(pv, p, x, d, out);
     double* c = pose_ptr(pv, p, true);
@@ -399,22 +468,30 @@
         sn += df * df;
         xn += out[k] * out[k];
     }
-    const double* Hp = H + 36 * (int64_t)p;
     double gd = 0.0, quad = 0.0;
     for (int a = 0; a < 6; ++a) {
-        gd += d[a] * g[6 * (int64_t)p + a];
+        gd += d[a] * gp[a];
         double r = 0.0;
         for (int b = 0; b < 6; ++b)
             r += Hp[6 * a + b] * d[b];
         quad += d[a] * r;
     }
-    const bool act = active[p] != 0;
+    const bool act = *actp != 0;
     double* o = pose_part + 5 * (int64_t)p;
     o[0] = gd;
     o[1] = quad;
     o[2] = act ? sn : 0.0;
     o[3] = act ? xn : 0.0;
     o[4] = bad;
+}
+
+__device__ __forceinline__ void candidate_for_pose(const PoseViews& pv, const int p, const double (&d)[6],
+                                                   double* __restrict__ delta, const double* __restrict__ H,
+                                                   const double* __restrict__ g, const int32_t* __restrict__ active,
+                                                   double* __restrict__ pose_part)
+{
+    candidate_for_pose(pv, p, d, delta, pose_ptr(pv, p, false), H + 36 * (int64_t)p, g + 6 * (int64_t)p, active + p,
+                       pose_part);
 }
 
 template <bool FUSE, bool SPARSE>
@@ -433,31 +510,75 @@
                                                  const int32_t* __restrict__ e_other,
                                                  const int32_t* __restrict__ row_of)
 {
+    const LmHead head = lm_head(ctl);
+    const bool kept_wg = FUSE && (int)blockIdx.x >= nb_e;
+    const int e = (int)blockIdx.x;
+    const int lane = threadIdx.x & 63, wave = threadIdx.x >> 6;
+    const int f = ((int)blockIdx.x - nb_e) * blockDim.x + threadIdx.x;
+    int t0 = 0, t1 = 0, frow = 0;
+    if (kept_wg) {
+        if (f < n_f)
+            frow = row_of ? row_of[f] : 6 * f;
+    } else if (e < n_e) {
+        t0 = pose_task[e];
+        t1 = pose_task[e + 1];
+    }
+    loads_requested();
     if (!FUSE && blockIdx.x == 0 && threadIdx.x == 0)
-        step_comm[7 * (int64_t)n_e] = (ctl->done == 2) ? 1.0 : 0.0;
-    if (ctl->done)
+        step_comm[7 * (int64_t)n_e] = (head.done == 2) ? 1.0 : 0.0;
+    if (head.done)
         return;
     phase_stamp(ctl, 4);
-    const bool lin_fail = ctl->lin_fail != 0;
-    const double* __restrict__ H = H0 + small_sel(ctl, alt_off);
-    const double* __restrict__ g = g0 + small_sel(ctl, alt_off);
-    if (FUSE && (int)blockIdx.x >= nb_e) {
-        const int f = ((int)blockIdx.x - nb_e) * blockDim.x + threadIdx.x;
+    const bool lin_fail = head.lin_fail != 0;
+    const double* __restrict__ H = H0 + small_sel(head, alt_off);
+    const double* __restrict__ g = g0 + small_sel(head, alt_off);
+    if (kept_wg) {
         if (f >= n_f)
             return;
         const int p = f_off_pose + f;
+        double xv[7], Hv[36], gv[6];
+        const double* x = pose_ptr(pv, p, false);
+#pragma unroll
+        for (int k = 0; k < 7; ++k)
+            xv[k] = x[k];
+#pragma unroll
+        for (int k = 0; k < 36; ++k)
+            Hv[k] = H[36 * (int64_t)p + k];
+#pragma unroll
+        for (int k = 0; k < 6; ++k)
+            gv[k] = g[6 * (int64_t)p + k];
+        const int32_t act = active[p];
         double d[6];
 #pragma unroll
         for (int k = 0; k < 6; ++k)
-            d[k] = lin_fail ? 0.0 : -yf[(row_of ? row_of[f] : 6 * f) + k] * scale[6 * (int64_t)p + k];
-        candidate_for_pose(pv, p, d, delta, H, g, active, pose_part);
-        return;
-    }
-    const int e = (int)blockIdx.x;
-    const int lane = threadIdx.x & 63, wave = threadIdx.x >> 6;
+            d[k] = lin_fail ? 0.0 : -yf[frow + k] * scale[6 * (int64_t)p + k];
+        loads_requested();
+        candidate_for_pose(pv, p, d, delta, xv, Hv, gv, &act, pose_part);
+        return;
+    }
     if (e >= n_e)
         return;
-    const bool owned = pose_task[e + 1] > pose_task[e];
+    const bool owned = t1 > t0;
+    constexpr int kBsL = 0, kBsZe = 36, kBsSc = 42, kBsH = 48, kBsG = 84, kBsX = 90, kBsN = 97;
+    __shared__ double s_pre[kBsN];
+    __shared__ int32_t s_act;
+    double pre0 = 0.0, pre1 = 0.0;
+    int32_t pre_act = 0;
+    if (wave == 0 && owned && !lin_fail) {
+        const int p = e_off_pose + e;
+        auto slot = [&](const int s) -> const double* {
+            return s < kBsZe  ? Le + 36 * (int64_t)e + (s - kBsL)
+                   : s < kBsSc ? ze + 6 * (int64_t)e + (s - kBsZe)
+                   : s < kBsH  ? scale + 6 * (int64_t)p + (s - kBsSc)
+                   : s < kBsG  ? H + 36 * (int64_t)p + (s - kBsH)
+                   : s < kBsX  ? g + 6 * (int64_t)p + (s - kBsG)
+                               : pose_ptr(pv, p, false) + (s - kBsX);
+        };
+        pre0 = *slot(lane);
+        pre1 = *slot(min(lane + 64, kBsN - 1));
+        pre_act = active[p];
+        loads_requested();
+    }
     if (!owned || lin_fail) {
         if (wave != 0)
             return;
@@ -502,6 +623,13 @@
         if (lane == 0)
             s_acc[wave][i] = a;
     }
+    if (wave == 0) {
+        s_pre[lane] = pre0;
+        if (lane + 64 < kBsN)
+            s_pre[lane + 64] = pre1;
+        if (lane == 0)
+            s_act = pre_act;
+    }
     __syncthreads();
     if (wave != 0)
         return;
@@ -510,10 +638,10 @@
 #pragma unroll
     for (int i = 0; i < 6; ++i) {
         const double a = (s_acc[0][i] + s_acc[1][i]) + (s_acc[2][i] + s_acc[3][i]);
-        v[i] = ze[6 * (int64_t)e + i] - a;
+        v[i] = s_pre[kBsZe + i] - a;
         cr += v[i] * a;
     }
-    const double* L = Le + 36 * (int64_t)e;
+    const double* L = s_pre + kBsL;
 #pragma unroll
     for (int i = 5; i >= 0; --i) {
         double s = v[i];
@@ -525,7 +653,7 @@
     double d[6];
 #pragma unroll
     for (int i = 0; i < 6; ++i)
-        d[i] = -v[i] * scale[6 * (int64_t)(e_off_pose + e) + i];
+        d[i] = -v[i] * s_pre[kBsSc + i];
     if (lane < 6) {
         double out = 0.0;
 #pragma unroll
@@ -536,7 +664,7 @@
     if (lane == 0) {
         part_cross[e] = cr;
         if (FUSE)
-            candidate_for_pose(pv, e_off_pose + e, d, delta, H, g, active, pose_part);
+            candidate_for_pose(pv, e_off_pose + e, d, delta, s_pre + kBsX, s_pre + kBsH, s_pre + kBsG, &s_act, pose_part);
     }
 }
 
@@ -547,13 +675,14 @@
                             const int32_t* __restrict__ active, double* __restrict__ pose_part,
                             const int32_t* __restrict__ row_of)
 {
+    const LmHead head = lm_head(ctl);
     const bool remote = step_comm[7 * (int64_t)n_e] > 0.0;
-    if (remote && blockIdx.x == 0 && threadIdx.x == 0 && ctl->done != 1) {
-        if (ctl->done == 0)
+    if (remote && blockIdx.x == 0 && threadIdx.x == 0 && head.done != 1) {
+        if (head.done == 0)
             atomicOr(&ctl->sync_timeout, 4);
-        atomicExch(&ctl->done, 2);
-    }
-    if (ctl->done || remote)
+        atomicExch(&ctl->head.done, 2);
+    }
+    if (head.done || remote)
         return;
     const int p = blockIdx.x * blockDim.x + threadIdx.x;
     const int n_pose = pv.n_cams + pv.n_tags;
@@ -562,7 +691,7 @@
     const bool is_e = (p >= e_off_pose) && (p < e_off_pose + n_e);
     double d[6];
     for (int k = 0; k < 6; ++k) {
-        if (ctl->lin_fail)
+        if (head.lin_fail)
             d[k] = 0.0;
         else if (is_e)
             d[k] = step_comm[6 * (int64_t)(p - e_off_pose) + k];
diff --git a/visual_marker_mapping_amd/csrc/kernels_schur.hip b/visual_marker_mapping_amd/csrc/kernels_schur.hip
--- a/visual_marker_mapping_amd/csrc/kernels_schur.hip
+++ b/visual_marker_mapping_amd/csrc/kernels_schur.hip
@@ -22,16 +22,20 @@
                                                  int f_off_pose, double* __restrict__ Z, int ldz, int zcol,
                                                  const int32_t* __restrict__ e_start)
 {
-    if (ctl->done)
+    const LmHead head = lm_head(ctl);
+    const int64_t i = (int64_t)blockIdx.x * blockDim.x + threadIdx.x;
+    const bool valid = i < n_obs;
+    const int e = valid ? own[i] : 0, f = valid ? other[i] : 0;
+    const int e_prev = (valid && i > 0) ? own[i - 1] : -1;
+    loads_requested();
+    if (head.done)
         return;
     phase_stamp(ctl, 2);
-    const int64_t i = (int64_t)blockIdx.x * blockDim.x + threadIdx.x;
-    if (i >= n_obs)
-        return;
-    const WT* __restrict__ W = ctl->w_which ? W1 : W0;
-    const double* __restrict__ H_E = H_E0 + small_sel(ctl, alt_off);
-    const double* __restrict__ g_E = g_E0 + small_sel(ctl, alt_off);
-    const int e = own[i], f = other[i];
+    if (!valid)
+        return;
+    const WT* __restrict__ W = head.w_which ? W1 : W0;
+    const double* __restrict__ H_E = H_E0 + small_sel(head, alt_off);
+    const double* __restrict__ g_E = g_E0 + small_sel(head, alt_off);
     const double* se = scale + 6 * (int64_t)(e_off_pose + e);
     const double* sf = scale + 6 * (int64_t)(f_off_pose + f);
     double L[36];
@@ -46,10 +50,10 @@
         }
     }
     const bool ok = chol6(L);
-    const bool first = i == 0 || own[i - 1] != e;
+    const bool first = e_prev != e;
     if (first) {
         if (!ok)
-            ctl->lin_fail = 1;
+            ctl->head.lin_fail = 1;
         double v[6];
 #pragma unroll
         for (int a = 0; a < 6; ++a)
@@ -106,32 +110,33 @@
     const int64_t* wg_u1;
     const int32_t* wg_seg0;
     const int32_t* tile_seg0;
+    const SyrkWgRec* wg_rec;
+    const SyrkTileRec* tile_rec;
     double* partials;
 };
 
 __global__ __launch_bounds__(256, 2) void k_syrk_streamk(const LmCtl* ctl, const double* __restrict__ Z, int ldz,
                                                          SyrkPlanDev pl)
 {
-    if (ctl && ctl->done)
+    const LmHead head = lm_head(ctl);
+    const SyrkWgRec rec = pl.wg_rec[blockIdx.x];
+    loads_requested();
+    if (head.done)
         return;
     __shared__ __attribute__((aligned(16))) double As[2][kSyrkKT * kSyrkRow];
     __shared__ __attribute__((aligned(16))) double Bs[2][kSyrkKT * kSyrkRow];
-    const int g = blockIdx.x;
-    int64_t u = pl.wg_u0[g];
-    const int64_t u_end = pl.wg_u1[g];
-    int seg = pl.wg_seg0[g];
+    int left = rec.units, t = rec.tile, seg = rec.seg;
     const int tid = threadIdx.x;
     const int lane = tid & 63, wave = tid >> 6;
     const int wi = wave >> 1, wj = wave & 1;
     const int lr = tid >> 5;
     const int lc = (tid & 31) * 4;
     const int fk = lane >> 4, fi = lane & 15;
-    while (u < u_end) {
-        const int t = (int)(u / pl.n_kt);
-        const int kt0 = (int)(u % pl.n_kt);
-        const int64_t left = u_end - u;
-        const int kt1 = (kt0 + left < pl.n_kt) ? (int)(kt0 + left) : pl.n_kt;
-        const int I0 = pl.tile_bi[t] * kSyrkT, J0 = pl.tile_bj[t] * kSyrkT;
+    bool head_seg = true;
+    while (left > 0) {
+        const int kt0 = head_seg ? rec.kt0 : 0;
+        const int kt1 = head_seg ? rec.kt1 : min(left, pl.n_kt);
+        const int I0 = head_seg ? rec.I0 : pl.tile_bi[t] * kSyrkT, J0 = head_seg ? rec.J0 : pl.tile_bj[t] * kSyrkT;
         const bool diag = I0 == J0;
         double4_t acc[4][4];
 #pragma unroll
@@ -197,8 +202,10 @@
                     for (int r = 0; r < 4; ++r)
                         Cb[(wi * 64 + a * 16 + fk + 4 * r) * kSyrkT + wj * 64 + b * 16 + fi] = acc[a][b][r];
         }
-        u += kt1 - kt0;
+        left -= kt1 - kt0;
         ++seg;
+        ++t;
+        head_seg = false;
     }
 }
 
@@ -334,20 +341,20 @@
 
 __global__ __launch_bounds__(512, 1) void k_syrk_wide(const LmCtl* ctl, const double* __restrict__ Z, int ldz, SyrkPlanDev pl)
 {
-    if (ctl && ctl->done)
+    const LmHead head = lm_head(ctl);
+    const SyrkWgRec rec = pl.wg_rec[blockIdx.x];
+    loads_requested();
+    if (head.done)
         return;
     __shared__ __attribute__((aligned(16))) double smem[4 * kWideStage];
     static_assert(4 * kWideStage >= 4 * 16 * 256, "the accumulator exchange must fit into the stage buffers");
-    const int gidx = blockIdx.x;
-    const int64_t u = pl.wg_u0[gidx], u_end = pl.wg_u1[gidx];
-    if (u >= u_end)
-        return;
-    const int t = (int)(u / pl.n_kt);
-    const int kt0 = (int)(u % pl.n_kt), kt1 = kt0 + (int)(u_end - u);
-    const int I0 = pl.tile_bi[t] * kSyrkT, J0 = pl.tile_bj[t] * kSyrkT;
-    double* Cb = pl.partials + (size_t)pl.wg_seg0[gidx] * kSyrkTile;
+    const int kt0 = rec.kt0, kt1 = rec.kt0 + rec.units;
+    if (kt1 <= kt0)
+        return;
+    const int I0 = rec.I0, J0 = rec.J0;
+    double* Cb = pl.partials + (size_t)rec.seg * kSyrkTile;
     const int w = __builtin_amdgcn_readfirstlane((int)(threadIdx.x >> 6) & 3);
-    if (I0 == J0) {
+    if (rec.diag) {
         switch (w) {
         case 0: syrk_wide_item<true, 0>(Z, ldz, I0, J0, kt0, kt1, smem, Cb); break;
         case 1: syrk_wide_item<true, 1>(Z, ldz, I0, J0, kt0, kt1, smem, Cb); break;
@@ -378,19 +385,51 @@
                                                          double* __restrict__ S, DiagArgs da,
                                                          double* __restrict__ packed = nullptr)
 {
-    if (ctl && ctl->done)
-        return;
+    const LmHead head = lm_head(ctl);
     const int t = blockIdx.x >> 4;
     const int sub = blockIdx.x & 15;
     const int qi = sub >> 3, qj = (sub >> 2) & 1, rs = sub & 3;
-    const int I0 = pl.tile_bi[t] * kSyrkT + 64 * qi, J0 = pl.tile_bj[t] * kSyrkT + 64 * qj;
+    const SyrkTileRec rec = pl.tile_rec[t];
+    loads_requested();
+    if (head.done)
+        return;
+    const int I0 = rec.I0 + 64 * qi, J0 = rec.J0 + 64 * qj;
     if (J0 > I0 || I0 + 16 * rs >= n_rows)
         return;
-    const int s0 = pl.tile_seg0[t], s1 = pl.tile_seg0[t + 1];
+    const int s0 = rec.s0, s1 = rec.s1;
     const int tr = 16 * rs + (threadIdx.x >> 5), tc = (threadIdx.x & 31) * 2;
     if (ADD_DIAG && ctl) {
-        da.H_F += small_sel(ctl, da.alt_off);
-        da.g_F += small_sel(ctl, da.alt_off);
+        da.H_F += small_sel(head, da.alt_off);
+        da.g_F += small_sel(head, da.alt_off);
+    }
+    double add[2][2][4];
+    int kind[2][2];
+#pragma unroll
+    for (int i = 0; i < 2; ++i) {
+        const int row = I0 + tr + 8 * i;
+#pragma unroll
+        for (int h = 0; h < 2; ++h) {
+            const int col = J0 + tc + h;
+            kind[i][h] = 0;
+            add[i][h][0] = add[i][h][1] = add[i][h][2] = add[i][h][3] = 0.0;
+            if (ADD_DIAG && row < n_rows) {
+                if (row == da.n_pad) {
+                    if (col < da.n_red) {
+                        kind[i][h] = 1;
+                        add[i][h][0] = da.scale_F[col];
+                        add[i][h][1] = da.g_F[col];
+                    }
+                } else if (row < da.n_red && col <= row && (row / 6) == (col / 6)) {
+                    const int f = row / 6, a = row % 6, b = col % 6;
+                    kind[i][h] = 2;
+                    add[i][h][0] = da.scale_F[row];
+                    add[i][h][1] = da.H_F[36 * (int64_t)f + 6 * a + b];
+                    add[i][h][2] = da.scale_F[col];
+                    if (a == b)
+                        add[i][h][3] = da.D2_F[row];
+                }
+            }
+        }
     }
     double2 acc[2] = { make_double2(0.0, 0.0), make_double2(0.0, 0.0) };
     const double* p0 = pl.partials + (size_t)(64 * qi + tr) * kSyrkT + 64 * qj + tc;
@@ -415,14 +454,12 @@
             const int col = J0 + tc + h;
             double v = out[h];
             if (ADD_DIAG) {
-                if (row == da.n_pad) {
-                    if (col < da.n_red)
-                        v += da.scale_F[col] * da.g_F[col];
-                } else if (row < da.n_red && col <= row && (row / 6) == (col / 6)) {
-                    const int f = row / 6, a = row % 6, b = col % 6;
-                    v += da.scale_F[row] * da.H_F[36 * (int64_t)f + 6 * a + b] * da.scale_F[col];
-                    if (a == b)
-                        v += da.D2_F[row];
+                if (kind[i][h] == 1) {
+                    v += add[i][h][0] * add[i][h][1];
+                } else if (kind[i][h] == 2) {
+                    v += add[i][h][0] * add[i][h][1] * add[i][h][2];
+                    if (row % 6 == col % 6)
+                        v += add[i][h][3];
                 } else if (row >= da.n_red && row < da.n_pad && col == row) {
                     v = 1.0;
                 }
@@ -465,7 +502,8 @@
 
 __global__ __launch_bounds__(kPairThreads) void k_schur_pairs(PairArgs a)
 {
-    if (a.ctl && a.ctl->done)
+    const LmHead head = lm_head(a.ctl);
+    if (head.done)
         return;
     const int tid = threadIdx.x;
     const int n_red = a.da.n_red, n_pad = a.da.n_pad, ld = a.ld;
@@ -594,8 +632,8 @@
     if (!active || sl != 0)
         return;
     if (a.add_diag && a.ctl) {
-        a.da.H_F += small_sel(a.ctl, a.da.alt_off);
-        a.da.g_F += small_sel(a.ctl, a.da.alt_off);
+        a.da.H_F += small_sel(head, a.da.alt_off);
+        a.da.g_F += small_sel(head, a.da.alt_off);
     }
     if (rhs) {
 #pragma unroll
@@ -621,7 +659,7 @@
 
 __global__ __launch_bounds__(256) void k_fill_lower(const LmCtl* ctl, double* __restrict__ S, int ld, int n_pad, int unit_diag)
 {
-    if (ctl && ctl->done)
+    if (lm_head(ctl).done)
         return;
     const int row = blockIdx.x;
     const int c1 = row == n_pad ? n_pad : (row / 64) * 64 + 64;
@@ -651,6 +689,8 @@
     d.wg_u1 = p.wg_u1;
     d.wg_seg0 = p.wg_seg0;
     d.tile_seg0 = p.tile_seg0;
+    d.wg_rec = p.wg_rec;
+    d.tile_rec = p.tile_rec;
     d.partials = p.partials;
     return d;
 }
@@ -772,7 +812,7 @@
 __global__ __launch_bounds__(256) void k_pack_lower(const LmCtl* ctl, const double* __restrict__ S, int ld, int n_rows,
                                                     double* __restrict__ packed, bool unpack, double* __restrict__ Sout)
 {
-    if (ctl && ctl->done)
+    if (lm_head(ctl).done)
         return;
     const int r = blockIdx.x;
     if (r >= n_rows)
@@ -793,7 +833,7 @@
                                                      int n_pad, const int32_t* __restrict__ pose_of_row,
                                                      const int32_t* __restrict__ row_of)
 {
-    if (ctl && ctl->done)
+    if (lm_head(ctl).done)
         return;
     const int r = blockIdx.x;
     const int64_t base = (int64_t)r * (r + 1) / 2;
diff --git a/visual_marker_mapping_amd/csrc/standalone.hip b/visual_marker_mapping_amd/csrc/standalone.hip
--- a/visual_marker_mapping_amd/csrc/standalone.hip
+++ b/visual_marker_mapping_amd/csrc/standalone.hip
@@ -183,9 +183,9 @@
     for (int attempt = 0; attempt < 2 && err == hipSuccess; ++attempt) {
         memset(&c, 0, sizeof(c));
         if (attempt == 0) {
-            c.spin_limit_df = e.sw.spin_df;
-            c.spin_limit_chain = e.sw.spin_chain;
-            c.spin_wg = e.sw.spin_wg;
+            c.head.spin_limit_df = e.sw.spin_df;
+            c.head.spin_limit_chain = e.sw.spin_chain;
+            c.head.spin_wg = e.sw.spin_wg;
         }
         err = hipMemcpyAsync(e.ctl, &c, sizeof(LmCtl), hipMemcpyHostToDevice, e.stream);
         if (err == hipSuccess)
@@ -197,7 +197,7 @@
         if (err == hipSuccess) err = hipMemcpyAsync(x, y, sizeof(double) * n, hipMemcpyDeviceToHost, e.stream);
         if (err == hipSuccess) err = hipMemcpyAsync(&c, e.ctl, sizeof(LmCtl), hipMemcpyDeviceToHost, e.stream);
         if (err == hipSuccess) err = hipStreamSynchronize(e.stream);
-        if (c.done != 2)
+        if (c.head.done != 2)
             break;
     }
     free_scratch(e);
@@ -206,7 +206,7 @@
         return VMM_BA_ERR_HIP;
     }
     if (info)
-        *info = c.lin_fail;
+        *info = c.head.lin_fail;
     return VMM_BA_OK;
 }
 
diff --git a/visual_marker_mapping_amd/csrc/vmm_ba.hip b/visual_marker_mapping_amd/csrc/vmm_ba.hip
--- a/visual_marker_mapping_amd/csrc/vmm_ba.hip
+++ b/visual_marker_mapping_amd/csrc/vmm_ba.hip
@@ -135,6 +135,30 @@
     if ((rc = upload(e, p.wg_u1, s.wg_u1))) return rc;
     if ((rc = upload(e, p.wg_seg0, s.wg_seg0))) return rc;
     if ((rc = upload(e, p.tile_seg0, s.tile_seg0))) return rc;
+    std::vector<SyrkWgRec> wg_rec((size_t)s.n_wg);
+    for (int g = 0; g < s.n_wg; ++g) {
+        SyrkWgRec r = {};
+        const int64_t u0 = s.wg_u0[g], u1 = s.wg_u1[g];
+        if (u1 > u0) {
+            const int t = (int)(u0 / s.n_kt);
+            r.tile = t;
+            r.units = (int32_t)(u1 - u0);
+            r.I0 = s.tile_bi[t] * kST;
+            r.J0 = s.tile_bj[t] * kST;
+            r.kt0 = (int32_t)(u0 % s.n_kt);
+            r.kt1 = (int32_t)std::min<int64_t>(r.kt0 + (u1 - u0), s.n_kt);
+            r.seg = s.wg_seg0[g];
+            r.diag = r.I0 == r.J0 ? 1 : 0;
+        }
+        wg_rec[g] = r;
+    }
+    std::vector<SyrkTileRec> tile_rec((size_t)s.n_tiles);
+    for (int t = 0; t < s.n_tiles; ++t)
+        tile_rec[t] = SyrkTileRec{ s.tile_bi[t] * kST, s.tile_bj[t] * kST, s.tile_seg0[t], s.tile_seg0[t + 1] };
+    if ((rc = dev_alloc(e, &p.wg_rec, wg_rec.size()))) return rc;
+    if ((rc = dev_alloc(e, &p.tile_rec, tile_rec.size()))) return rc;
+    if ((rc = upload(e, p.wg_rec, wg_rec))) return rc;
+    if ((rc = upload(e, p.tile_rec, tile_rec))) return rc;
     HIP_TRY(hipStreamSynchronize(e.stream));
     return VMM_BA_OK;
 }
@@ -472,10 +496,10 @@
     c.num_sync_timeouts++;
     c.sync_kernels |= c.sync_timeout;
     c.sync_timeout = 0;
-    c.lin_fail = 0;
-    c.done = 0;
+    c.head.lin_fail = 0;
+    c.head.done = 0;
     if (e.sw.spin_once)
-        c.spin_limit_df = c.spin_limit_chain = 0;
+        c.head.spin_limit_df = c.head.spin_limit_chain = 0;
     HIP_TRY(hipMemcpyAsync(e.ctl, e.ctl_host, sizeof(LmCtl), hipMemcpyHostToDevice, e.stream));
     Range r("vmm_ba sync time-out recovery");
     int rc;
@@ -521,9 +545,9 @@
 void init_ctl(Engine& e, LmCtl& c, const vmm_ba_options& o, int trace_capacity)
 {
     memset(&c, 0, sizeof(c));
-    c.spin_limit_df = e.sw.spin_df;
-    c.spin_limit_chain = e.sw.spin_chain;
-    c.spin_wg = e.sw.spin_wg;
+    c.head.spin_limit_df = e.sw.spin_df;
+    c.head.spin_limit_chain = e.sw.spin_chain;
+    c.head.spin_wg = e.sw.spin_wg;
     c.max_num_iterations = o.max_num_iterations;
     c.robustify = o.robustify;
     c.jacobi_scaling = o.jacobi_scaling;
@@ -539,7 +563,7 @@
     c.max_lm_diagonal = o.max_lm_diagonal;
     c.radius = o.initial_trust_region_radius;
     c.decrease_factor = 2.0;
-    c.first_eval = 1;
+    c.head.first_eval = 1;
     c.termination = VMM_BA_NO_CONVERGENCE;
     c.trace_capacity = trace_capacity;
 }
@@ -709,6 +733,9 @@
         set_error("hipMemsetAsync(obs_mask) failed");
         return VMM_BA_ERR_HIP;
     }
+    if ((rc = dev_alloc(e, &e.ordE.mask, (size_t)std::max<int64_t>(e.ordE.n, 1), false))) return rc;
+    if ((rc = dev_alloc(e, &e.ordF.mask, (size_t)std::max<int64_t>(e.ordF.n, 1), false))) return rc;
+    launch_sort_mask(e);
     if ((rc = dev_alloc(e, &e.pose_const, (size_t)n_pose))) return rc;
     if ((rc = upload_pose_const(e, nullptr, nullptr))) return rc;
     const size_t n_stat = (size_t)e.ordE.n_tasks + (size_t)e.ordF.n_tasks + 1;
@@ -1127,7 +1154,7 @@
         }
         HIP_TRY(hipMemcpyAsync(e.ctl_host, e.ctl, sizeof(LmCtl), hipMemcpyDeviceToHost, e.stream));
         HIP_TRY(hipStreamSynchronize(e.stream));
-        if (e.ctl_host->done == 2) {
+        if (e.ctl_host->head.done == 2) {
             if (e.ctl_host->num_sync_timeouts >= 1000) {
                 set_error("the one-launch factorisation gave up waiting in 1000 passes of one solve (kernels: "
                           + std::to_string(e.ctl_host->sync_kernels | e.ctl_host->sync_timeout) + ")");
@@ -1137,7 +1164,7 @@
             enq = e.ctl_host->num_lm_iterations;
             continue;
         }
-        if (e.ctl_host->done)
+        if (e.ctl_host->head.done)
             break;
         if (enq >= max_steps) {
             set_error("LM loop did not terminate within max_num_iterations + 2 passes");
@@ -1212,6 +1239,8 @@
     } else {
         HIP_TRY(hipMemsetAsync(e.obs_mask, 1, (size_t)e.n_obs, e.stream));
     }
+    launch_sort_mask(e);
+    HIP_TRY(hipGetLastError());
     return VMM_BA_OK;
 }
 
```

After: 2535 LM iterations/s, median of 6. 1.02x the previous value.
